# wuqianliang/Diff-Reg

Hardware: AMD Instinct MI355X
Metric: scene-pairs/sec @ 20 denoise steps (N=M=256); IR/FMR parity vs ref (higher is better)
Workload: dtype f32; 1 GPU; cfg2: 3DMatch N=M=256, C=432, 20 denoise steps, max_condition_num=200 (warp active), 256 independent B=1 pairs per pass per GPU as 2 concurrent batch(es), one HIP-graph replay each on its own stream; pairs_per_pass_per_gpu=256, streams=2, denoise_steps=20, N=256, M=256, graph=True, parallelism=pairs sharded over 1 GPU(s)

## Files before the change

diff-reg_amd/csrc/api.hip:

```cpp
#include <stdlib.h>
#include "loop_common.h"
#include <vector>
#include <stdio.h>
#include <string.h>

namespace dr {
static thread_local char g_hip_err[512] = "";
void set_hip_error(hipError_t e, const char* where) {
    snprintf(g_hip_err, sizeof(g_hip_err), "%s: %s (%d)", where, hipGetErrorString(e), (int)e);
}

static bool g_env_knobs = false;
void enable_env_knobs(bool on) { g_env_knobs = on; }
int env_knob(const char* name, int def) {
    if (!g_env_knobs) return def;
    const char* e = getenv(name);
    return e ? atoi(e) : def;
}

int device_cu_count() {
    static int cache[64];
    int d = 0;
    if (hipGetDevice(&d) != hipSuccess || d < 0 || d >= 64) return 256;
    if (!cache[d]) {
        hipDeviceProp_t pr;
        cache[d] = hipGetDeviceProperties(&pr, d) == hipSuccess && pr.multiProcessorCount > 0 ? pr.multiProcessorCount : 256;
    }
    return cache[d];
}

bool g_prof_on = false;
struct ProfRec { int kind; double work; hipEvent_t a, b; };
static std::vector<ProfRec> g_prof;
static std::vector<hipEvent_t> g_pool;
static hipEvent_t get_event() {
    if (!g_pool.empty()) { hipEvent_t e = g_pool.back(); g_pool.pop_back(); return e; }
    hipEvent_t e = nullptr; (void)hipEventCreate(&e); return e;
}
void prof_begin(int kind, double work, hipStream_t st) {
    ProfRec r; r.kind = kind; r.work = work; r.a = get_event(); r.b = nullptr;
    (void)hipEventRecord(r.a, st);
    g_prof.push_back(r);
}
void prof_end(int kind, hipStream_t st) {
    for (size_t i = g_prof.size(); i-- > 0;)
        if (g_prof[i].kind == kind && !g_prof[i].b) { g_prof[i].b = get_event(); (void)hipEventRecord(g_prof[i].b, st); return; }
}
}

namespace dr {
__global__ void noop_kernel(int* p) { if (p && threadIdx.x == 0 && blockIdx.x == 0) *p = 0; }
}

extern "C" {
void dr_prof_enable(int on) { dr::g_prof_on = on != 0; }

int dr_prof_collect(int* calls, double* ms, double* work) {
    using namespace dr;
    DR_HIP_CHECK(hipDeviceSynchronize());
    for (int k = 0; k < PK_COUNT; ++k) { calls[k] = 0; ms[k] = 0; work[k] = 0; }
    for (auto& r : g_prof) {
        if (r.b) {
            float t = 0.f;
            (void)hipEventElapsedTime(&t, r.a, r.b);
            calls[r.kind] += 1; ms[r.kind] += t; work[r.kind] += r.work;
            g_pool.push_back(r.b);
        }
        g_pool.push_back(r.a);
    }
    g_prof.clear();
    return DR_OK;
}

int dr_debug_launch_chain(int n, int workgroups, int threads, void* stream) {
    if (n < 0 || workgroups < 1 || threads < 64 || threads > 1024) return DR_EINVAL;
    for (int i = 0; i < n; ++i) hipLaunchKernelGGL(dr::noop_kernel, dim3(workgroups), dim3(threads), 0, (hipStream_t)stream, (int*)nullptr);
    DR_LAUNCH_CHECK();
    return DR_OK;
}

int dr_version(void) { return DR_ABI_VERSION;  }

const char* dr_strerror(int code) {
    switch (code) {
        case DR_OK: return "ok";
        case DR_EINVAL: return "invalid argument";
        case DR_ELAUNCH: return "HIP call failed";
        case DR_ENOSUP: return "shape not supported by this build";
        case DR_EWORKSPACE: return "workspace missing or too small";
        case DR_ETIMEOUT: return "a kernel gave up waiting for a workgroup that was not resident (outputs of that call are unspecified: NaN where the waiting workgroup wrote)";
        default: return "unknown error";
    }
}

const char* dr_last_hip_error(void) { return dr::g_hip_err; }
}

using namespace dr;

extern "C" {

int dr_init(void) {
    int rc = attention_configure();
    if (rc == DR_OK) rc = gemm_configure();
    if (rc == DR_OK) rc = pgemm_configure();
    if (rc == DR_OK) rc = vit_f32_configure();
    if (rc == DR_OK && !device_status_word()) rc = DR_ELAUNCH;
    return rc;
}

void dr_debug_enable_env(int on) { enable_env_knobs(on != 0); }
void dr_debug_gemm_config(int c) { gemm_force_config(c); }

int dr_debug_gemm_f32(const dr_debug_gemm_problem* problems, int n, void* stream) {
    if (!problems || n < 1 || n > 4) return DR_EINVAL;
    GemmBatch g;
    memset(&g, 0, sizeof(g));
    for (int i = 0; i < n; ++i) {
        const dr_debug_gemm_problem& q = problems[i];
        const int K1 = q.A2 ? q.K1 : q.K;
        if (q.rows < 0 || q.ncols <= 0 || q.K <= 0 || !q.A || !q.W || !q.out || q.nbatch < 0) return DR_EINVAL;
        if (q.lda < K1 || q.ldo < q.ncols || (q.A2 && (K1 <= 0 || K1 >= q.K || q.lda2 < q.K - K1))) return DR_EINVAL;
        if ((q.epilogue & ~(EPI_RELU | EPI_ROTARY)) ||
            ((q.epilogue & EPI_ROTARY) && (!q.cos_t || !q.sin_t || q.rot_C <= 0 || (q.rot_C & 1))))
            return DR_EINVAL;
        GemmProblem& p = g.p[i];
        p.A = q.A; p.A2 = q.A2; p.W = q.W; p.out = q.out; p.cosT = q.cos_t; p.sinT = q.sin_t; p.bias = q.bias; p.addend = q.addend;
        p.rows = q.rows; p.ncols = q.ncols; p.K = q.K; p.K1 = K1; p.lda = q.lda; p.lda2 = q.A2 ? q.lda2 : 0; p.ldo = q.ldo;
        p.epi = q.epilogue; p.rot_C = q.rot_C; p.scale = q.scale;
        p.nbatch = q.nbatch; p.sA = q.stride_a; p.sW = q.stride_w; p.sO = q.stride_o;
    }
    g.n = n;
    return launch_gemm(g, (hipStream_t)stream);
}
void dr_debug_attention_config(int flash_min_workgroups) { attention_force_flash_min(flash_min_workgroups); }
void dr_debug_attention_split(int on) { attention_force_split(on); }
int dr_debug_attention_last_form(void) { return attention_last_form(); }
int dr_debug_procrustes_last_form(void) { return procrustes_last_form(); }

int dr_vol_pe_f32(int rows, int rows_per_pair, int C, const float* xyz, const float* R, const float* t, float origin_x,
                  float origin_y, float origin_z, float voxel, const float* freq, float* cos_out, float* sin_out,
                  void* stream) {
    if (rows < 0 || C <= 0 || !xyz || !freq || !cos_out || !sin_out || rows_per_pair < 1) return DR_EINVAL;
    if ((R == nullptr) != (t == nullptr)) return DR_EINVAL;
    return launch_vol_pe(xyz, rows, rows_per_pair, R, t, C, origin_x, origin_y, origin_z, voxel, freq, cos_out, sin_out,
                         (hipStream_t)stream);
}

int dr_linear_f32(int rows, int ncols, int K, const float* x, const float* W, float* out, int epilogue, const float* cos_t,
                  const float* sin_t, int rot_C, float scale, void* stream) {
    if (rows < 0 || ncols <= 0 || K <= 0 || !x || !W || !out) return DR_EINVAL;
    if ((epilogue & EPI_ROTARY) && (!cos_t || !sin_t || rot_C <= 0 || (rot_C & 1))) return DR_EINVAL;
    return gemm1(x, K, W, nullptr, out, ncols, rows, ncols, K, epilogue, scale, nullptr, (hipStream_t)stream, cos_t, sin_t, rot_C);
}

int dr_gemm_nt_batched_f32(int nbatch, int rows, int ncols, int K, const float* A, long long stride_a, const float* W, long long stride_w, float* out,
                           long long stride_o, float scale, void* stream) {
    if (nbatch < 0 || rows < 0 || ncols <= 0 || K <= 0 || (K & 3) || !A || !W || !out) return DR_EINVAL;
    if (nbatch == 0 || rows == 0) return DR_OK;
    return gemm1(A, K, W, nullptr, out, ncols, rows, ncols, K, EPI_NONE, scale, nullptr, (hipStream_t)stream, nullptr, nullptr, 0, nbatch, stride_a,
                 stride_w, stride_o);
}

int dr_linear_ex_f32(int rows, int ncols, int K, const float* x, int lda, const float* W, const float* bias, float* out, int ldo,
                     int epilogue, float scale, void* stream) {
    if (rows < 0 || ncols <= 0 || K <= 0 || !x || !W || !out || lda < K || ldo < ncols || (epilogue & EPI_ROTARY)) return DR_EINVAL;
    return gemm1(x, lda, W, bias, out, ldo, rows, ncols, K, epilogue, scale, nullptr, (hipStream_t)stream);
}

size_t dr_procrustes_workspace_bytes(int P, int N, int M) {
    return (P < 1 || N < 1 || M < 1) ? 0 : procrustes_workspace_bytes(P, N, M);
}

int dr_procrustes_f32(int P, int N, int M, const float* conf, const float* src_pcd, const float* tgt_pcd,
                      const uint8_t* src_mask, const uint8_t* tgt_mask, int use_mask_len, float sample_rate,
                      float max_condition_num, float* R, float* t, float* R_forwd, float* t_forwd, double* condition,
                      int32_t* solution_mask, int32_t* topk_idx, void* workspace, size_t workspace_bytes, void* stream) {
    if (P < 0 || N < 1 || M < 1 || !conf || !src_pcd || !tgt_pcd || !R || !t || !R_forwd || !t_forwd || !condition || !solution_mask)
        return DR_EINVAL;
    if (P == 0) return DR_OK;
    const size_t wsb = procrustes_workspace_bytes(P, N, M);
    if (wsb && (!workspace || workspace_bytes < wsb)) return DR_EWORKSPACE;
    return launch_procrustes(conf, src_pcd, tgt_pcd, src_mask, tgt_mask, P, N, M, use_mask_len, sample_rate, max_condition_num,
                             R, t, R_forwd, t_forwd, condition, solution_mask, topk_idx, (hipStream_t)stream, wsb ? workspace : nullptr, wsb);
}

size_t dr_top1_union_workspace_bytes(int P, int N, int M, int elem_bytes) {
    return (P < 1 || N < 1 || M < 1 || (elem_bytes != 4 && elem_bytes != 8)) ? 0 : top1_union_workspace_bytes(P, N, M, (size_t)elem_bytes);
}

}
template <typename T>
static int top1_union_entry(const T* conf, int P, int N, int M, int64_t* matches, int32_t* count, void* ws, size_t ws_bytes, hipStream_t st) {
    if (P < 0 || N < 1 || M < 1 || !conf || !matches || !count) return DR_EINVAL;
    if (P == 0) return DR_OK;
    const size_t wsb = top1_union_workspace_bytes(P, N, M, sizeof(T));
    if (wsb && (!ws || ws_bytes < wsb)) return DR_EWORKSPACE;
    return launch_top1_union<T>(conf, P, N, M, (long long*)matches, count, st, nullptr, nullptr, wsb ? ws : nullptr, wsb);
}
extern "C" {
int dr_top1_union_f64(int P, int N, int M, const double* conf, int64_t* matches, int32_t* count, void* workspace, size_t workspace_bytes,
                      void* stream) {
    return top1_union_entry<double>(conf, P, N, M, matches, count, workspace, workspace_bytes, (hipStream_t)stream);
}
int dr_top1_union_f32(int P, int N, int M, const float* conf, int64_t* matches, int32_t* count, void* workspace, size_t workspace_bytes,
                      void* stream) {
    return top1_union_entry<float>(conf, P, N, M, matches, count, workspace, workspace_bytes, (hipStream_t)stream);
}

}
```

diff-reg_amd/csrc/loop.hip:

```cpp
#include "loop_common.h"

namespace dr {

struct LayerWs {
    float *qkv, *att, *mrg, *msg, *hid, *g2;
    size_t T;
    static size_t carve(Carver& c, LayerWs& w, size_t T, int C) {
        w.T = T;
        w.qkv = c.take<float>(T * 3 * C);
        w.att = c.take<float>(T * C);
        w.mrg = c.take<float>(T * C);
        w.msg = c.take<float>(T * C);
        w.hid = c.take<float>(T * 2 * C);
        w.g2 = c.take<float>(T * C);
        return c.off;
    }
};

struct PrepackLayer {
    PgW qkv, merge, mlp0, mlp2;
    const float *lnB1, *lnB2;
};
struct Prepack {
    static constexpr int MAXL = 16;
    PrepackLayer L[MAXL];
    PgW head;
    int dp;
    static bool supported(const dr_loop_config& cfg) {
        if (!(cfg.n_layers <= MAXL && pgemm_shape_ok(cfg.C) && cfg.C % cfg.H == 0 && (cfg.C / cfg.H) % 4 == 0)) return false;
        const int dp = (cfg.C / cfg.H + 15) / 16 * 16;
        return pgemm_shape_ok(cfg.H * dp) && pgemm_bn(cfg.H * dp) == pgemm_bn(cfg.C) && (dp == 64 || dp == 112 || dp == 144);
    }
    static bool wide_layout(const dr_loop_config& cfg) { return pgemm_bn(cfg.C) > 448 && env_knob("DR_PG_WIDE", 1) != 0; }
    static size_t carve(void* buf, const dr_loop_config& cfg, Prepack* pp) {
        Carver c(buf);
        const int C = cfg.C, d = C / cfg.H, dp = (d + 15) / 16 * 16, nC = C / 16;
        if (pp) pp->dp = dp;
        const bool wide = wide_layout(cfg);
        for (int l = 0; l < cfg.n_layers; ++l) {
            PrepackLayer* L = pp ? &pp->L[l] : nullptr;
            take_weight(c, C, 3, nC, L ? &L->qkv : nullptr, wide);
            take_weight(c, C, 1, cfg.H * dp / 16, L ? &L->merge : nullptr);
            take_weight(c, C, 2, 2 * nC, L ? &L->mlp0 : nullptr, wide);
            take_weight(c, C, 1, 2 * nC, L ? &L->mlp2 : nullptr);
            float* b = c.take<float>(2);
            if (L && buf) { L->lnB1 = b; L->lnB2 = b + 1; }
        }
        take_weight(c, C, 1, nC, pp ? &pp->head : nullptr, wide);
        return c.off + 256;
    }
    static int fill(void* buf, const dr_loop_config& cfg, const dr_loop_weights& W, hipStream_t st) {
        Prepack pp;
        carve(buf, cfg, &pp);
        const int C = cfg.C, d = C / cfg.H;
        for (int l = 0; l < cfg.n_layers; ++l) {
            const dr_layer_weights& w = W.layers[l];
            const PrepackLayer& L = pp.L[l];
            const int Cq = cfg.H * pp.dp;
            int rc = pack_weight_block(w.q_proj, Cq, C, C, C, L.qkv, 0, st, d, pp.dp);
            if (rc == DR_OK) rc = pack_weight_block(w.k_proj, Cq, C, C, C, L.qkv, 1, st, d, pp.dp);
            if (rc == DR_OK) rc = pack_weight_block(w.v_proj, Cq, C, C, C, L.qkv, 2, st, d, pp.dp);
            if (rc == DR_OK) rc = pack_weight_block(w.merge, C, C, d, pp.dp, L.merge, 0, st);
            if (rc == DR_OK) rc = pack_weight_block(w.mlp0, C, 2 * C, 2 * C, 2 * C, L.mlp0, 0, st);
            if (rc == DR_OK) rc = pack_weight_block(w.mlp0 + (size_t)C * 2 * C, C, 2 * C, 2 * C, 2 * C, L.mlp0, 1, st);
            if (rc == DR_OK) rc = pack_weight_block(w.mlp2, C, 2 * C, 2 * C, 2 * C, L.mlp2, 0, st);
            if (rc == DR_OK) rc = launch_ln_bound(w.norm1_w, w.norm1_b, C, (float*)L.lnB1, st);
            if (rc == DR_OK) rc = launch_ln_bound(w.norm2_w, w.norm2_b, C, (float*)L.lnB2, st);
            if (rc) return rc;
        }
        return pack_weight_block(W.src_proj, C, C, C, C, pp.head, 0, st);
    }
};

struct PlanesWs {
    bool on;
    Tok feat0, fa, fb, tgt_l0;
    char *att_img, *msg_img, *hid_img;
    float *att_bnd, *msg_bnd, *hid_bnd;
    char *qkv_img, *kvc_img;
    float *qkv_bnd, *kvc_bnd;
    float* grp_x;
    bool hoist;
    float* pre0;
    char* v0_img; float *v0_bnd, *grp0;
    char* q1_img; float* q1_bnd;
    float* csT;
    size_t qkv_stride;
    size_t side_C, side_att, side_hid;
    void* own_pack;
    float* xk_buf; unsigned* xk_flags; mutable unsigned xk_epoch; unsigned* status;
    static size_t img_bytes(int PN, int PM, int K) { return plane_image_bytes(PN, K) + plane_image_bytes(PM, K); }
    static void carve(Carver& c, PlanesWs& w, const dr_loop_config& cfg, int P, int N, int M) {
        const int C = cfg.C, PN = P * N, PM = P * M, T = PN + PM;
        w.on = planes_wanted(cfg.flags, Prepack::supported(cfg), T);
        if (!w.on) return;
        const int dp = (C / cfg.H + 15) / 16 * 16;
        w.side_C = plane_image_bytes(PN, C); w.side_att = plane_image_bytes(PN, cfg.H * dp); w.side_hid = plane_image_bytes(PN, 2 * C);
        Tok* toks[4] = {&w.feat0, &w.fa, &w.fb, &w.tgt_l0};
        for (Tok* t : toks) { t->f32 = nullptr; t->img = c.take<char>(img_bytes(PN, PM, C)); t->bnd = c.take<float>(T); }
        w.att_img = c.take<char>(img_bytes(PN, PM, cfg.H * dp)); w.att_bnd = c.take<float>(T);
        w.msg_img = c.take<char>(img_bytes(PN, PM, C)); w.msg_bnd = c.take<float>(T);
        w.hid_img = c.take<char>(img_bytes(PN, PM, 2 * C)); w.hid_bnd = c.take<float>(T);
        w.qkv_stride = (img_bytes(PN, PM, cfg.H * dp) + 255) & ~(size_t)255;
        w.qkv_img = c.take<char>(3 * w.qkv_stride); w.qkv_bnd = c.take<float>(3 * (size_t)T);
        w.kvc_img = c.take<char>(2 * w.qkv_stride); w.kvc_bnd = c.take<float>(2 * (size_t)T);
        w.grp_x = c.take<float>(2 * (size_t)P);
        w.hoist = false;
        w.csT = c.take<float>((size_t)T * C);
        w.own_pack = c.take<char>(Prepack::carve(nullptr, cfg, nullptr));
        const bool xk = (T + 63) / 64 + 2 <= PG_XK_MAX_RB;
        w.xk_buf = xk ? c.take<float>(pgemm_xk_buf_bytes(pgemm_bn(C)) / 4) : nullptr;
        w.xk_flags = xk ? c.take<unsigned>(pgemm_xk_flag_bytes() / 4) : nullptr;
        w.xk_epoch = 0; w.status = nullptr;
    }
    static void carve_hoist(PlanesWs& w, char* mem, size_t bytes, const dr_loop_config& cfg, int P, int N, int M) {
        const int PN = P * N, PM = P * M, T = PN + PM, Cq = cfg.H * ((cfg.C / cfg.H + 15) / 16 * 16);
        Carver c(mem);
        w.pre0 = c.take<float>((size_t)PN * 2 * Cq);
        w.v0_img = c.take<char>(plane_image_bytes(PN, Cq)); w.v0_bnd = c.take<float>(PN); w.grp0 = c.take<float>(P);
        w.q1_img = c.take<char>(plane_image_bytes(PM, Cq)); w.q1_bnd = c.take<float>(T);
        w.hoist = c.off <= bytes && env_knob("DR_LOOP_HOIST", 1) != 0;
    }
};

static int layer_call(const dr_layer_weights& W, int C, int H, int P, const float* xin, int xr0, int xrows,
                      const float* yin, int yr0, int yrows, const float* cosT, const float* sinT,
                      const uint8_t* tokmask, const Family& f1, const Family* f2, const LayerWs& ws, float* out,
                      hipStream_t st, const float* kv_cached = nullptr, float* kv_store = nullptr, const float* xq_in = nullptr,
                      const float* yk_in = nullptr) {
    const int halfC = C / 2, d = C / H;
    const bool rotary = cosT != nullptr;
    const float* const qin = xq_in ? xq_in : xin;
    const float* const kin = yk_in ? yk_in : yin;
    GemmBatch g;
    memset(&g, 0, sizeof(g));
    auto proj = [&](GemmProblem& p, const float* in, int r0, int rows, const float* Wm, int coloff, bool rot) {
        p.A = in + (size_t)r0 * C; p.A2 = nullptr; p.W = Wm; p.out = ws.qkv + (size_t)r0 * 3 * C + coloff;
        p.rows = rows; p.ncols = C; p.K = C; p.K1 = C; p.lda = C; p.lda2 = 0; p.ldo = 3 * C;
        p.epi = (rot && rotary) ? EPI_ROTARY : EPI_NONE; p.rot_C = C; p.scale = 1.f;
        p.cosT = rotary ? cosT + (size_t)r0 * halfC : nullptr; p.sinT = rotary ? sinT + (size_t)r0 * halfC : nullptr;
    };
    int rc;
    if (kv_store) {
        proj(g.p[0], kin, yr0, yrows, W.k_proj, 0, true);
        proj(g.p[1], yin, yr0, yrows, W.v_proj, 0, false);
        g.p[0].out = kv_store + (size_t)yr0 * 2 * C; g.p[0].ldo = 2 * C;
        g.p[1].out = kv_store + (size_t)yr0 * 2 * C + C; g.p[1].ldo = 2 * C;
        g.n = 2;
        return launch_gemm(g, st);
    }
    proj(g.p[0], qin, xr0, xrows, W.q_proj, 0, true);
    g.n = 1;
    if (!kv_cached) {
        proj(g.p[1], kin, yr0, yrows, W.k_proj, C, true);
        proj(g.p[2], yin, yr0, yrows, W.v_proj, 2 * C, false);
        g.n = 3;
    }
    rc = launch_gemm(g, st);
    if (rc) return rc;

    AttnArgs a;
    memset(&a, 0, sizeof(a));
    a.q = ws.qkv; a.k = ws.qkv + C; a.v = ws.qkv + 2 * C; a.out = ws.att;
    a.ldq = a.ldk = a.ldv = 3 * C; a.ldo = C; a.H = H; a.d = d;
    if (kv_cached) { a.k = kv_cached; a.v = kv_cached + C; a.ldk = a.ldv = 2 * C; }
    a.qmask = tokmask; a.kmask = tokmask;
    attn_families(a, P, f1, f2);
    a.scale = 1.0f / sqrtf((float)d);
    rc = launch_attention(a, st);
    if (rc) return rc;

    memset(&g, 0, sizeof(g));
    GemmProblem& m = g.p[0];
    m.A = ws.att + (size_t)xr0 * C; m.W = W.merge; m.out = ws.mrg + (size_t)xr0 * C;
    m.rows = xrows; m.ncols = C; m.K = C; m.K1 = C; m.lda = C; m.ldo = C; m.epi = EPI_NONE; m.scale = 1.f;
    g.n = 1;
    rc = launch_gemm(g, st);
    if (rc) return rc;
    rc = launch_layernorm(ws.mrg + (size_t)xr0 * C, C, W.norm1_w, W.norm1_b, nullptr, 0, ws.msg + (size_t)xr0 * C, C, xrows, C, st);
    if (rc) return rc;
    memset(&g, 0, sizeof(g));
    GemmProblem& h = g.p[0];
    h.A = xin + (size_t)xr0 * C; h.A2 = ws.msg + (size_t)xr0 * C; h.W = W.mlp0; h.out = ws.hid + (size_t)xr0 * 2 * C;
    h.rows = xrows; h.ncols = 2 * C; h.K = 2 * C; h.K1 = C; h.lda = C; h.lda2 = C; h.ldo = 2 * C; h.epi = EPI_RELU; h.scale = 1.f;
    g.n = 1;
    rc = launch_gemm(g, st);
    if (rc) return rc;
    memset(&g, 0, sizeof(g));
    GemmProblem& o = g.p[0];
    o.A = ws.hid + (size_t)xr0 * 2 * C; o.W = W.mlp2; o.out = ws.g2 + (size_t)xr0 * C;
    o.rows = xrows; o.ncols = C; o.K = 2 * C; o.K1 = 2 * C; o.lda = 2 * C; o.ldo = C; o.epi = EPI_NONE; o.scale = 1.f;
    g.n = 1;
    rc = launch_gemm(g, st);
    if (rc) return rc;
    return launch_layernorm(ws.g2 + (size_t)xr0 * C, C, W.norm2_w, W.norm2_b, xin + (size_t)xr0 * C, C, out + (size_t)xr0 * C, C,
                            xrows, C, st);
}


using PlCtx = PlaneCtx<Prepack, PlanesWs>;
static void xk_assign(const PlanesWs& pw, int C, PgProblem& p, size_t& next, size_t units) {
    if (!pw.xk_buf || next + units > (size_t)PG_XK_MAX_RB) return;
    p.xk_buf = pw.xk_buf + next * (pgemm_xk_buf_bytes(pgemm_bn(C)) / 4 / PG_XK_MAX_RB); p.xk_flags = pw.xk_flags + next * 2; p.xk_cap = (int)units;
    p.xk_epoch = pw.xk_epoch + 1; p.xk_status = pw.status;
    next += units;
}
static size_t xk_wide_units(const PgProblem& p) { return (size_t)(p.rows + 127) / 128 * p.nblk * 2; }

struct PlHoist {
    bool l0_fill = false;
    bool l0_use = false;
    bool q1_fill = false;
    bool q1_use = false;
};
static int layer_call_planes(const PlCtx& X, const dr_layer_weights& W, int l, const Tok& xin, int xs, const Tok& yin, int ys,
                             const Tok& out, const Family& f1, const Family* f2, hipStream_t st, const float* kv_cached = nullptr,
                             float* kv_store = nullptr, const PlHoist& hz = PlHoist()) {
    const Sides& S = X.S;
    const int C = X.C, H = X.H, PN = S.rows_a, PM = S.rows_b, halfC = C / 2, d = C / H, nC = C / 16, dp = X.pp->dp;
    const PrepackLayer& L = X.pp->L[l];
    const PlanesWs& pw = *X.pw;
    PgBatch g;
    size_t xk_next = 0;
    auto reset = [&]() { memset(&g, 0, sizeof(g)); xk_next = 0; };
    auto add = [&]() -> PgProblem& { return g.p[g.n++]; };
    auto xk = [&](PgProblem& p, size_t units) { xk_assign(pw, C, p, xk_next, units); };
    int rc;

    const int T = PN + PM, Cq = H * dp, nq = Cq / 16;
    const bool cached = kv_cached != nullptr;
    char* const kv_img = kv_store ? pw.kvc_img : pw.qkv_img + pw.qkv_stride;
    float* const kv_bnd = kv_store ? pw.kvc_bnd : pw.qkv_bnd + T;
    const bool grp_inline = S.La % 128 == 0 && S.Lb % 128 == 0 && env_knob("DR_LOOP_GRP_INLINE", 1) != 0;
    if (!cached && !grp_inline && !hz.l0_fill && !hz.l0_use && !hz.q1_fill) {
        rc = side_group_max(S, ys, yin.bnd, pw.grp_x, st);
        if (rc) return rc;
    }
    auto proj = [&](const Tok& tin, int side, int b0, int nblk, char* img, float* bnd, int rotm, int grpm) {
        PgProblem& p = add();
        p.A0 = S.at(tin.img, pw.side_C, side); p.bnd0 = tin.bnd + S.r0(side); p.nc0 = nC;
        p.W = pgw_blocks(L.qkv, b0, C); p.nblk = nblk; p.rows = S.rows(side); p.C = Cq; p.k_alg = C; p.mode = PG_PLANES;
        p.rot_mask = rotm; p.rot_C = C; p.rot_piece_len = d; p.rot_piece_pad = dp; p.scale = 1.f;
        p.cosT = X.cosT + (size_t)S.r0(side) * halfC; p.sinT = X.sinT + (size_t)S.r0(side) * halfC;
        p.csT = X.pw->csT + (size_t)S.r0(side) * halfC * 2;
        p.pimg = S.at(img, pw.side_att, side); p.p_nct = nq; p.pbnd = bnd + S.r0(side);
        p.pimg_blk_stride = (long long)pw.qkv_stride; p.pbnd_blk_stride = T;
        p.grp_bnd = grp_inline ? nullptr : pw.grp_x; p.grp_mask = grpm; p.grp_first = S.grp_first(side); p.grp_rows = S.per_pair(side);
        if (p.W.sub == 2) xk(p, xk_wide_units(p));
    };
    reset();
    if (kv_store) {
        S.for_sides(ys, [&](int side) { proj(yin, side, 1, 2, kv_img, kv_bnd, 1, 3); });
        ++pw.xk_epoch;
        return launch_pgemm(g, st);
    }
    const int rbS = (PN + 127) / 128, rbT = (PM + 127) / 128;
    if (hz.l0_fill) {
        rc = launch_group_max(xin.bnd, S.P, S.La, pw.grp0, st);
        if (rc) return rc;
        proj(xin, SIDE_A, 0, 2, pw.qkv_img, pw.qkv_bnd, 0, 0);
        g.p[0].mode = PG_F32; g.p[0].pimg = nullptr; g.p[0].pbnd = nullptr;
        g.p[0].out = pw.pre0; g.p[0].ldo = 2 * Cq; g.p[0].blk_stride = Cq;
        g.wg_as = 3 * rbS;
        ++pw.xk_epoch;
        rc = launch_pgemm(g, st);
        if (rc) return rc;
        reset();
        proj(xin, SIDE_A, 2, 1, pw.v0_img, pw.v0_bnd, 0, 1);
        g.p[0].grp_bnd = pw.grp0; g.p[0].grp_first = 0;
        g.wg_as = 3 * rbS;
        ++pw.xk_epoch;
        return launch_pgemm(g, st);
    }
    if (hz.q1_fill) {
        proj(xin, SIDE_B, 0, 1, pw.qkv_img, pw.qkv_bnd, 1, 0);
        g.p[0].pimg = pw.q1_img; g.p[0].pbnd = pw.q1_bnd + PN;
        g.wg_as = rbT + 2 * rbS;
        ++pw.xk_epoch;
        return launch_pgemm(g, st);
    }
    const bool self = xs == ys && xin.img == yin.img && !cached;
    if (hz.l0_use) {
        RotImgArgs r;
        memset(&r, 0, sizeof(r));
        r.x = pw.pre0; r.ldx = 2 * Cq; r.x_blk = Cq; r.rows = PN; r.C = Cq; r.nblk = 2;
        r.csT = pw.csT; r.rot_mask = 3; r.rot_C = C; r.rot_piece_len = d; r.rot_piece_pad = dp; r.scale = 1.f;
        r.bnd0 = xin.bnd; r.wnorm = L.qkv.wnorm; r.wide_form = L.qkv.sub == 2; r.grp_bnd = pw.grp0; r.grp_mask = 2; r.grp_first = 0; r.grp_rows = S.La;
        r.pimg = pw.qkv_img; r.p_nct = nq; r.pbnd = pw.qkv_bnd; r.pimg_blk_stride = (long long)pw.qkv_stride; r.pbnd_blk_stride = T;
        rc = launch_rot_images(r, st);
        if (rc) return rc;
    } else {
        if (self) {
            S.for_sides(xs, [&](int side) { proj(xin, side, 0, 3, pw.qkv_img, pw.qkv_bnd, 3, 6); });
        } else {
            if (!hz.q1_use) S.for_sides(xs, [&](int side) { proj(xin, side, 0, 1, pw.qkv_img, pw.qkv_bnd, 1, 0); });
            else g.wg_as = rbT + 2 * rbS;
            if (!cached) S.for_sides(ys, [&](int side) { proj(yin, side, 1, 2, kv_img, kv_bnd, 1, 3); });
        }
        ++pw.xk_epoch;
        rc = launch_pgemm(g, st);
        if (rc) return rc;
    }

    AttnArgs a;
    memset(&a, 0, sizeof(a));
    a.H = H; a.d = d;
    a.qmask = X.tokmask; a.kmask = X.tokmask;
    attn_families(a, S.P, f1, f2);
    a.scale = 1.0f / sqrtf((float)d);
    a.pimg[0] = pw.att_img; a.pimg[1] = pw.att_img + pw.side_att; a.p_split = PN; a.p_nct = nq; a.p_dp = dp;
    a.pbnd = pw.att_bnd;
    {
        const char* kimg = cached ? pw.kvc_img : pw.qkv_img + pw.qkv_stride;
        const float* kb = cached ? pw.kvc_bnd : pw.qkv_bnd + T;
        a.qimg[0] = pw.qkv_img; a.qimg[1] = pw.qkv_img + pw.side_att;
        a.kimg[0] = kimg; a.kimg[1] = kimg + pw.side_att;
        a.vimg[0] = kimg + pw.qkv_stride; a.vimg[1] = kimg + pw.qkv_stride + pw.side_att;
        a.qbnd = pw.qkv_bnd; a.kgb = kb; a.vgb = kb + T;
        if (hz.l0_use) { a.vimg[0] = pw.v0_img; a.vgb = pw.v0_bnd; }
        if (hz.q1_use) { a.qimg[1] = pw.q1_img; a.qbnd = pw.q1_bnd; }
        a.f16_single = X.attn_f16;
    }
    rc = launch_attention(a, st);
    if (rc) return rc;

    reset();
    S.for_sides(xs, [&](int side) {
        PgProblem& p = add();
        p.A0 = S.at(pw.att_img, pw.side_att, side); p.bnd0 = pw.att_bnd + S.r0(side); p.nc0 = H * dp / 16;
        p.W = L.merge; p.nblk = 1; p.rows = S.rows(side); p.C = C; p.mode = PG_LN; p.k_alg = C;
        p.gamma = W.norm1_w; p.beta = W.norm1_b; p.lnB = L.lnB1;
        p.pimg = S.at(pw.msg_img, pw.side_C, side); p.p_nct = nC; p.pbnd = pw.msg_bnd + S.r0(side);
        xk(p, (size_t)(p.rows + 63) / 64);
    });
    ++pw.xk_epoch;
    rc = launch_pgemm(g, st);
    if (rc) return rc;
    reset();
    S.for_sides(xs, [&](int side) {
        PgProblem& p = add();
        p.A0 = S.at(xin.img, pw.side_C, side); p.bnd0 = xin.bnd + S.r0(side); p.nc0 = nC;
        p.A1 = S.at(pw.msg_img, pw.side_C, side); p.bnd1 = pw.msg_bnd + S.r0(side); p.nc1 = nC;
        p.W = L.mlp0; p.nblk = 2; p.rows = S.rows(side); p.C = C; p.mode = PG_PLANES; p.relu = 1; p.scale = 1.f;
        p.pimg = S.at(pw.hid_img, pw.side_hid, side); p.p_nct = 2 * nC; p.pbnd = pw.hid_bnd + S.r0(side);
        if (p.W.sub == 2) xk(p, xk_wide_units(p));
    });
    ++pw.xk_epoch;
    rc = launch_pgemm(g, st);
    if (rc) return rc;
    reset();
    S.for_sides(xs, [&](int side) {
        PgProblem& p = add();
        p.A0 = S.at(pw.hid_img, pw.side_hid, side); p.bnd0 = pw.hid_bnd + S.r0(side); p.nc0 = 2 * nC;
        p.W = L.mlp2; p.nblk = 1; p.rows = S.rows(side); p.C = C; p.mode = PG_LN;
        p.gamma = W.norm2_w; p.beta = W.norm2_b; p.lnB = L.lnB2;
        p.resid = xin.f32 + (size_t)S.r0(side) * C; p.ldr = C; p.bnd_res = xin.bnd + S.r0(side);
        p.out = out.f32 + (size_t)S.r0(side) * C; p.ldo = C;
        p.pimg = S.at(out.img, pw.side_C, side); p.p_nct = nC; p.pbnd = out.bnd + S.r0(side);
        xk(p, (size_t)(p.rows + 63) / 64);
    });
    ++pw.xk_epoch;
    return launch_pgemm(g, st);
}

struct DenoiseWs {
    LayerWs lw;
    float *fa, *fb, *cosT, *sinT, *proj, *sim;
    float *tgt_l0, *kv_l1;
    PlanesWs pl;
    const Prepack* pp;
    Sides S;
    static void carve(Carver& c, DenoiseWs& w, const dr_loop_config& cfg, int P, int N, int M) {
        const int C = cfg.C;
        w.S = Sides(P, N, M);
        const size_t T = (size_t)P * (N + M);
        const size_t lw_begin = align256(c.off);
        LayerWs::carve(c, w.lw, T, C);
        const size_t lw_end = c.off;
        PlanesWs::carve(c, w.pl, cfg, P, N, M);
        if (w.pl.on) PlanesWs::carve_hoist(w.pl, c.base ? c.base + lw_begin : nullptr, lw_end - lw_begin, cfg, P, N, M);
        w.tgt_l0 = c.take<float>(T * C);
        w.kv_l1 = c.take<float>(T * 2 * C);
        w.fa = c.take<float>(T * C);
        w.fb = c.take<float>(T * C);
        w.cosT = c.take<float>(T * (C / 2));
        w.sinT = c.take<float>(T * (C / 2));
        w.proj = c.take<float>(T * C);
        w.sim = c.take<float>((size_t)P * N * M);
        if (w.pl.on) { w.pl.fa.f32 = w.fa; w.pl.fb.f32 = w.fb; w.pl.tgt_l0.f32 = w.tgt_l0; }
    }
};

static PlCtx plane_ctx(const dr_loop_config& cfg, const DenoiseWs& ws, const uint8_t* tokmask) {
    return PlCtx{ws.pp, &ws.pl, ws.S, cfg.C, cfg.H, (cfg.flags & DR_LOOP_ATTN_F16) ? 1 : 0, ws.cosT, ws.sinT, tokmask};
}
static int layer_call_sides(const dr_loop_config& cfg, const dr_layer_weights& W, const float* x, int xs, const float* y, int ys, const uint8_t* tokmask,
                            const Family& f1, const Family* f2, const DenoiseWs& ws, float* out, hipStream_t st, const float* kv_cached = nullptr,
                            float* kv_store = nullptr) {
    const Sides& S = ws.S;
    return layer_call(W, cfg.C, cfg.H, S.P, x, S.r0(xs), S.rows(xs), y, S.r0(ys), S.rows(ys), ws.cosT, ws.sinT, tokmask, f1, f2, ws.lw, out, st,
                      kv_cached, kv_store);
}

static int fill_step_invariants(const dr_loop_config& cfg, const dr_loop_weights& w, const float* feat0, const uint8_t* tokmask, DenoiseWs& ws,
                                hipStream_t st) {
    const Family self_s = ws.S.self_a(), self_t = ws.S.self_b();
    if (ws.pl.on) {
        const PlCtx X = plane_ctx(cfg, ws, tokmask);
        int rc = layer_call_planes(X, w.layers[0], 0, ws.pl.feat0, SIDE_B, ws.pl.feat0, SIDE_B, ws.pl.tgt_l0, self_t, nullptr, st);
        if (rc == DR_OK && ws.pl.hoist) {
            PlHoist hz; hz.l0_fill = true;
            rc = layer_call_planes(X, w.layers[0], 0, ws.pl.feat0, SIDE_A, ws.pl.feat0, SIDE_A, ws.pl.tgt_l0, self_s, nullptr, st, nullptr, nullptr, hz);
        }
        if (rc || cfg.n_layers < 2) return rc;
        rc = layer_call_planes(X, w.layers[1], 1, ws.pl.tgt_l0, 0, ws.pl.tgt_l0, SIDE_B, ws.pl.tgt_l0, self_t, nullptr, st, nullptr, ws.kv_l1);
        if (rc || !ws.pl.hoist) return rc;
        PlHoist hz; hz.q1_fill = true;
        return layer_call_planes(X, w.layers[1], 1, ws.pl.tgt_l0, SIDE_B, ws.pl.tgt_l0, 0, ws.pl.tgt_l0, self_t, nullptr, st, nullptr, nullptr, hz);
    }
    int rc = layer_call_sides(cfg, w.layers[0], feat0, SIDE_B, feat0, SIDE_B, tokmask, self_t, nullptr, ws, ws.tgt_l0, st);
    if (rc || cfg.n_layers < 2) return rc;
    return layer_call_sides(cfg, w.layers[1], nullptr, 0, ws.tgt_l0, SIDE_B, tokmask, self_t, nullptr, ws, nullptr, st, nullptr, ws.kv_l1);
}

static int denoiser_and_sim(const dr_loop_config& cfg, const dr_loop_weights& w, const float* feat0, const uint8_t* tokmask, DenoiseWs& ws,
                            const float** final_feats, hipStream_t st, bool use_cache = false) {
    const Sides& S = ws.S;
    const int C = cfg.C, P = S.P, N = S.La, M = S.Lb, PN = S.rows_a;
    auto head = [&](const float* feats) {
        return gemm1(feats, C, w.src_proj, nullptr, ws.proj, C, S.rows(SIDE_BOTH), C, C, EPI_ROTARY, 1.0f / sqrtf((float)C), nullptr, st, ws.cosT, ws.sinT, C);
    };
    auto sim = [&]() {
        return gemm1(ws.proj, C, ws.proj + (size_t)PN * C, nullptr, ws.sim, M, N, M, C, EPI_NONE, 1.f, nullptr, st, nullptr, nullptr, 0, P,
                     (long long)N * C, (long long)M * C, (long long)N * M);
    };
    const int l_begin = use_cache ? 1 : 0;
    if (ws.pl.on) {
        const PlCtx X = plane_ctx(cfg, ws, tokmask);
        const Tok* cur = &ws.pl.feat0;
        int rc = DR_OK;
        if (use_cache) {
            PlHoist hz; hz.l0_use = ws.pl.hoist;
            rc = layer_call_planes(X, w.layers[0], 0, *cur, SIDE_A, *cur, SIDE_A, ws.pl.tgt_l0, S.self_a(), nullptr, st, nullptr, nullptr, hz);
            cur = &ws.pl.tgt_l0;
        }
        if (rc == DR_OK)
            rc = layer_schedule(S, l_begin, cfg.n_layers, cur, (const Tok*)&ws.pl.fa, (const Tok*)&ws.pl.fb,
                                [&](int l, int xs, const Tok* x, int ys, const Tok* y, const Tok* out, const Family& f1, const Family* f2) {
                const bool l1 = use_cache && l == 1;
                PlHoist hz; hz.q1_use = l1 && xs == SIDE_B && ws.pl.hoist;
                return layer_call_planes(X, w.layers[l], l, *x, xs, *y, ys, *out, f1, f2, st, (l1 && xs == SIDE_A) ? ws.kv_l1 : nullptr, nullptr, hz);
            });
        if (rc) return rc;
        *final_feats = cur->f32;
        if (env_knob("DR_HEAD_F32", 0)) {
            rc = head(cur->f32);
            return rc ? rc : sim();
        }
        PgBatch g;
        memset(&g, 0, sizeof(g));
        size_t xk_next = 0;
        S.for_sides(SIDE_BOTH, [&](int side) {
            PgProblem& p = g.p[g.n++];
            const int r0 = S.r0(side);
            p.A0 = S.at(cur->img, ws.pl.side_C, side); p.bnd0 = cur->bnd + r0; p.nc0 = C / 16;
            p.W = ws.pp->head; p.nblk = 1; p.rows = S.rows(side); p.C = C; p.mode = PG_F32;
            p.out = ws.proj + (size_t)r0 * C; p.ldo = C; p.blk_stride = 0; p.rot_mask = 1; p.rot_C = C; p.scale = 1.0f / sqrtf((float)C);
            p.cosT = ws.cosT + (size_t)r0 * (C / 2); p.sinT = ws.sinT + (size_t)r0 * (C / 2);
            p.csT = ws.pl.csT + (size_t)r0 * C;
            if (p.W.sub == 2) xk_assign(ws.pl, C, p, xk_next, xk_wide_units(p));
        });
        ++ws.pl.xk_epoch;
        rc = launch_pgemm(g, st);
        return rc ? rc : sim();
    }
    const float* cur = feat0;
    int rc = DR_OK;
    if (use_cache) {
        rc = layer_call_sides(cfg, w.layers[0], cur, SIDE_A, cur, SIDE_A, tokmask, S.self_a(), nullptr, ws, ws.tgt_l0, st);
        cur = ws.tgt_l0;
    }
    if (rc == DR_OK)
        rc = layer_schedule(S, l_begin, cfg.n_layers, cur, ws.fa, ws.fb,
                            [&](int l, int xs, const float* x, int ys, const float* y, float* out, const Family& f1, const Family* f2) {
            return layer_call_sides(cfg, w.layers[l], x, xs, y, ys, tokmask, f1, f2, ws, out, st, (use_cache && l == 1 && xs == SIDE_A) ? ws.kv_l1 : nullptr);
        });
    if (rc) return rc;
    *final_feats = cur;
    rc = head(cur);
    return rc ? rc : sim();
}

static int fill_pe(const dr_loop_config& cfg, const dr_loop_weights& w, int P, int N, int M, const float* s_pcd,
                   const float* Rf, const float* tf, const float* t_pcd, bool do_src, bool do_tgt, DenoiseWs& ws,
                   hipStream_t st) {
    const int halfC = cfg.C / 2;
    int rc = DR_OK;
    if (do_src)
        rc = launch_vol_pe(s_pcd, P * N, N, Rf, tf, cfg.C, cfg.origin[0], cfg.origin[1], cfg.origin[2], cfg.voxel, w.pe_freq,
                           ws.cosT, ws.sinT, st, ws.pl.on ? ws.pl.csT : nullptr);
    if (rc == DR_OK && do_tgt)
        rc = launch_vol_pe(t_pcd, P * M, M, nullptr, nullptr, cfg.C, cfg.origin[0], cfg.origin[1], cfg.origin[2], cfg.voxel,
                           w.pe_freq, ws.cosT + (size_t)P * N * halfC, ws.sinT + (size_t)P * N * halfC, st,
                           ws.pl.on ? ws.pl.csT + (size_t)P * N * halfC * 2 : nullptr);
    return rc;
}

struct LoopWs {
    DenoiseWs dw;
    float *feat0, *wconf, *x0, *R, *t, *Rf, *tf, *conf32;
    double *x, *dmin, *cond;
    void* pmin;
    int* ok;
    uint8_t* tokmask;
    void* skws;
    size_t skws_bytes;
    void* pws;
    size_t pws_bytes;
    unsigned* status;
    static size_t carve(Carver& c, LoopWs& w, const dr_loop_config& cfg, int P, int N, int M) {
        const size_t T = (size_t)P * (N + M), NM = (size_t)P * N * M;
        w.status = c.take<unsigned>(4);
        DenoiseWs::carve(c, w.dw, cfg, P, N, M);
        w.feat0 = c.take<float>(T * cfg.C);
        if (w.dw.pl.on) w.dw.pl.feat0.f32 = w.feat0;
        w.wconf = c.take<float>(NM);
        w.x0 = c.take<float>(NM);
        w.conf32 = c.take<float>(NM);
        w.x = c.take<double>(NM);
        w.dmin = c.take<double>(P);
        w.cond = c.take<double>(P);
        w.pmin = (void*)c.take<char>(pair_min_scratch_bytes(P));
        w.R = c.take<float>((size_t)P * 9);
        w.t = c.take<float>((size_t)P * 3);
        w.Rf = c.take<float>((size_t)P * 9);
        w.tf = c.take<float>((size_t)P * 3);
        w.ok = c.take<int>(P);
        w.tokmask = c.take<uint8_t>(T);
        sampler_scratch(c, P, N, M, cfg.flags, w.skws, w.skws_bytes, w.pws, w.pws_bytes);
        return c.off + 256;
    }
};

static int planes_begin(const dr_loop_config& cfg, const dr_loop_weights& w, DenoiseWs& ws, Prepack& pp, hipStream_t st) {
    if (!ws.pl.on) return DR_OK;
    int rc = packed_or_own(cfg, w, ws.pl.own_pack, pp, st);
    if (rc) return rc;
    ws.pp = &pp;
    if (ws.pl.xk_flags) {
        DR_HIP_CHECK(hipMemsetAsync(ws.pl.xk_flags, 0, pgemm_xk_flag_bytes(), st));
        ws.pl.xk_epoch = 0;
    }
    ws.S.for_sides(SIDE_BOTH, [&](int side) { if (rc == DR_OK) rc = side_planes_from_f32(ws.S, side, ws.pl.feat0, cfg.C, ws.pl.side_C, st); });
    return rc;
}

static int loop_begin(const dr_loop_config& cfg, int P, int N, int M, const float* src_feats, const float* tgt_feats, const uint8_t* src_mask,
                      const uint8_t* tgt_mask, void* workspace, LoopWs& L, hipStream_t st) {
    Carver c(workspace);
    LoopWs::carve(c, L, cfg, P, N, M);
    DR_HIP_CHECK(hipMemsetAsync(L.status, 0, 16, st));
    L.dw.pl.status = L.status;
    const size_t PN = (size_t)P * N, PM = (size_t)P * M;
    DR_HIP_CHECK(hipMemcpyAsync(L.feat0, src_feats, PN * cfg.C * 4, hipMemcpyDeviceToDevice, st));
    DR_HIP_CHECK(hipMemcpyAsync(L.feat0 + PN * cfg.C, tgt_feats, PM * cfg.C * 4, hipMemcpyDeviceToDevice, st));
    if (src_mask) {
        DR_HIP_CHECK(hipMemcpyAsync(L.tokmask, src_mask, PN, hipMemcpyDeviceToDevice, st));
        DR_HIP_CHECK(hipMemcpyAsync(L.tokmask + PN, tgt_mask, PM, hipMemcpyDeviceToDevice, st));
    }
    return DR_OK;
}

}

using namespace dr;

extern "C" {

size_t dr_attention_layer_workspace_bytes(int P, int Lx, int Ly, int C) {
    Carver c(nullptr);
    LayerWs w;
    const size_t T = (size_t)P * (Lx + Ly);
    LayerWs::carve(c, w, T, C);
    c.take<float>(T * C);
    c.take<float>(T * C);
    c.take<float>(T * (C / 2));
    c.take<float>(T * (C / 2));
    c.take<uint8_t>(T);
    c.take<float>(T * C);
    return c.off + 256;
}

int dr_attention_layer_f32(const dr_layer_weights* w, int C, int H, int P, int Lx, int Ly, const float* x, const float* y,
                           const float* cos_x, const float* sin_x, const float* cos_y, const float* sin_y,
                           const uint8_t* x_mask, const uint8_t* y_mask, float* out, void* workspace,
                           size_t workspace_bytes, void* stream) {
    if (!cos_x || !sin_x || !cos_y || !sin_y) return DR_EINVAL;
    return dr_attention_layer_pe_f32(w, C, H, P, Lx, Ly, x, y, nullptr, nullptr, cos_x, sin_x, cos_y, sin_y, x_mask, y_mask, out, workspace,
                                     workspace_bytes, stream);
}

int dr_attention_layer_pe_f32(const dr_layer_weights* w, int C, int H, int P, int Lx, int Ly, const float* x, const float* y,
                              const float* xq, const float* yk, const float* cos_x, const float* sin_x, const float* cos_y, const float* sin_y,
                              const uint8_t* x_mask, const uint8_t* y_mask, float* out, void* workspace,
                              size_t workspace_bytes, void* stream) {
    if (!w || !x || !y || !out || P < 1 || Lx < 1 || Ly < 1 || C % H || (C / H) % 4 || C % 4) return DR_EINVAL;
    if ((x_mask == nullptr) != (y_mask == nullptr)) return DR_EINVAL;
    const bool rotary = cos_x != nullptr;
    if ((sin_x != nullptr) != rotary || (cos_y != nullptr) != rotary || (sin_y != nullptr) != rotary) return DR_EINVAL;
    if ((xq == nullptr) != (yk == nullptr) || (xq && rotary)) return DR_EINVAL;
    if (workspace_bytes < dr_attention_layer_workspace_bytes(P, Lx, Ly, C) || !workspace) return DR_EWORKSPACE;
    hipStream_t st = (hipStream_t)stream;
    Carver c(workspace);
    LayerWs lw;
    const size_t T = (size_t)P * (Lx + Ly), PX = (size_t)P * Lx, PY = (size_t)P * Ly;
    const int halfC = C / 2;
    LayerWs::carve(c, lw, T, C);
    float* tok = c.take<float>(T * C);
    float* otok = c.take<float>(T * C);
    float* cosT = c.take<float>(T * halfC);
    float* sinT = c.take<float>(T * halfC);
    uint8_t* mask = c.take<uint8_t>(T);
    float* qk_buf = c.take<float>(T * C);
    DR_HIP_CHECK(hipMemcpyAsync(tok, x, PX * C * 4, hipMemcpyDeviceToDevice, st));
    DR_HIP_CHECK(hipMemcpyAsync(tok + PX * C, y, PY * C * 4, hipMemcpyDeviceToDevice, st));
    float* qk_tok = nullptr;
    if (rotary) {
        DR_HIP_CHECK(hipMemcpyAsync(cosT, cos_x, PX * halfC * 4, hipMemcpyDeviceToDevice, st));
        DR_HIP_CHECK(hipMemcpyAsync(cosT + PX * halfC, cos_y, PY * halfC * 4, hipMemcpyDeviceToDevice, st));
        DR_HIP_CHECK(hipMemcpyAsync(sinT, sin_x, PX * halfC * 4, hipMemcpyDeviceToDevice, st));
        DR_HIP_CHECK(hipMemcpyAsync(sinT + PX * halfC, sin_y, PY * halfC * 4, hipMemcpyDeviceToDevice, st));
    } else if (xq) {
        qk_tok = qk_buf;
        DR_HIP_CHECK(hipMemcpyAsync(qk_tok, xq, PX * C * 4, hipMemcpyDeviceToDevice, st));
        DR_HIP_CHECK(hipMemcpyAsync(qk_tok + PX * C, yk, PY * C * 4, hipMemcpyDeviceToDevice, st));
    }
    if (x_mask) {
        DR_HIP_CHECK(hipMemcpyAsync(mask, x_mask, PX, hipMemcpyDeviceToDevice, st));
        DR_HIP_CHECK(hipMemcpyAsync(mask + PX, y_mask, PY, hipMemcpyDeviceToDevice, st));
    }
    const Family f{0, Lx, (int)PX, Ly};
    int rc = layer_call(*w, C, H, P, tok, 0, (int)PX, tok, (int)PX, (int)PY, rotary ? cosT : nullptr, rotary ? sinT : nullptr,
                        x_mask ? mask : nullptr, f, nullptr, lw, otok, st, nullptr, nullptr, qk_tok, qk_tok);
    if (rc) return rc;
    DR_HIP_CHECK(hipMemcpyAsync(out, otok, PX * C * 4, hipMemcpyDeviceToDevice, st));
    return DR_OK;
}

static int check_cfg(const dr_loop_config* cfg, const dr_loop_weights* w, int P, int N, int M) {
    if (!cfg || !w || P < 1 || N < 1 || M < 1) return DR_EINVAL;
    if (cfg->C % cfg->H || (cfg->C / cfg->H) % 4 || cfg->C % 6 || cfg->n_layers < 1 || cfg->sk_iters < 1) return DR_EINVAL;
    if (!w->layers || !w->src_proj || !w->bin_score || !w->pe_freq) return DR_EINVAL;
    if (cfg->variant != DR_VARIANT_3DMATCH && cfg->variant != DR_VARIANT_4DMATCH) return DR_EINVAL;
    return DR_OK;
}

size_t dr_loop_prepack_bytes(const dr_loop_config* cfg) {
    if (!cfg || !Prepack::supported(*cfg)) return 0;
    return Prepack::carve(nullptr, *cfg, nullptr);
}

int dr_loop_prepack(const dr_loop_config* cfg, const dr_loop_weights* w, void* packed, size_t packed_bytes, void* stream) {
    if (!cfg || !w || !w->layers || !w->src_proj || !packed || ((uintptr_t)packed & 255)) return DR_EINVAL;
    if (!Prepack::supported(*cfg)) return DR_ENOSUP;
    if (packed_bytes < Prepack::carve(nullptr, *cfg, nullptr)) return DR_EWORKSPACE;
    return Prepack::fill(packed, *cfg, *w, (hipStream_t)stream);
}

size_t dr_denoise_loop_workspace_bytes(const dr_loop_config* cfg, int P, int N, int M) {
    if (!cfg || P < 1 || N < 1 || M < 1) return 0;
    Carver c(nullptr);
    LoopWs w;
    return LoopWs::carve(c, w, *cfg, P, N, M);
}

int dr_denoise_loop_status(void* workspace, void* stream, int clear) {
    if (!workspace) return DR_EINVAL;
    Carver c(workspace);
    return sinkhorn_call_status(c.take<unsigned>(4), (hipStream_t)stream, clear != 0);
}

int dr_denoiser_match_f32(const dr_loop_config* cfg, const dr_loop_weights* w, int P, int N, int M, const float* src_feats,
                          const float* tgt_feats, const float* s_pcd_warped, const float* t_pcd, const uint8_t* src_mask,
                          const uint8_t* tgt_mask, float* src_out, float* tgt_out, float* conf, void* workspace,
                          size_t workspace_bytes, void* stream) {
    int rc = check_cfg(cfg, w, P, N, M);
    if (rc) return rc;
    if (!src_feats || !tgt_feats || !s_pcd_warped || !t_pcd || !conf) return DR_EINVAL;
    if ((src_mask == nullptr) != (tgt_mask == nullptr)) return DR_EINVAL;
    if (!workspace || workspace_bytes < dr_denoise_loop_workspace_bytes(cfg, P, N, M)) return DR_EWORKSPACE;
    hipStream_t st = (hipStream_t)stream;
    LoopWs L;
    rc = loop_begin(*cfg, P, N, M, src_feats, tgt_feats, src_mask, tgt_mask, workspace, L, st);
    if (rc) return rc;
    const int C = cfg->C;
    const size_t PN = (size_t)P * N, PM = (size_t)P * M;
    Prepack pp;
    rc = planes_begin(*cfg, *w, L.dw, pp, st);
    if (rc) return rc;
    rc = fill_pe(*cfg, *w, P, N, M, s_pcd_warped, nullptr, nullptr, t_pcd, true, true, L.dw, st);
    if (rc) return rc;
    const float* fin = nullptr;
    rc = denoiser_and_sim(*cfg, *w, L.feat0, src_mask ? L.tokmask : nullptr, L.dw, &fin, st);
    if (rc) return rc;
    if (src_out) DR_HIP_CHECK(hipMemcpyAsync(src_out, fin, PN * C * 4, hipMemcpyDeviceToDevice, st));
    if (tgt_out) DR_HIP_CHECK(hipMemcpyAsync(tgt_out, fin + PN * C, PM * C * 4, hipMemcpyDeviceToDevice, st));
    return sinkhorn_f32(P, N, M, L.dw.sim, src_mask, tgt_mask, w->bin_score, cfg->sk_iters,
                        DR_SK_OUT_CONF | (src_mask ? DR_SK_APPLY_MASK : 0), conf, L.skws, L.skws_bytes, st, L.status);
}

int dr_denoise_loop(const dr_loop_config* cfg, const dr_loop_weights* w, int P, int N, int M, const float* src_feats,
                    const float* tgt_feats, const float* s_pcd, const float* t_pcd, const uint8_t* src_mask,
                    const uint8_t* tgt_mask, const float* x_T, const float* noise, double* conf, double* x_final,
                    int64_t* matches, int32_t* match_count, float* R_final, float* t_final, const dr_loop_trace* trace,
                    void* workspace, size_t workspace_bytes, void* stream) {
    int rc = check_cfg(cfg, w, P, N, M);
    if (rc) return rc;
    if (!src_feats || !tgt_feats || !s_pcd || !t_pcd || !x_T || !conf || cfg->steps < 1 || !cfg->h_alphas_cumprod || !cfg->h_times)
        return DR_EINVAL;
    if ((src_mask == nullptr) != (tgt_mask == nullptr)) return DR_EINVAL;
    const bool v4d = cfg->variant == DR_VARIANT_4DMATCH;
    if (v4d && !noise) return DR_EINVAL;
    if ((matches == nullptr) != (match_count == nullptr) || (R_final == nullptr) != (t_final == nullptr)) return DR_EINVAL;
    if (trace && (trace->force_R == nullptr) != (trace->force_t == nullptr)) return DR_EINVAL;
    if (!workspace || workspace_bytes < dr_denoise_loop_workspace_bytes(cfg, P, N, M)) return DR_EWORKSPACE;
    hipStream_t st = (hipStream_t)stream;
    LoopWs L;
    rc = loop_begin(*cfg, P, N, M, src_feats, tgt_feats, src_mask, tgt_mask, workspace, L, st);
    if (rc) return rc;
    const int C = cfg->C;
    const size_t PN = (size_t)P * N, PM = (size_t)P * M, NM = (size_t)P * N * M;
    const uint8_t* tokmask = src_mask ? L.tokmask : nullptr;
    const int strict = (cfg->flags & DR_LOOP_STRICT_F64) ? DR_SK_STRICT : 0;
    const bool ragged = (cfg->flags & DR_LOOP_RAGGED) && src_mask;
    const int mflag = src_mask ? (DR_SK_APPLY_MASK | (ragged ? DR_SK_RAGGED : 0)) : 0;
    const uint8_t* rsm = ragged ? src_mask : nullptr;
    const uint8_t* rtm = ragged ? tgt_mask : nullptr;

    rc = launch_f32_to_f64(x_T, L.x, NM, st);
    if (rc) return rc;
    if (!v4d && P <= 32)
        DR_HIP_CHECK(hipMemsetAsync((char*)L.pmin + pair_min_scratch_bytes(P) - 64 * (size_t)P, 0, 64 * (size_t)P, st));
    Prepack pp;
    rc = planes_begin(*cfg, *w, L.dw, pp, st);
    if (rc) return rc;
    rc = fill_pe(*cfg, *w, P, N, M, s_pcd, nullptr, nullptr, t_pcd, false, true, L.dw, st);
    if (rc) return rc;
    rc = fill_step_invariants(*cfg, *w, L.feat0, tokmask, L.dw, st);
    if (rc) return rc;

    const float* fin = nullptr;
    SamplerArgs sa;
    memset(&sa, 0, sizeof(sa));
    sa.P = P; sa.N = N; sa.M = M; sa.steps = cfg->steps; sa.alphas_cumprod = cfg->h_alphas_cumprod; sa.times = cfg->h_times;
    sa.sample_rate = cfg->sample_rate; sa.max_condition_num = cfg->max_condition_num; sa.sk_iters = cfg->sk_iters; sa.strict = strict;
    sa.s_pcd = s_pcd; sa.warp_tgt_pcd = t_pcd; sa.src_mask = src_mask; sa.warp_tgt_mask = tgt_mask;
    sa.warp_mflag = mflag; sa.use_mask_len = (v4d || ragged) ? 1 : 0;
    sa.min_shift = !v4d; sa.rsm = rsm; sa.rtm = rtm; sa.dmin = L.dmin; sa.pmin = P <= 32 ? L.pmin : nullptr;
    sa.noise = v4d ? noise : nullptr; sa.bin_score = w->bin_score; sa.trace = trace;
    sa.x = L.x; sa.x_final = x_final; sa.x0 = L.x0; sa.wconf = L.wconf; sa.R = L.R; sa.t = L.t; sa.Rf = L.Rf; sa.tf = L.tf; sa.cond = L.cond; sa.ok = L.ok;
    sa.skws = L.skws; sa.skws_bytes = L.skws_bytes; sa.pws = L.pws; sa.pws_bytes = L.pws_bytes; sa.status = L.status;
    rc = reverse_sampling(sa, [&](const float* Rf, const float* tf) -> int {
        int r = fill_pe(*cfg, *w, P, N, M, s_pcd, Rf, tf, t_pcd, true, false, L.dw, st);
        if (r == DR_OK) r = denoiser_and_sim(*cfg, *w, L.feat0, tokmask, L.dw, &fin, st, true);
        if (r) return r;
        return sinkhorn_f32(P, N, M, L.dw.sim, src_mask, tgt_mask, w->bin_score, cfg->sk_iters, DR_SK_OUT_CONF | mflag, L.x0, L.skws, L.skws_bytes, st,
                            L.status);
    }, st);
    if (rc) return rc;
    if (trace && (trace->feats_nopos || trace->feats_pos) && fin) {
        for (int pos = 0; pos < 2; ++pos) {
            float* dst = pos ? trace->feats_pos : trace->feats_nopos;
            if (!dst) continue;
            rc = gemm1(fin, C, w->src_proj, nullptr, dst, C, (int)(PN + PM), C, C, pos ? EPI_ROTARY : EPI_NONE, 1.f, nullptr, st, L.dw.cosT, L.dw.sinT, C);
            if (rc) return rc;
        }
    }

    if (v4d) {
        rc = launch_sigmoid(L.x, conf, NM, st);
        if (rc) return rc;
    } else {
        rc = launch_pair_min(L.x, P, N * M, L.dmin, st, M, rsm, rtm, P <= 32 ? L.pmin : nullptr);
        if (rc) return rc;
        rc = sinkhorn_f64(P, N, M, L.x, L.dmin, src_mask, tgt_mask, w->bin_score, cfg->sk_iters, DR_SK_OUT_CONF | mflag | strict,
                          conf, L.skws, L.skws_bytes, st, L.status);
        if (rc) return rc;
        if (matches) {
            rc = launch_top1_union<double>(conf, P, N, M, (long long*)matches, match_count, st, rsm, rtm, L.x0, NM * 4);
            if (rc) return rc;
        }
    }
    if (R_final) {
        rc = launch_f64_to_f32(conf, L.conf32, NM, st);
        if (rc) return rc;
        rc = launch_procrustes(L.conf32, s_pcd, t_pcd, src_mask, tgt_mask, P, N, M, (v4d || ragged) ? 1 : 0, cfg->sample_rate,
                               cfg->max_condition_num, R_final, t_final, L.Rf, L.tf, L.cond, L.ok, nullptr, st, L.pws, L.pws_bytes);
        if (rc) return rc;
    }
    return DR_OK;
}

}
```

diff-reg_amd/csrc/pgemm.h:

```cpp
#pragma once
#include "kernels.h"

namespace dr {

constexpr int PI_BM = 128;
inline size_t plane_image_bytes(size_t rows, int K) { return ((rows + PI_BM - 1) / PI_BM) * (size_t)(K / 16) * (PI_BM * 64); }

struct PgW {
    const char* img;
    const float* cinv;
    const float* wnorm;
    int nct;
    int sub;
};

enum { PG_F32 = 0, PG_PLANES = 1, PG_LN = 2 };

struct PgProblem {
    const char* A0; const char* A1;
    const float* bnd0; const float* bnd1;
    int nc0, nc1;
    PgW W;
    int nblk;
    int rows, C;
    int k_alg;
    int mode;
    float* out; int ldo; int blk_stride;
    const float* cosT; const float* sinT; int rot_mask; int rot_C; float scale;
    const float* csT;
    int rot_piece_len, rot_piece_pad;
    char* pimg; int p_nct; int p_kc0; float* pbnd;
    long long pimg_blk_stride; long long pbnd_blk_stride;
    const float* grp_bnd; int grp_mask, grp_first, grp_rows;
    int relu;
    const float* gamma; const float* beta; const float* resid; int ldr; const float* bnd_res; const float* lnB;
    int ln_postadd;
    const float* bias; const float* bias_max;
    float* xk_buf; unsigned* xk_flags; unsigned xk_epoch; unsigned* xk_status; int ksplit;
    int xk_cap;
};
constexpr int PG_XK_MAX_RB = 160;
inline size_t pgemm_xk_buf_bytes(int bn) { return (size_t)PG_XK_MAX_RB * 2 * 4 * (bn / 64) * 2 * 64 * 16; }
inline size_t pgemm_xk_flag_bytes() { return (size_t)PG_XK_MAX_RB * 2 * sizeof(unsigned); }
struct PgBatch { PgProblem p[3]; int n; int dbg; int wg_as; };

bool pgemm_shape_ok(int C);
int pgemm_bn(int C);
int launch_pgemm(const PgBatch& g, hipStream_t st);
int pgemm_configure();

size_t pgemm_weight_bytes(int C, int nblk, int nct);
void pgemm_weight_view(void* buf, int C, int nblk, int nct, PgW* view);
int pgemm_pack_weights(const float* W, int nblk, int C, int K, int piece_len, int piece_pad, void* buf, hipStream_t st);
int pgemm_pack_weights_block(const float* W, int C, int K, int piece_len, int piece_pad, const PgW& view, int nb, hipStream_t st, int out_len = 0,
                             int out_pad = 0);
bool pgemm16w_shape_ok(int C);
size_t pgemm16w_weight_bytes(int nblk, int nct);
void pgemm16w_weight_view(void* buf, int nblk, int nct, PgW* view);
int pgemm16w_pack_weights_block(const float* W, int C, int K, int piece_len, int piece_pad, const PgW& view, int nb, hipStream_t st, int out_len = 0,
                                int out_pad = 0);
int launch_group_max(const float* bnd, int ngroups, int grp_rows, float* out, hipStream_t st);

struct RotImgArgs {
    const float* x; int ldx, x_blk;
    int rows, C, nblk;
    const float* csT; int rot_mask, rot_C, rot_piece_len, rot_piece_pad; float scale;
    const float* bnd0;
    const float* wnorm;
    int wide_form;
    const float* grp_bnd; int grp_mask, grp_first, grp_rows;
    char* pimg; int p_nct; float* pbnd; long long pimg_blk_stride, pbnd_blk_stride;
};
int launch_rot_images(const RotImgArgs& a, hipStream_t st);

int launch_planes_from_f32(const float* x, int ldx, int rows, int K, char* img, float* bnd, hipStream_t st, const float* bnd_in = nullptr);
int launch_planes_to_f32(const char* img, const float* bnd, int rows, int K, float* out, int ldo, hipStream_t st);
int launch_ln_bound(const float* gamma, const float* beta, int C, float* out, hipStream_t st);
int launch_absmax_blocks(const float* x, int nblk, int n, float* out, hipStream_t st);

}
```

diff-reg_amd/csrc/pgemm.hip:

```cpp
#include <cstdlib>
#include <string.h>
#include <type_traits>
#include "pgemm.h"

namespace dr {
namespace {

typedef float f32x16 __attribute__((ext_vector_type(16)));
typedef float f32x2 __attribute__((ext_vector_type(2)));
typedef _Float16 f16x8 __attribute__((ext_vector_type(8)));
typedef _Float16 f16x2 __attribute__((ext_vector_type(2)));
typedef unsigned u32x4 __attribute__((ext_vector_type(4)));
typedef __attribute__((address_space(3))) void lds_void;
typedef const __attribute__((address_space(1))) void glb_void;

__device__ __forceinline__ void split2(float x0, float x1, unsigned& hi, unsigned& lo) {
    const f32x2 f = {x0, x1};
    const f16x2 h = __builtin_convertvector(f, f16x2);
    hi = __builtin_bit_cast(unsigned, h);
    const f32x2 hf = __builtin_convertvector(h, f32x2);
    const f32x2 r = {x0 - hf.x, x1 - hf.y};
    lo = __builtin_bit_cast(unsigned, __builtin_convertvector(r, f16x2));
}
__device__ __forceinline__ int scale_exp(float m) {
    const unsigned bits = __float_as_uint(m);
    const int e = (int)((bits >> 23) & 0xff) - 127;
    const bool ok = m > 0.f && e < 128;
    return ok ? min(max(14 - e, -100), 100) : 0;
}
__device__ __forceinline__ float pow2i(int s) { return __uint_as_float((unsigned)(127 + s) << 23); }
__device__ __forceinline__ unsigned dpp_xor1(unsigned v) {
    return (unsigned)__builtin_amdgcn_mov_dpp((int)v, 0xB1, 0xF, 0xF, true);
}
__device__ __forceinline__ float dpp_xor1f(float v) { return __uint_as_float(dpp_xor1(__float_as_uint(v))); }
__device__ __forceinline__ float dpp_xor2f(float v) {
    return __uint_as_float((unsigned)__builtin_amdgcn_mov_dpp((int)__float_as_uint(v), 0x4E, 0xF, 0xF, true));
}
__device__ __forceinline__ void wave_fence() {
    __builtin_amdgcn_fence(__ATOMIC_ACQ_REL, "wavefront");
    __builtin_amdgcn_wave_barrier();
}

template <int TNW_, int NST_, int WMN_ = 4>
struct PgGeom {
    static constexpr int TNW = TNW_, NST = NST_, WMN = WMN_;
    static constexpr int BM = 32 * WMN, BNW = 32 * TNW, BN = 2 * BNW, NTHR = 128 * WMN;
    static constexpr int A_ST = BM * 64, B_ST = BN * 64, STAGE = A_ST + B_ST;
    static constexpr int A_IMG = 128 * 64;
    static constexpr int NA = A_ST / 1024;
    static constexpr int NB = B_ST / 1024;
    static constexpr int NFULL = NB / 8, REM = NB % 8;
    static constexpr int RING = NST * STAGE;
    static constexpr int NI = BNW / 16;
    static constexpr int EP_S = (BNW - 48 + 63) / 64 * 64 + 48;
    static constexpr int EP_BYTES = 2 * WMN * 16 * EP_S * 4;
    static constexpr int WORK = RING > EP_BYTES ? RING : EP_BYTES;
    static constexpr int SMEM = WORK + 7 * 128 * 4 + 4 * BN * 4;
    static constexpr int SMEM16 = WORK + 11 * 128 * 4 + 4 * BN * 4;
    static constexpr int MID = (TNW - 1) / 2 - 1 < 0 ? 0 : (TNW - 1) / 2 - 1;
};

#define PG_READ(dst, addr, off) asm volatile("ds_read_b128 %0, %1 offset:%2" : "=v"(dst) : "v"(addr), "i"(off) : "memory")
#define PG_VMCNT(n) asm volatile("s_waitcnt vmcnt(%0)" ::"i"(n) : "memory")

typedef float f32x4 __attribute__((ext_vector_type(4)));

template <int TNW, int NST, int MODE, int WMN = 4, bool M16 = false>
__global__ __launch_bounds__(128 * WMN) __attribute__((amdgpu_waves_per_eu(WMN / 2, WMN / 2))) void pgemm_kernel(PgBatch G) {
    using GG = PgGeom<TNW, NST, WMN>;
    constexpr int BNW = GG::BNW, BN = GG::BN, STAGE = GG::STAGE, A_ST = GG::A_ST, NI = GG::NI, EP_S = GG::EP_S, BM = GG::BM, NTHR = GG::NTHR;
    extern __shared__ __attribute__((aligned(16))) float smem[];
    char* const lds = reinterpret_cast<char*>(smem);
    const unsigned lds_base = (unsigned)(size_t)(lds_void*)lds;

    const PgProblem& P = G.p[blockIdx.y];
    constexpr bool KS_OK = !M16 && WMN == 2 && MODE == PG_LN;
    const bool ksplit = KS_OK && P.ksplit != 0;
    const int rows = P.rows, C = P.C, nblk = ksplit ? 2 : P.nblk, nc1 = P.A1 ? P.nc1 : 0;
    const int rbs = (rows + BM - 1) / BM;
    const int grp = blockIdx.x / (8 * nblk), rem = blockIdx.x % (8 * nblk);
    const int rb = grp * 8 + (rem & 7), khalf = ksplit ? (rem >> 3) : 0, nb = ksplit ? 0 : (rem >> 3);
    if (rb >= rbs) return;
    const int kbeg = khalf ? (P.nc0 + 1) / 2 : 0;
    const int nc0 = ksplit ? (khalf ? P.nc0 - kbeg : (P.nc0 + 1) / 2) : P.nc0, nst = nc0 + nc1;
    const int t = threadIdx.x, lane = t & 63, l31 = lane & 31, h = lane >> 5;
    const int w = __builtin_amdgcn_readfirstlane(t >> 6), wm = w % WMN, wn = w / WMN;
    const int rb128 = (rb * BM) >> 7, sub = (rb * BM) & 127;

    float* const s_fac = reinterpret_cast<float*>(lds + GG::WORK);
    float* const s_rinv = s_fac + 128;
    constexpr int NCW = M16 ? 4 : 2;
    float* const s_sum = s_rinv + 128;
    float* const s_sq = s_sum + NCW * 128;
    const bool has_bias = P.bias != nullptr;
    float* const s_bias = s_sq + NCW * 128 + 2 * BN;
    float* const s_gam = s_sq + NCW * 128;
    float* const s_bet = s_gam + BN;
    float* const s_cinv = s_bias + BN;
    float* const s_bound = s_cinv + BN;
    const bool rot = MODE != PG_LN && ((P.rot_mask >> nb) & 1);
    const bool per_blk = P.pimg_blk_stride != 0;
    auto stage_inputs = [&]() __attribute__((always_inline)) {
        if (has_bias) {
            const float* bp = P.bias + (size_t)nb * C;
            for (int c = t; c < BN; c += NTHR) s_bias[c] = c < C ? bp[c] : 0.f;
        }
        {
            const float* cp = P.W.cinv + (size_t)nb * BN;
            for (int c = t; c < BN; c += NTHR) s_cinv[c] = cp[c];
            if (MODE == PG_LN && P.gamma)
                for (int c = t; c < BN; c += NTHR) {
                    s_gam[c] = c < C ? P.gamma[c] : 0.f;
                    s_bet[c] = c < C ? P.beta[c] : 0.f;
                }
        }
        float gmax = 0.f;
        if (MODE != PG_LN && ((P.grp_mask >> nb) & 1) && !P.grp_bnd) {
            const int gbase = (rb * BM) / P.grp_rows * P.grp_rows;
            float m = 0.f;
            for (int i = t; i < P.grp_rows; i += NTHR) m = fmaxf(m, P.bnd0[gbase + i]);
            m = wave_max(m);
            if (lane == 0) s_sum[w] = m;
            __syncthreads();
#pragma unroll
            for (int k = 0; k < NTHR / 64; ++k) gmax = fmaxf(gmax, s_sum[k]);
        }
        if (t < BM) {
            const int row = min(rb * BM + t, rows - 1);
            const float b0 = P.bnd0[row], b1 = nc1 > 0 ? P.bnd1[row] : 0.f;
            const int e0 = scale_exp(b0);
            int e1 = e0;
            if (nc1 > 0) e1 = scale_exp(b1);
            s_fac[t] = pow2i(min(max(e1 - e0, -120), 120));
            s_rinv[t] = pow2i(-e1);
            if (P.pimg) {
                float bound;
                if (MODE == PG_LN) bound = ((P.bnd_res && !P.ln_postadd) ? P.bnd_res[row] : 0.f) + (P.lnB ? P.lnB[0] : 0.f);
                else {
                    const float bin = ((P.grp_mask >> nb) & 1) ? (P.grp_bnd ? P.grp_bnd[P.grp_first + row / P.grp_rows] : gmax) : fmaxf(b0, b1);
                    float wn_ = P.W.wnorm[nb];
                    if (!per_blk)
                        for (int b2 = 0; b2 < nblk; ++b2) wn_ = fmaxf(wn_, P.W.wnorm[b2]);
                    float bm = 0.f;
                    if (P.bias_max) {
                        bm = P.bias_max[nb];
                        if (!per_blk)
                            for (int b2 = 0; b2 < nblk; ++b2) bm = fmaxf(bm, P.bias_max[b2]);
                    }
                    bound = (bin * wn_ + bm) * (rot ? 1.41421366f : 1.f) * fabsf(P.scale);
                }
                s_bound[t] = bound;
            }
        }
    };

    const int sw = (l31 >> 2) & 3;
    const unsigned offAh = (wm * 32 + l31) * 64 + ((h ^ sw) << 4), offAl = (wm * 32 + l31) * 64 + (((2 + h) ^ sw) << 4);
    const unsigned offBh = A_ST + (wn * BNW + l31) * 64 + ((h ^ sw) << 4), offBl = A_ST + (wn * BNW + l31) * 64 + (((2 + h) ^ sw) << 4);

    f32x16 acc[TNW];
#pragma unroll
    for (int j = 0; j < TNW; ++j)
#pragma unroll
        for (int r = 0; r < 16; ++r) acc[j][r] = 0.f;
    u32x4 fa0[2], fa1[2], fx[TNW / 2][2], fy[TNW - TNW / 2][2];
    f32x4 c16[M16 ? 4 : 1][M16 ? 7 : 1];

    auto run = [&](auto grp_t) __attribute__((always_inline)) {
        constexpr int GRP = decltype(grp_t)::value;
        constexpr bool EARLY = GRP == 0 && NST >= 4;
        constexpr int AHEAD = EARLY ? NST - 2 : NST - 1;
        constexpr bool ALL0 = NST >= 4 && WMN == 4;
        constexpr int AG = ALL0 ? 0 : 1;
        constexpr int WB_CNT = ALL0 ? 0 : (GG::NB + GG::NA) / 2 - GG::NA;
        constexpr int NW0 = GG::NB - WB_CNT;
        constexpr int NAP = GRP == AG ? 2 : 0;
        constexpr int NPIECE = GRP ? NAP + (WB_CNT + WMN - 1) / WMN : NAP + (NW0 + WMN - 1) / WMN;
        constexpr int NFULLP = GRP ? NAP + WB_CNT / WMN : NAP + NW0 / WMN;
        constexpr int PSTEP = (2 * NPIECE <= 3 * (TNW - TNW / 2)) ? 2 : 1;
        static_assert(EARLY || PSTEP * NPIECE <= 3 * (TNW - TNW / 2), "the DMA pieces of a stage must fit the gaps of the second burst");
        static_assert(!EARLY || NPIECE <= 3 * (TNW / 2), "... and those of the early group the gaps of the first");
        constexpr int REMP = GRP ? WB_CNT % WMN : NW0 % WMN;
        const int wl = w % WMN;
        const int st0 = GRP ? wl * (WB_CNT / WMN) + min(wl, WB_CNT % WMN) : WB_CNT + wl * (NW0 / WMN) + min(wl, NW0 % WMN);
        const unsigned voffW = lane * 16 + st0 * 1024, voffA = lane * 16 + 2 * wl * 1024;
        const char* ga = P.A0 + ((size_t)rb128 * P.nc0 + kbeg) * GG::A_IMG + sub * 64;
        const char* gb = P.W.img + ((size_t)nb * (P.nc0 + nc1) + kbeg) * GG::B_ST;
        const char* const ga1 = nc1 > 0 ? P.A1 + (size_t)rb128 * nc1 * GG::A_IMG + sub * 64 : nullptr;
        int ti = 0;
#define PG_DMA(ldsaddr, voff, gbase, imm)                                                                  \
    asm volatile("s_mov_b32 m0, %0\n\ts_nop 0\n\tglobal_load_lds_dwordx4 %1, %2 offset:%3" ::"s"(ldsaddr), "v"(voff), "s"(gbase), "i"(imm) : "memory")
        auto dma_piece = [&](int p, unsigned dstb) __attribute__((always_inline)) {
            const unsigned m0w = dstb + A_ST + st0 * 1024;
            const int pw = p - NAP;
            const unsigned hop = (unsigned)(pw >> 2) * 4096;
            if (p < NAP) PG_DMA(dstb + 2 * wl * 1024, voffA, ga, p * 1024);
            else if (pw < (GRP ? WB_CNT : NW0) / WMN || wl < (GRP ? WB_CNT : NW0) % WMN) PG_DMA(m0w + hop, voffW + hop, gb, (pw & 3) * 1024);
        };
        auto dma_advance = [&]() __attribute__((always_inline)) {
            ++ti;
            gb += GG::B_ST;
            ga = (ti == nc0) ? ga1 : ga + GG::A_IMG;
        };

        auto stage = [&](int s, auto steady_t, u32x4 (&ac)[2], u32x4 (&an)[2]) __attribute__((always_inline)) {
            constexpr bool STEADY = decltype(steady_t)::value;
            constexpr int NT1 = TNW / 2, NT2 = TNW - NT1, M1 = 3 * NT1;
            const unsigned sb = lds_base + (unsigned)(s % NST) * STAGE, sbn = lds_base + (unsigned)((s + 1) % NST) * STAGE;
            const unsigned Bh = sb + offBh, Bl = sb + offBl, Bhn = sbn + offBh, Bln = sbn + offBl;
            const bool has_next = STEADY || s + 1 < nst;
            const bool do_issue = STEADY || ti < nst;
            const unsigned dstb = lds_base + (unsigned)(ti % NST) * STAGE;
            if (s == nc0 && nc1 > 0) {
                const unsigned fb0 = lds_base + GG::WORK + (wm * 32 + 4 * h) * 4;
                u32x4 f[4];
                PG_READ(f[0], fb0, 0); PG_READ(f[1], fb0, 32); PG_READ(f[2], fb0, 64); PG_READ(f[3], fb0, 96);
                asm volatile("s_waitcnt lgkmcnt(0)" ::: "memory");
                __builtin_amdgcn_sched_barrier(0);
#pragma unroll
                for (int j = 0; j < TNW; ++j)
#pragma unroll
                    for (int r = 0; r < 16; ++r) acc[j][r] *= __uint_as_float(f[r >> 2][r & 3]);
                __builtin_amdgcn_sched_barrier(0);
            }
            auto gap = [&](int m) __attribute__((always_inline)) {
                {
                    if (m < NT2) {
                        PG_READ(fy[m][0], Bh, (NT1 + m) * 2048);
                        PG_READ(fy[m][1], Bl, (NT1 + m) * 2048);
                    } else if (m == M1 && has_next) {
                        PG_READ(an[0], sbn + offAh, 0);
                        PG_READ(an[1], sbn + offAl, 0);
                    } else if (m > M1 && m <= M1 + NT1 && has_next) {
                        PG_READ(fx[m - M1 - 1][0], Bhn, (m - M1 - 1) * 2048);
                        PG_READ(fx[m - M1 - 1][1], Bln, (m - M1 - 1) * 2048);
                    }
                }
                constexpr int MF = EARLY ? 0 : (PSTEP == 2 ? M1 + 1 : M1), STEP = EARLY ? 1 : PSTEP;
                if (m >= MF && m < MF + STEP * NPIECE && (m - MF) % STEP == 0) {
                    if (do_issue) dma_piece((m - MF) / STEP, dstb);
                    if ((m - MF) / STEP == NPIECE - 1 && do_issue) dma_advance();
                }
                if (m == M1 - 1) {
                    if (has_next) {
                        if (NST >= 4 && (STEADY || s + 2 < nst)) {
                            if (wl < REMP) PG_VMCNT(NFULLP + 1); else PG_VMCNT(NFULLP);
                        } else {
                            PG_VMCNT(0);
                        }
                    }
                    __builtin_amdgcn_s_barrier();
                    asm volatile("s_waitcnt lgkmcnt(0)" ::: "memory");
                }
            };
            const f16x8 ah = __builtin_bit_cast(f16x8, ac[0]), al = __builtin_bit_cast(f16x8, ac[1]);
#define PG_MFMA(X, Y, g)                                                        \
    acc[j] = __builtin_amdgcn_mfma_f32_32x32x16_f16(X, Y, acc[j], 0, 0, 0);      \
    __builtin_amdgcn_sched_barrier(0);                                          \
    gap(3 * j + g);                                                             \
    __builtin_amdgcn_sched_barrier(0);
            asm volatile("s_waitcnt lgkmcnt(0)" ::: "memory");
            __builtin_amdgcn_sched_barrier(0);
#pragma unroll
            for (int j = 0; j < NT1; ++j) {
                const f16x8 bh = __builtin_bit_cast(f16x8, fx[j][0]), bl = __builtin_bit_cast(f16x8, fx[j][1]);
                PG_MFMA(al, bh, 0)
                PG_MFMA(ah, bl, 1)
                PG_MFMA(ah, bh, 2)
            }
#pragma unroll
            for (int j = NT1; j < TNW; ++j) {
                const f16x8 bh = __builtin_bit_cast(f16x8, fy[j - NT1][0]), bl = __builtin_bit_cast(f16x8, fy[j - NT1][1]);
                PG_MFMA(al, bh, 0)
                PG_MFMA(ah, bl, 1)
                PG_MFMA(ah, bh, 2)
            }
#undef PG_MFMA
        };

#pragma unroll
        for (int q2 = 0; q2 < AHEAD; ++q2) {
            const unsigned dstb = lds_base + (unsigned)q2 * STAGE;
#pragma unroll
            for (int i = 0; i < NPIECE; ++i) dma_piece(i, dstb);
            dma_advance();
            if (q2 == 0) {
                __builtin_amdgcn_sched_barrier(0);
                stage_inputs();
                __builtin_amdgcn_sched_barrier(0);
                PG_VMCNT(0);
            }
        }
        __builtin_amdgcn_s_barrier();
        PG_READ(fa0[0], lds_base + offAh, 0);
        PG_READ(fa0[1], lds_base + offAl, 0);
#pragma unroll
        for (int j = 0; j < TNW / 2; ++j) {
            PG_READ(fx[j][0], lds_base + offBh, j * 2048);
            PG_READ(fx[j][1], lds_base + offBl, j * 2048);
        }
        int s = 0;
        for (; s + 1 < nst - (NST - 1); s += 2) {
            stage(s, std::true_type{}, fa0, fa1);
            stage(s + 1, std::true_type{}, fa1, fa0);
        }
        for (; s < nst; s += 2) {
            stage(s, std::false_type{}, fa0, fa1);
            if (s + 1 < nst) stage(s + 1, std::false_type{}, fa1, fa0);
        }
    };
    auto run16 = [&](auto iss_t) __attribute__((always_inline)) {
        constexpr bool ISS = decltype(iss_t)::value;
        const int l15 = lane & 15, g = lane >> 4, cs = g & 1, uh = g >> 1, sw16 = (l15 >> 2) & 3;
        const int wn4 = w & 3, wm2 = w >> 2;
        const unsigned oAh = cs * STAGE + (wm2 * 64 + l15) * 64 + ((uh ^ sw16) << 4), oAl = cs * STAGE + (wm2 * 64 + l15) * 64 + (((2 + uh) ^ sw16) << 4);
        const unsigned oBh = cs * STAGE + A_ST + (wn4 * 112 + l15) * 64 + ((uh ^ sw16) << 4), oBl = cs * STAGE + A_ST + (wn4 * 112 + l15) * 64 + (((2 + uh) ^ sw16) << 4);
#pragma unroll
        for (int i = 0; i < 4; ++i)
#pragma unroll
            for (int j = 0; j < 7; ++j) c16[i][j] = f32x4{0.f, 0.f, 0.f, 0.f};
        u32x4 fb[7][2], fa[2][2];
        const int nv0 = (nc0 + 1) & ~1, nvt = nv0 + ((nc1 + 1) & ~1), npair = nvt >> 1;
        const int z0 = (nc0 & 1) ? nv0 - 1 : -1, z1 = (nc1 & 1) ? nvt - 1 : -1;
        const int wl = w & 3, st0 = wl * 7;
        const unsigned voffW = lane * 16 + st0 * 1024, voffA = lane * 16 + 2 * wl * 1024;
        const char* ga = P.A0 + (size_t)rb128 * nc0 * GG::A_IMG + sub * 64;
        const char* gb = P.W.img + (size_t)nb * nst * GG::B_ST;
        const char* const ga1 = nc1 > 0 ? P.A1 + (size_t)rb128 * nc1 * GG::A_IMG + sub * 64 : nullptr;
        int ti = 0, tr = 0;
        auto piece = [&](int q) __attribute__((always_inline)) {
            if (ti == z0 || ti == z1) return;
            const unsigned dstb = lds_base + (unsigned)(ti % NST) * STAGE;
            const unsigned m0w = dstb + A_ST + st0 * 1024;
            const int pw = q - 2;
            const unsigned hop = (unsigned)(pw >> 2) * 4096;
            if (q < 2) PG_DMA(dstb + 2 * wl * 1024, voffA, ga, q * 1024);
            else PG_DMA(m0w + hop, voffW + hop, gb, (pw & 3) * 1024);
        };
        auto advance = [&]() __attribute__((always_inline)) {
            if (ti != z0 && ti != z1) {
                ++tr;
                gb += GG::B_ST;
                ga = (tr == nc0) ? ga1 : ga + GG::A_IMG;
            }
            ++ti;
        };
        auto stage = [&](int p, auto steady_t) __attribute__((always_inline)) {
            constexpr bool STEADY = decltype(steady_t)::value;
            const unsigned zm = ((2 * p + 1 == z0 || 2 * p + 1 == z1) && cs) ? 0u : ~0u;
            const unsigned sb = lds_base + (unsigned)(p & 1) * 2 * STAGE, sbn = lds_base + (unsigned)((p + 1) & 1) * 2 * STAGE;
            const bool has_next = STEADY || p + 1 < npair;
            if (2 * p == nv0 && nc1 > 0) {
#pragma unroll
                for (int i = 0; i < 4; ++i) {
                    const float f = s_fac[wm2 * 64 + 16 * i + l15];
#pragma unroll
                    for (int j = 0; j < 7; ++j) c16[i][j] *= f;
                }
                __builtin_amdgcn_sched_barrier(0);
            }
            auto gap = [&](int m) __attribute__((always_inline)) {
                const int pass = m / 21, gi = m % 21;
                if (pass < 3) {
                    if (gi == 0) PG_READ(fa[(pass + 1) & 1][0], sb + oAh, (pass + 1) * 1024);
                    if (gi == 1) PG_READ(fa[(pass + 1) & 1][1], sb + oAl, (pass + 1) * 1024);
                } else if (has_next) {
                    if (gi == 0) PG_READ(fa[0][0], sbn + oAh, 0);
                    if (gi == 1) PG_READ(fa[0][1], sbn + oAl, 0);
                    if (gi >= 1 && gi <= 7) PG_READ(fb[gi - 1][1], sbn + oBl, (gi - 1) * 1024);
                    if (gi >= 15 && gi <= 20) PG_READ(fb[gi - 15][0], sbn + oBh, (gi - 15) * 1024);
                    if (gi == 20) PG_READ(fb[6][0], sbn + oBh, 6 * 1024);
                }
                if (ISS) {
                    if (pass == 3 && gi >= 8 && gi <= 14) {
                        if (STEADY || ti < nvt) piece(gi - 8);
                    }
                    if (pass == 0 && gi % 3 == 2) {
                        const int q = 7 + gi / 3;
                        if (STEADY || ti < nvt) {
                            piece(q < 9 ? q : q - 9);
                            if (q == 8) advance();
                        }
                    }
                    if (pass == 1 && gi % 3 == 2 && gi <= 11) {
                        const int q = 14 + gi / 3;
                        if (STEADY || ti < nvt) {
                            piece(q - 9);
                            if (q == 17) advance();
                        }
                    }
                }
                if (pass == 2 && gi == 17) {
                    if (ISS && has_next) PG_VMCNT(0);
                    __builtin_amdgcn_s_barrier();
                }
            };
#define PG_MFMA16(X, Y, m)                                                              \
    c16[i][j] = __builtin_amdgcn_mfma_f32_16x16x32_f16(Y, X, c16[i][j], 0, 0, 0);       \
    __builtin_amdgcn_sched_barrier(0);                                                  \
    gap(m);                                                                             \
    __builtin_amdgcn_sched_barrier(0);
#pragma unroll
            for (int i = 0; i < 4; ++i) {
                if (i == 0) asm volatile("s_waitcnt lgkmcnt(7)" ::: "memory");
                else asm volatile("s_waitcnt lgkmcnt(0)" ::: "memory");
                __builtin_amdgcn_sched_barrier(0);
                const u32x4 a_h = fa[i & 1][0] & zm, a_l = fa[i & 1][1] & zm;
                const f16x8 ah = __builtin_bit_cast(f16x8, a_h), al = __builtin_bit_cast(f16x8, a_l);
#pragma unroll
                for (int j = 0; j < 7; ++j) { PG_MFMA16(ah, __builtin_bit_cast(f16x8, fb[j][1]), 21 * i + j) }
                if (i == 0) { asm volatile("s_waitcnt lgkmcnt(2)" ::: "memory"); __builtin_amdgcn_sched_barrier(0); }
#pragma unroll
                for (int j = 0; j < 7; ++j) { PG_MFMA16(al, __builtin_bit_cast(f16x8, fb[j][0]), 21 * i + 7 + j) }
#pragma unroll
                for (int j = 0; j < 7; ++j) { PG_MFMA16(ah, __builtin_bit_cast(f16x8, fb[j][0]), 21 * i + 14 + j) }
            }
#undef PG_MFMA16
        };
        if (ISS) {
#pragma unroll
            for (int q = 0; q < 9; ++q) piece(q);
            advance();
#pragma unroll
            for (int q = 0; q < 9; ++q) piece(q);
            advance();
            __builtin_amdgcn_sched_barrier(0);
            stage_inputs();
            __builtin_amdgcn_sched_barrier(0);
            PG_VMCNT(0);
#pragma unroll
            for (int q = 0; q < 7; ++q) piece(q);
        } else {
            stage_inputs();
        }
        __builtin_amdgcn_s_barrier();
        PG_READ(fa[0][0], lds_base + oAh, 0);
        PG_READ(fa[0][1], lds_base + oAl, 0);
#pragma unroll
        for (int j = 0; j < 7; ++j) PG_READ(fb[j][1], lds_base + oBl, j * 1024);
#pragma unroll
        for (int j = 0; j < 7; ++j) PG_READ(fb[j][0], lds_base + oBh, j * 1024);
        int p = 0;
        for (; p < npair - 2; ++p) stage(p, std::true_type{});
        for (; p < npair; ++p) stage(p, std::false_type{});
    };
    if constexpr (M16) {
        if (w < 4) run16(std::true_type{});
        else run16(std::false_type{});
    } else {
        if (wn == 0) run(std::integral_constant<int, 0>{});
        else run(std::integral_constant<int, 1>{});
    }
    if (G.dbg & 1) {
        float keep = 0.f;
        if constexpr (M16) {
#pragma unroll
            for (int i = 0; i < 4; ++i)
#pragma unroll
                for (int j = 0; j < 7; ++j) keep += c16[i][j][0] + c16[i][j][1] + c16[i][j][2] + c16[i][j][3];
        } else {
#pragma unroll
            for (int j = 0; j < TNW; ++j)
#pragma unroll
                for (int r = 0; r < 16; ++r) keep += acc[j][r];
        }
        if (keep == 123.456f && P.out) P.out[0] = keep;
        return;
    }
    __syncthreads();

    int keep = -1;
    if constexpr (KS_OK) {
        if (ksplit) {
            keep = khalf;
            const int give = 1 - khalf;
            int* const s_bad = reinterpret_cast<int*>(s_sum);
            if (t == 0) *s_bad = 0;
            float* const xsend = P.xk_buf + ((((size_t)rb * 2 + give) * 4 + w) * TNW * 2) * 256 + lane * 4;
            const float* const xrecv = P.xk_buf + ((((size_t)rb * 2 + khalf) * 4 + w) * TNW * 2) * 256 + lane * 4;
#pragma unroll
            for (int j = 0; j < TNW; ++j)
#pragma unroll
                for (int q2 = 0; q2 < 2; ++q2) {
                    const f32x4 x = {acc[j][8 * give + 4 * q2], acc[j][8 * give + 4 * q2 + 1], acc[j][8 * give + 4 * q2 + 2], acc[j][8 * give + 4 * q2 + 3]};
                    asm volatile("global_store_dwordx4 %0, %1, off sc0 sc1\n\ts_nop 1" ::"v"(xsend + (j * 2 + q2) * 256), "v"(x) : "memory");
                }
            asm volatile("s_waitcnt vmcnt(0)" ::: "memory");
            __syncthreads();
            unsigned* const fl = P.xk_flags + (size_t)rb * 2;
            if (t == 0) __hip_atomic_store(fl + khalf, P.xk_epoch, __ATOMIC_RELAXED, __HIP_MEMORY_SCOPE_AGENT);
            if (w == 0) {
                unsigned spins = 0;
                while (__hip_atomic_load(fl + give, __ATOMIC_RELAXED, __HIP_MEMORY_SCOPE_AGENT) != P.xk_epoch) {
                    __builtin_amdgcn_s_sleep(1);
                    if (++spins > (1u << 22)) {
                        if (lane == 0) { *s_bad = 1; if (P.xk_status) atomicOr(P.xk_status, 2u); }
                        break;
                    }
                }
            }
            __syncthreads();
            const bool bad = *s_bad != 0;
            f32x4 y[TNW][2];
#pragma unroll
            for (int j = 0; j < TNW; ++j)
#pragma unroll
                for (int q2 = 0; q2 < 2; ++q2)
                    asm volatile("global_load_dwordx4 %0, %1, off sc1" : "=&v"(y[j][q2]) : "v"(xrecv + (j * 2 + q2) * 256) : "memory");
            asm volatile("s_waitcnt vmcnt(0)" ::: "memory");
            __builtin_amdgcn_sched_barrier(0);
            const float poison = bad ? __uint_as_float(0x7fc00000u) : 0.f;
#pragma unroll
            for (int j = 0; j < TNW; ++j)
#pragma unroll
                for (int q2 = 0; q2 < 2; ++q2)
#pragma unroll
                    for (int e = 0; e < 4; ++e) acc[j][8 * khalf + 4 * q2 + e] += y[j][q2][e] + poison;
            __syncthreads();
            if (G.dbg & 64) {
                float kp = 0.f;
#pragma unroll
                for (int j = 0; j < TNW; ++j)
#pragma unroll
                    for (int r = 0; r < 16; ++r) kp += acc[j][r];
                if (kp == 123.456f && P.out) P.out[0] = kp;
                return;
            }
        }
    }
    auto skip = [&](int rr) __attribute__((always_inline)) { return KS_OK && keep >= 0 && rr != keep; };

    const int lr = M16 ? (lane & 15) : (lane >> 2), q = M16 ? (lane >> 4) : (lane & 3);
    constexpr int NR = M16 ? 4 : 2, NIE = M16 ? 7 : NI, EPS = M16 ? 112 : EP_S;
    const int wcol0 = M16 ? (w & 3) * 112 : wn * BNW, wrow0 = M16 ? (w >> 2) * 64 : wm * 32, wcw = M16 ? (w & 3) : wn;
    const int lrow = lr;
    float* const ep = reinterpret_cast<float*>(lds) + w * (16 * EPS);
    float cv[M16 ? 1 : TNW];
    if constexpr (!M16) {
#pragma unroll
        for (int j = 0; j < TNW; ++j) cv[j] = s_cinv[wn * BNW + l31 + 32 * j];
    }
    auto transpose_round = [&](int rr, float4 (&dst)[NIE]) __attribute__((always_inline)) {
        if constexpr (M16) {
            const float rinv = s_rinv[wrow0 + 16 * rr + lrow];
#pragma unroll
            for (int i = 0; i < NIE; ++i) {
                const float4 c4 = *reinterpret_cast<const float4*>(s_cinv + wcol0 + 16 * i + 4 * q);
                const f32x4 a = c16[rr][i];
                dst[i] = make_float4(a[0] * c4.x * rinv, a[1] * c4.y * rinv, a[2] * c4.z * rinv, a[3] * c4.w * rinv);
            }
            return;
        } else {
#pragma unroll
            for (int j = 0; j < TNW; ++j)
#pragma unroll
                for (int r8 = 0; r8 < 8; ++r8) {
                    const int r = 8 * rr + r8;
                    ep[((r & 3) + 8 * ((r >> 2) & 1) + 4 * h) * EPS + 32 * j + l31] = acc[j][r] * cv[j];
                }
        }
        wave_fence();
        const float rinv = s_rinv[wrow0 + 16 * rr + lrow];
#pragma unroll
        for (int i = 0; i < NIE; ++i) {
            float4 x = *reinterpret_cast<const float4*>(ep + lr * EPS + 16 * i + 4 * q);
            x.x *= rinv; x.y *= rinv; x.z *= rinv; x.w *= rinv;
            dst[i] = x;
        }
        wave_fence();
    };
    const int colw = wcol0 + 4 * q;
    auto add_bias = [&](float4 (&dst)[NIE]) __attribute__((always_inline)) {
        if (has_bias) {
#pragma unroll
            for (int i = 0; i < NIE; ++i) {
                const float4 b4 = *reinterpret_cast<const float4*>(s_bias + colw + 16 * i);
                dst[i].x += b4.x; dst[i].y += b4.y; dst[i].z += b4.z; dst[i].w += b4.w;
            }
        }
    };
    int grow[NR];
#pragma unroll
    for (int rr = 0; rr < NR; ++rr) grow[rr] = rb * BM + wrow0 + 16 * rr + lrow;
    constexpr int mode = MODE;

    float4 v[NR][NIE];
    auto row_sum4 = [&](float s) __attribute__((always_inline)) {
        if constexpr (M16) {
            typedef unsigned u32x2 __attribute__((ext_vector_type(2)));
            const unsigned u = __float_as_uint(s);
            const u32x2 a = __builtin_amdgcn_permlane16_swap(u, u, false, false);
            const float t2 = __uint_as_float(a.x) + __uint_as_float(a.y);
            const unsigned w2 = __float_as_uint(t2);
            const u32x2 b = __builtin_amdgcn_permlane32_swap(w2, w2, false, false);
            return __uint_as_float(b.x) + __uint_as_float(b.y);
        } else {
            s += dpp_xor1f(s);
            s += dpp_xor2f(s);
            return s;
        }
    };
    if (mode != PG_LN) {
        const int halfC = P.rot_C >> 1, rpad = P.rot_piece_pad, rlen = P.rot_piece_len;
        const unsigned rmagic = rpad > 0 ? ((1u << 20) + rpad - 1) / rpad : 0u;
        const float scale = P.scale;
#define PG_TABLE_INDEX(i)                                                                                                   \
    int col = min(colw + 16 * (i), C - 4);                                                                                  \
    if (rpad > 0) { const int hq = (int)(((unsigned)col * rmagic) >> 20); col = hq * rlen + min(col - hq * rpad, rlen - 4); } \
    if (col >= P.rot_C) col %= P.rot_C;                     \
    const int ridx = col >> 1;
#define PG_LOAD_TABLES(rr, tb)                                                                                              \
    {                                                                                                                       \
    if (P.csT) {                                          \
        const float* pp = P.csT + (size_t)min(grow[rr], rows - 1) * halfC * 2;                                              \
        _Pragma("unroll") for (int i = 0; i < NIE; ++i) {                                                                   \
            PG_TABLE_INDEX(i)                                                                                               \
            const float4 cs = *reinterpret_cast<const float4*>(pp + 2 * ridx);                                              \
            tb[i] = make_float4(cs.x, cs.z, cs.y, cs.w);                                                                    \
        }                                                                                                                   \
    } else {                                                                                                                \
        const float* cp = P.cosT + (size_t)min(grow[rr], rows - 1) * halfC;                                                 \
        const float* sp = P.sinT + (size_t)min(grow[rr], rows - 1) * halfC;                                                 \
        _Pragma("unroll") for (int i = 0; i < NIE; ++i) {                                                                   \
            PG_TABLE_INDEX(i)                                                                                               \
            const float2 c = *reinterpret_cast<const float2*>(cp + ridx), sn = *reinterpret_cast<const float2*>(sp + ridx); \
            tb[i] = make_float4(c.x, c.y, sn.x, sn.y);                                                                      \
        }                                                                                                                   \
    }                                                                                                                       \
    }
        auto finish_round = [&](int rr, const float4 (&tb)[NIE]) __attribute__((always_inline)) {
            add_bias(v[rr]);
#pragma unroll
            for (int i = 0; i < NIE; ++i) {
                float4 x = v[rr][i];
                if (rot) {
                    const float x0 = x.x, x1 = x.y, x2 = x.z, x3 = x.w;
                    x.x = __fadd_rn(__fmul_rn(x0, tb[i].x), __fmul_rn(-x1, tb[i].z));
                    x.y = __fadd_rn(__fmul_rn(x1, tb[i].x), __fmul_rn(x0, tb[i].z));
                    x.z = __fadd_rn(__fmul_rn(x2, tb[i].y), __fmul_rn(-x3, tb[i].w));
                    x.w = __fadd_rn(__fmul_rn(x3, tb[i].y), __fmul_rn(x2, tb[i].w));
                }
                x.x *= scale; x.y *= scale; x.z *= scale; x.w *= scale;
                if (mode == PG_PLANES && P.relu) { x.x = fmaxf(x.x, 0.f); x.y = fmaxf(x.y, 0.f); x.z = fmaxf(x.z, 0.f); x.w = fmaxf(x.w, 0.f); }
                v[rr][i] = x;
            }
        };
        if constexpr (!M16) {
#pragma unroll
            for (int rr = 0; rr < NR; ++rr) {
                float4 tb[NIE];
                if (rot && !(G.dbg & 32)) PG_LOAD_TABLES(rr, tb)
                transpose_round(rr, v[rr]);
                finish_round(rr, tb);
                __builtin_amdgcn_sched_barrier(0);
            }
        } else {
            float4 tb0[NIE], tb1[NIE];
            if (rot && !(G.dbg & 32)) { PG_LOAD_TABLES(0, tb0) PG_LOAD_TABLES(1, tb1) }
            transpose_round(0, v[0]);
            transpose_round(1, v[1]);
            finish_round(0, tb0);
            __builtin_amdgcn_sched_barrier(0);
            if (rot && !(G.dbg & 32)) PG_LOAD_TABLES(2, tb0)
            finish_round(1, tb1);
            __builtin_amdgcn_sched_barrier(0);
            if (rot && !(G.dbg & 32)) PG_LOAD_TABLES(3, tb1)
            transpose_round(2, v[2]);
            transpose_round(3, v[3]);
            finish_round(2, tb0);
            finish_round(3, tb1);
            __builtin_amdgcn_sched_barrier(0);
        }
#undef PG_LOAD_TABLES
#undef PG_TABLE_INDEX
        if (mode == PG_F32) {
            float* __restrict__ outp = P.out + (size_t)nb * P.blk_stride;
#pragma unroll
            for (int rr = 0; rr < NR; ++rr) {
                if (grow[rr] >= rows) continue;
#pragma unroll
                for (int i = 0; i < NIE; ++i) {
                    const int col = colw + 16 * i;
                    if (wcol0 + 16 * i < C && !(G.dbg & 4)) *reinterpret_cast<float4*>(outp + (size_t)grow[rr] * P.ldo + col) = v[rr][i];
                }
            }
            return;
        }
        if (mode == PG_PLANES && P.out) {
            float* __restrict__ outp = P.out + (size_t)nb * P.blk_stride;
#pragma unroll
            for (int rr = 0; rr < NR; ++rr) {
                if (grow[rr] >= rows) continue;
#pragma unroll
                for (int i = 0; i < NIE; ++i) {
                    const int col = colw + 16 * i;
                    if (wcol0 + 16 * i < C && !(G.dbg & 4)) *reinterpret_cast<float4*>(outp + (size_t)grow[rr] * P.ldo + col) = v[rr][i];
                }
            }
        }
    } else {
#pragma unroll
        for (int rr = 0; rr < NR; ++rr) if (!skip(rr)) transpose_round(rr, v[rr]);
#pragma unroll
        for (int rr = 0; rr < NR; ++rr) if (!skip(rr)) add_bias(v[rr]);
    }

    if (mode == PG_LN) {
        const float* __restrict__ res = P.resid;
        constexpr int NRR = NR / 2;
        float4 r0[NRR][NIE];
        auto park = [&](int rr) __attribute__((always_inline)) { return ep + (rr - NRR) * (8 * 16 * EPS) + lr * EPS + 4 * q; };
        if (res && !(G.dbg & 16)) {
#pragma unroll
            for (int rr = NRR; rr < NR; ++rr) {
                if (skip(rr)) continue;
                const float* rp = res + (size_t)min(grow[rr], rows - 1) * P.ldr;
#pragma unroll
                for (int i = 0; i < NIE; ++i) {
                    const int col = colw + 16 * i;
                    const float4 x = wcol0 + 16 * i < C ? *reinterpret_cast<const float4*>(rp + col) : make_float4(0.f, 0.f, 0.f, 0.f);
                    *reinterpret_cast<float4*>(park(rr) + 16 * i) = x;
                }
            }
#pragma unroll
            for (int rr = 0; rr < NRR; ++rr) {
                if (skip(rr)) continue;
                const float* rp = res + (size_t)min(grow[rr], rows - 1) * P.ldr;
#pragma unroll
                for (int i = 0; i < NIE; ++i) {
                    const int col = colw + 16 * i;
                    r0[rr][i] = wcol0 + 16 * i < C ? *reinterpret_cast<const float4*>(rp + col) : make_float4(0.f, 0.f, 0.f, 0.f);
                }
            }
        }
        const bool postadd = res && P.ln_postadd;
        if (postadd) {
#pragma unroll
            for (int rr = 0; rr < NR; ++rr)
#pragma unroll
                for (int i = 0; i < NIE; ++i) {
                    if (skip(rr)) continue;
                    const float4 r4 = rr < NRR ? r0[rr < NRR ? rr : 0][i] : *reinterpret_cast<const float4*>(park(rr) + 16 * i);
                    v[rr][i].x += r4.x; v[rr][i].y += r4.y; v[rr][i].z += r4.z; v[rr][i].w += r4.w;
                }
        }
// ... 354 lines not shown
            unsigned spins = 0;
            while (__hip_atomic_load(fl + give, __ATOMIC_RELAXED, __HIP_MEMORY_SCOPE_AGENT) != P.xk_epoch) {
                __builtin_amdgcn_s_sleep(1);
                if (++spins > (1u << 22)) {
                    if (lane == 0) { *s_bad = 1; if (P.xk_status) atomicOr(P.xk_status, 2u); }
                    break;
                }
            }
        }
        __syncthreads();
        const float poison = *s_bad != 0 ? __uint_as_float(0x7fc00000u) : 0.f;
        auto recv = [&](auto KV) __attribute__((always_inline)) {
            constexpr int k0 = 2 * decltype(KV)::value;
            const float* const xr = xrecv;
            f32x4 y[NJ][2];
#pragma unroll
            for (int j = 0; j < NJ; ++j)
#pragma unroll
                for (int r2 = 0; r2 < 2; ++r2)
                    asm volatile("global_load_dwordx4 %0, %1, off sc1" : "=&v"(y[j][r2]) : "v"(xr + (j * 2 + r2) * 256) : "memory");
            asm volatile("s_waitcnt vmcnt(0)" ::: "memory");
            __builtin_amdgcn_sched_barrier(0);
#pragma unroll
            for (int j = 0; j < NJ; ++j)
#pragma unroll
                for (int r2 = 0; r2 < 2; ++r2) c16[k0 + r2][j] += y[j][r2] + poison;
        };
        if (khalf == 0) recv(std::integral_constant<int, 0>{}); else recv(std::integral_constant<int, 1>{});
        __syncthreads();
    }
    auto skip = [&](int rr) __attribute__((always_inline)) { return ksplit && (rr >> 1) != khalf; };

    const int lr = l15, q = g;
    constexpr int NR = 4, NIE = NJ;
    const int wloc = wn * 144, wcol0 = csub + wloc, wrow0 = wm2 * 64;
    const int colw = wcol0 + 4 * q;
    int grow[NR];
#pragma unroll
    for (int rr = 0; rr < NR; ++rr) grow[rr] = rb * BM + wrow0 + 16 * rr + lr;
    float4 v[NR][NIE];
    auto scale_round = [&](int rr, float4 (&dst)[NIE]) __attribute__((always_inline)) {
        const float rinv = s_rinv[wrow0 + 16 * rr + lr];
#pragma unroll
        for (int i = 0; i < NIE; ++i) {
            const float4 c4 = *reinterpret_cast<const float4*>(s_cinv + wloc + 16 * i + 4 * q);
            const f32x4 a = c16[rr][i];
            dst[i] = make_float4(a[0] * c4.x * rinv, a[1] * c4.y * rinv, a[2] * c4.z * rinv, a[3] * c4.w * rinv);
        }
    };
    const int halfC = P.rot_C >> 1, rpad = P.rot_piece_pad, rlen = P.rot_piece_len;
    const unsigned rmagic = rpad > 0 ? ((1u << 20) + rpad - 1) / rpad : 0u;
    const float scale = P.scale;
    auto load_tables = [&](int rr, float4 (&tb)[NIE]) __attribute__((always_inline)) {
#pragma unroll
        for (int i = 0; i < NIE; ++i) {
            int col = min(colw + 16 * i, C - 4);
            if (rpad > 0) { const int hq = (int)(((unsigned)col * rmagic) >> 20); col = hq * rlen + min(col - hq * rpad, rlen - 4); }
            if (col >= P.rot_C) col %= P.rot_C;
            const int ridx = col >> 1;
            if (P.csT) {
                const float4 cs4 = *reinterpret_cast<const float4*>(P.csT + (size_t)min(grow[rr], rows - 1) * halfC * 2 + 2 * ridx);
                tb[i] = make_float4(cs4.x, cs4.z, cs4.y, cs4.w);
            } else {
                const float2 c = *reinterpret_cast<const float2*>(P.cosT + (size_t)min(grow[rr], rows - 1) * halfC + ridx);
                const float2 sn = *reinterpret_cast<const float2*>(P.sinT + (size_t)min(grow[rr], rows - 1) * halfC + ridx);
                tb[i] = make_float4(c.x, c.y, sn.x, sn.y);
            }
        }
    };
    auto finish_round = [&](int rr, const float4 (&tb)[NIE]) __attribute__((always_inline)) {
#pragma unroll
        for (int i = 0; i < NIE; ++i) {
            float4 x = v[rr][i];
            if (has_bias) {
                const float4 b4 = *reinterpret_cast<const float4*>(s_bias + wloc + 4 * q + 16 * i);
                x.x += b4.x; x.y += b4.y; x.z += b4.z; x.w += b4.w;
            }
            if (rot) {
                const float x0 = x.x, x1 = x.y, x2 = x.z, x3 = x.w;
                x.x = __fadd_rn(__fmul_rn(x0, tb[i].x), __fmul_rn(-x1, tb[i].z));
                x.y = __fadd_rn(__fmul_rn(x1, tb[i].x), __fmul_rn(x0, tb[i].z));
                x.z = __fadd_rn(__fmul_rn(x2, tb[i].y), __fmul_rn(-x3, tb[i].w));
                x.w = __fadd_rn(__fmul_rn(x3, tb[i].y), __fmul_rn(x2, tb[i].w));
            }
            x.x *= scale; x.y *= scale; x.z *= scale; x.w *= scale;
            if (MODE == PG_PLANES && P.relu) { x.x = fmaxf(x.x, 0.f); x.y = fmaxf(x.y, 0.f); x.z = fmaxf(x.z, 0.f); x.w = fmaxf(x.w, 0.f); }
            v[rr][i] = x;
        }
    };
    if (ksplit) {
        float4 tb0[NIE], tb1[NIE];
        if (khalf == 0) {
            if (rot) { load_tables(0, tb0); load_tables(1, tb1); }
            scale_round(0, v[0]); scale_round(1, v[1]);
            finish_round(0, tb0); finish_round(1, tb1);
        } else {
            if (rot) { load_tables(2, tb0); load_tables(3, tb1); }
            scale_round(2, v[2]); scale_round(3, v[3]);
            finish_round(2, tb0); finish_round(3, tb1);
        }
        __builtin_amdgcn_sched_barrier(0);
    } else {
        float4 tb0[NIE], tb1[NIE];
        if (rot) { load_tables(0, tb0); load_tables(1, tb1); }
        scale_round(0, v[0]);
        scale_round(1, v[1]);
        finish_round(0, tb0);
        __builtin_amdgcn_sched_barrier(0);
        if (rot) load_tables(2, tb0);
        finish_round(1, tb1);
        __builtin_amdgcn_sched_barrier(0);
        if (rot) load_tables(3, tb1);
        scale_round(2, v[2]);
        scale_round(3, v[3]);
        finish_round(2, tb0);
        finish_round(3, tb1);
        __builtin_amdgcn_sched_barrier(0);
    }
    if (MODE == PG_F32 || P.out) {
        float* __restrict__ outp = P.out + (size_t)nb * P.blk_stride;
#pragma unroll
        for (int rr = 0; rr < NR; ++rr) {
            if (grow[rr] >= rows || skip(rr)) continue;
#pragma unroll
            for (int i = 0; i < NIE; ++i)
                if (wcol0 + 16 * i < C) *reinterpret_cast<float4*>(outp + (size_t)grow[rr] * P.ldo + colw + 16 * i) = v[rr][i];
        }
    }
    if (MODE == PG_F32 || !P.pimg) return;
#pragma unroll
    for (int rr = 0; rr < NR; ++rr) {
        if (skip(rr)) continue;
        const bool rok = grow[rr] < rows;
        const float bound = s_bound[wrow0 + 16 * rr + lr];
        if (P.pbnd && rok && (nb == 0 || per_blk) && wcol0 == 0 && q == 0) P.pbnd[(size_t)nb * P.pbnd_blk_stride + grow[rr]] = bound;
        const float sc = pow2i(scale_exp(bound));
        const int rl = wrow0 + 16 * rr + lr, swz = (rl >> 2) & 3;
        char* const rowp = P.pimg + (size_t)nb * P.pimg_blk_stride +
                           (((size_t)rb * P.p_nct + P.p_kc0 + (per_blk ? 0 : nb * (C >> 4)) + (wcol0 >> 4)) * 128 + rl) * 64;
        const unsigned uhi = (unsigned)(((q >> 1) ^ swz) << 4), ulo = (unsigned)(((2 + (q >> 1)) ^ swz) << 4);
        const bool odd = q & 1;
#pragma unroll
        for (int i = 0; i < NIE; ++i) {
            if (wcol0 + 16 * i >= C) continue;
            unsigned h0, l0, h1, l1;
            split2(v[rr][i].x * sc, v[rr][i].y * sc, h0, l0);
            split2(v[rr][i].z * sc, v[rr][i].w * sc, h1, l1);
            typedef unsigned u32x2 __attribute__((ext_vector_type(2)));
            const u32x2 e0 = __builtin_amdgcn_permlane16_swap(h0, l0, false, false), e1 = __builtin_amdgcn_permlane16_swap(h1, l1, false, false);
            const u32x4 U = {e0.x, e1.x, e0.y, e1.y};
            if (rok) __builtin_nontemporal_store(U, reinterpret_cast<u32x4*>(rowp + (size_t)i * 8192 + (odd ? ulo : uhi)));
        }
    }
}

__device__ __forceinline__ int pg_src_row(int c, int C, int olen, int opad, int rows_src) {
    if (c >= C) return -1;
    const int r = (c / opad) * olen + c % opad;
    return (c % opad < olen && r < rows_src) ? r : -1;
}
__global__ __launch_bounds__(256) void pg_wscale_kernel(const float* __restrict__ W, int nblk, int C, int K, int BN, float* __restrict__ cinv,
                                                        float* __restrict__ wnorm, int olen, int opad, int rows_src) {
    const int idx = blockIdx.x * 4 + (threadIdx.x >> 6), lane = threadIdx.x & 63;
    if (idx >= nblk * BN) return;
    const int nb = idx / BN, c = idx % BN;
    const int sr = pg_src_row(c, C, olen, opad, rows_src);
    if (sr < 0) { if (lane == 0) cinv[idx] = 1.f; return; }
    const float* wr = W + (size_t)(nb * rows_src + sr) * K;
    float mx = 0.f, l1 = 0.f;
    for (int k = lane; k < K; k += 64) { const float a = fabsf(wr[k]); mx = fmaxf(mx, a); l1 += a; }
    mx = wave_max(mx);
    l1 = wave_sum(l1);
    if (lane == 0) {
        cinv[idx] = pow2i(-scale_exp(mx));
        if (l1 == l1) atomicMax(reinterpret_cast<unsigned*>(wnorm + nb), __float_as_uint(l1 * 1.0001f));
        else wnorm[nb] = l1;
    }
}
__global__ __launch_bounds__(256) void pg_pack_kernel(const float* __restrict__ W, int nblk, int C, int K, int BN, int nct, int piece_len,
                                                      int piece_pad, const float* __restrict__ cinv, char* __restrict__ img, int olen, int opad,
                                                      int rows_src) {
    const size_t n = (size_t)nblk * nct * BN * 2, idx = (size_t)blockIdx.x * blockDim.x + threadIdx.x;
    if (idx >= n) return;
    const int half = (int)(idx & 1);
    size_t rest = idx >> 1;
    const int c = (int)(rest % BN); rest /= BN;
    const int kc = (int)(rest % nct), nb = (int)(rest / nct);
    const int sr = c < BN ? pg_src_row(c, C, olen, opad, rows_src) : -1;
    const float sc = sr >= 0 ? 1.0f / cinv[nb * BN + c] : 0.f;
    float x[8];
#pragma unroll
    for (int e = 0; e < 8; ++e) {
        const int kp = kc * 16 + half * 8 + e, piece = kp / piece_pad, off = kp % piece_pad, k = piece * piece_len + off;
        x[e] = (sr >= 0 && off < piece_len && k < K) ? W[(size_t)(nb * rows_src + sr) * K + k] * sc : 0.f;
    }
    uint4 hi, lo;
    split2(x[0], x[1], hi.x, lo.x); split2(x[2], x[3], hi.y, lo.y); split2(x[4], x[5], hi.z, lo.z); split2(x[6], x[7], hi.w, lo.w);
    char* d = img + (((size_t)nb * nct + kc) * BN + c) * 64;
    const int swz = (c >> 2) & 3;
    *reinterpret_cast<uint4*>(d + ((half ^ swz) << 4)) = hi;
    *reinterpret_cast<uint4*>(d + (((2 + half) ^ swz) << 4)) = lo;
}

__global__ __launch_bounds__(256) void pg_pack16w_kernel(const float* __restrict__ W, int nblk, int C, int K, int nct, int piece_len, int piece_pad,
                                                         const float* __restrict__ cinv, char* __restrict__ img, int olen, int opad, int rows_src) {
    constexpr int SB = PgGeomW::BN, LBN = PgGeomW::LBN;
    const size_t n = (size_t)nblk * 2 * nct * SB * 2, idx = (size_t)blockIdx.x * blockDim.x + threadIdx.x;
    if (idx >= n) return;
    const int half = (int)(idx & 1);
    size_t rest = idx >> 1;
    const int c = (int)(rest % SB); rest /= SB;
    const int kc = (int)(rest % nct), pb = (int)(rest / nct), nb = pb >> 1, cl = (pb & 1) * SB + c;
    const int sr = pg_src_row(cl, C, olen, opad, rows_src);
    const float sc = sr >= 0 ? 1.0f / cinv[nb * LBN + cl] : 0.f;
    float x[8];
#pragma unroll
    for (int e = 0; e < 8; ++e) {
        const int kp = kc * 16 + half * 8 + e, piece = kp / piece_pad, off = kp % piece_pad, k = piece * piece_len + off;
        x[e] = (sr >= 0 && off < piece_len && k < K) ? W[(size_t)(nb * rows_src + sr) * K + k] * sc : 0.f;
    }
    uint4 hi, lo;
    split2(x[0], x[1], hi.x, lo.x); split2(x[2], x[3], hi.y, lo.y); split2(x[4], x[5], hi.z, lo.z); split2(x[6], x[7], hi.w, lo.w);
    char* d = img + (((size_t)pb * nct + kc) * SB + c) * 64;
    const int swz = (c >> 2) & 3;
    *reinterpret_cast<uint4*>(d + ((half ^ swz) << 4)) = hi;
    *reinterpret_cast<uint4*>(d + (((2 + half) ^ swz) << 4)) = lo;
}

__global__ __launch_bounds__(256) void planes_from_f32_kernel(const float* __restrict__ x, int ldx, int rows, int K, char* __restrict__ img,
                                                              float* __restrict__ bnd, const float* __restrict__ bnd_in) {
    const int row = blockIdx.x * 4 + (threadIdx.x >> 6), lane = threadIdx.x & 63;
    if (row >= rows) return;
    const int ng = K >> 3, nct = K >> 4;
    float4 v[2][2];
    float mx = 0.f;
#pragma unroll
    for (int g = 0; g < 2; ++g) {
        const int gi = lane + 64 * g;
        if (gi < ng) {
            v[g][0] = *reinterpret_cast<const float4*>(x + (size_t)row * ldx + 8 * gi);
            v[g][1] = *reinterpret_cast<const float4*>(x + (size_t)row * ldx + 8 * gi + 4);
            mx = fmaxf(mx, fmaxf(fmaxf(fabsf(v[g][0].x), fabsf(v[g][0].y)), fmaxf(fabsf(v[g][0].z), fabsf(v[g][0].w))));
            mx = fmaxf(mx, fmaxf(fmaxf(fabsf(v[g][1].x), fabsf(v[g][1].y)), fmaxf(fabsf(v[g][1].z), fabsf(v[g][1].w))));
        }
    }
    mx = wave_max(mx);
    if (bnd_in) mx = bnd_in[row];
    if (lane == 0) bnd[row] = mx;
    const float sc = pow2i(scale_exp(mx));
    const int rb = row >> 7, r = row & 127, swz = (r >> 2) & 3;
#pragma unroll
    for (int g = 0; g < 2; ++g) {
        const int gi = lane + 64 * g;
        if (gi < ng) {
            uint4 hi, lo;
            split2(v[g][0].x * sc, v[g][0].y * sc, hi.x, lo.x); split2(v[g][0].z * sc, v[g][0].w * sc, hi.y, lo.y);
            split2(v[g][1].x * sc, v[g][1].y * sc, hi.z, lo.z); split2(v[g][1].z * sc, v[g][1].w * sc, hi.w, lo.w);
            char* d = img + (((size_t)rb * nct + (gi >> 1)) * 128 + r) * 64;
            *reinterpret_cast<uint4*>(d + (((gi & 1) ^ swz) << 4)) = hi;
            *reinterpret_cast<uint4*>(d + (((2 + (gi & 1)) ^ swz) << 4)) = lo;
        }
    }
}
__global__ __launch_bounds__(256) void planes_to_f32_kernel(const char* __restrict__ img, const float* __restrict__ bnd, int rows, int K,
                                                            float* __restrict__ out, int ldo) {
    const int row = blockIdx.x * 4 + (threadIdx.x >> 6), lane = threadIdx.x & 63;
    if (row >= rows) return;
    const int ng = K >> 3, nct = K >> 4, rb = row >> 7, r = row & 127, swz = (r >> 2) & 3;
    const float inv = pow2i(-scale_exp(bnd[row]));
    for (int gi = lane; gi < ng; gi += 64) {
        const char* d = img + (((size_t)rb * nct + (gi >> 1)) * 128 + r) * 64;
        const f16x8 hi = *reinterpret_cast<const f16x8*>(d + (((gi & 1) ^ swz) << 4));
        const f16x8 lo = *reinterpret_cast<const f16x8*>(d + (((2 + (gi & 1)) ^ swz) << 4));
#pragma unroll
        for (int e = 0; e < 8; ++e) out[(size_t)row * ldo + 8 * gi + e] = ((float)hi[e] + (float)lo[e]) * inv;
    }
}
__global__ __launch_bounds__(256) void ln_bound_kernel(const float* __restrict__ g, const float* __restrict__ b, int C, float* __restrict__ out) {
    __shared__ float sg[4], sb[4];
    float mg = 0.f, mb = 0.f;
    for (int c = threadIdx.x; c < C; c += 256) { mg = fmaxf(mg, fabsf(g[c])); mb = fmaxf(mb, fabsf(b[c])); }
    mg = wave_max(mg); mb = wave_max(mb);
    if ((threadIdx.x & 63) == 0) { sg[threadIdx.x >> 6] = mg; sb[threadIdx.x >> 6] = mb; }
    __syncthreads();
    if (threadIdx.x == 0) {
        mg = fmaxf(fmaxf(sg[0], sg[1]), fmaxf(sg[2], sg[3]));
        mb = fmaxf(fmaxf(sb[0], sb[1]), fmaxf(sb[2], sb[3]));
        out[0] = (sqrtf((float)C) * mg + mb) * 1.0001f;
    }
}

using G4 = PgGeom<4, 4>;
using G4H = PgGeom<4, 4, 2>;
using G7 = PgGeom<7, 4>;
using G9 = PgGeom<9, 3>;
using G7H = PgGeom<7, 4, 2>;
using G9H = PgGeom<9, 3, 2>;

}

bool pgemm_shape_ok(int C) { return C > 0 && C % 16 == 0 && C <= G9::BN; }
int pgemm_bn(int C) { return C <= G4::BN ? G4::BN : (C <= G7::BN ? G7::BN : G9::BN); }
static size_t pg_bst(int C) { return (size_t)pgemm_bn(C) * 64; }

template <int TNW, int NST, int MODE>
static int configure_mode() {
    if constexpr (TNW <= 7)
        DR_HIP_CHECK(hipFuncSetAttribute((const void*)pgemm_kernel<TNW, NST, MODE, 4>, hipFuncAttributeMaxDynamicSharedMemorySize, (int)PgGeom<TNW, NST, 4>::SMEM));
    if constexpr (TNW == 7) {
        DR_HIP_CHECK(hipFuncSetAttribute((const void*)pgemm_kernel<TNW, NST, MODE, 4, true>, hipFuncAttributeMaxDynamicSharedMemorySize, (int)PgGeom<TNW, NST, 4>::SMEM16));
    }
    DR_HIP_CHECK(hipFuncSetAttribute((const void*)pgemm_kernel<TNW, NST, MODE, 2>, hipFuncAttributeMaxDynamicSharedMemorySize, (int)PgGeom<TNW, NST, 2>::SMEM));
    return DR_OK;
}
int pgemm_configure() {
    int rc = configure_mode<4, 4, PG_F32>();
    if (rc == DR_OK) rc = configure_mode<4, 4, PG_PLANES>();
    if (rc == DR_OK) rc = configure_mode<4, 4, PG_LN>();
    if (rc == DR_OK) rc = configure_mode<7, 4, PG_F32>();
    if (rc == DR_OK) rc = configure_mode<7, 4, PG_PLANES>();
    if (rc == DR_OK) rc = configure_mode<7, 4, PG_LN>();
    if (rc == DR_OK) rc = configure_mode<9, 3, PG_F32>();
    if (rc == DR_OK) rc = configure_mode<9, 3, PG_PLANES>();
    if (rc == DR_OK) rc = configure_mode<9, 3, PG_LN>();
    if (rc == DR_OK) {
        DR_HIP_CHECK(hipFuncSetAttribute((const void*)pgemm16w_kernel<PG_F32>, hipFuncAttributeMaxDynamicSharedMemorySize, (int)PgGeomW::SMEM));
        DR_HIP_CHECK(hipFuncSetAttribute((const void*)pgemm16w_kernel<PG_PLANES>, hipFuncAttributeMaxDynamicSharedMemorySize, (int)PgGeomW::SMEM));
    }
    return rc;
}

template <int TNW, int NST, int WMN>
static void pg_launch(int mode, dim3 grid, hipStream_t st, const PgBatch& g) {
    using GG = PgGeom<TNW, NST, WMN>;
    if (mode == PG_F32) hipLaunchKernelGGL((pgemm_kernel<TNW, NST, PG_F32, WMN>), grid, dim3(GG::NTHR), GG::SMEM, st, g);
    else if (mode == PG_PLANES) hipLaunchKernelGGL((pgemm_kernel<TNW, NST, PG_PLANES, WMN>), grid, dim3(GG::NTHR), GG::SMEM, st, g);
    else hipLaunchKernelGGL((pgemm_kernel<TNW, NST, PG_LN, WMN>), grid, dim3(GG::NTHR), GG::SMEM, st, g);
}

static int launch_pgemm16w(const PgBatch& g, hipStream_t st) {
    int maxt = 0;
    double flops = 0;
    const int mode = g.p[0].mode;
    if (mode != PG_F32 && mode != PG_PLANES) return DR_ENOSUP;
    bool ksplit = env_knob("DR_PG_KSPLIT", 1) != 0 && env_knob("DR_PG_KSPLITW", 1) != 0;
    long tiles = 0;
    for (int i = 0; i < g.n; ++i) {
        const PgProblem& p = g.p[i];
        const long tl_ = (long)((p.rows + 127) / 128) * p.nblk * 2;
        ksplit = ksplit && p.xk_buf && p.xk_flags && tl_ <= p.xk_cap && (p.A1 ? (p.nc0 >= 5 && p.nc1 >= 5) : p.nc0 >= 12);
        tiles += tl_;
    }
    if (g.wg_as > 0) tiles = 2L * g.wg_as;
    ksplit = ksplit && 2 * tiles <= (long)device_cu_count();
    for (int i = 0; i < g.n; ++i) {
        const PgProblem& p = g.p[i];
        const int nst = p.nc0 + (p.A1 ? p.nc1 : 0);
        if (p.W.sub != 2 || !pgemm16w_shape_ok(p.C) || p.rows < 1 || p.nblk < 1 || p.nc0 < 5 || (p.A1 && p.nc1 < 5) || p.mode != mode) return DR_ENOSUP;
        if (p.W.nct != nst) return DR_EINVAL;
        const int tl = ((p.rows + 127) / 128 + 7) / 8 * 8 * p.nblk * 2 * (ksplit ? 2 : 1);
        maxt = tl > maxt ? tl : maxt;
        flops += 2.0 * p.rows * p.C * p.nblk * (p.k_alg > 0 ? (double)p.k_alg : 16.0 * p.W.nct);
    }
    ProfScope ps(PK_GEMM_SPLIT, flops, st);
    PgBatch gd = g;
    gd.dbg = env_knob("DR_PG_NOEPI", 0);
    for (int i = 0; i < g.n; ++i) gd.p[i].ksplit = ksplit ? 1 : 0;
    const dim3 grid(maxt, g.n);
    if (mode == PG_F32) hipLaunchKernelGGL((pgemm16w_kernel<PG_F32>), grid, dim3(PgGeomW::NTHR), PgGeomW::SMEM, st, gd);
    else hipLaunchKernelGGL((pgemm16w_kernel<PG_PLANES>), grid, dim3(PgGeomW::NTHR), PgGeomW::SMEM, st, gd);
    DR_LAUNCH_CHECK();
    return DR_OK;
}

int launch_pgemm(const PgBatch& g, hipStream_t st) {
    if (g.n < 1 || g.n > 3) return DR_EINVAL;
    if (g.p[0].W.sub == 2) return launch_pgemm16w(g, st);
    int maxt = 0;
    double flops = 0;
    const int bn = pgemm_bn(g.p[0].C), nst_min = bn == G9::BN ? G9::NST : G7::NST;
    const int half_env = env_knob("DR_PG_HALF", 1);
    const int n_cu = device_cu_count();
    long wg128 = 0;
    for (int i = 0; i < g.n; ++i) wg128 += (long)((g.p[i].rows + 127) / 128) * g.p[i].nblk;
    if (g.wg_as > 0) wg128 = g.wg_as;
    const bool half = bn == G9::BN || half_env == 2 || (half_env == 1 && wg128 * 100 < (long)n_cu * env_knob("DR_PG_HALF_PCT", 51));
    const int bm = half ? 64 : 128;
    bool ksplit = half && g.p[0].mode == PG_LN && env_knob("DR_PG_KSPLIT", 1) != 0;
    long wg64 = 0;
    for (int i = 0; i < g.n; ++i) {
        const PgProblem& p = g.p[i];
        const long rb64 = (p.rows + 63) / 64;
        ksplit = ksplit && p.xk_buf && p.xk_flags && p.nblk == 1 && !p.A1 && p.nc0 / 2 >= nst_min && rb64 <= p.xk_cap;
        wg64 += rb64;
    }
    ksplit = ksplit && 2 * wg64 <= (long)n_cu;
    for (int i = 0; i < g.n; ++i) {
        const PgProblem& p = g.p[i];
        if (!pgemm_shape_ok(p.C) || pgemm_bn(p.C) != bn || p.rows < 1 || p.nblk < 1 || p.nc0 < 1 || p.nc0 + (p.A1 ? p.nc1 : 0) < nst_min) return DR_ENOSUP;
        if (p.W.nct != p.nc0 + (p.A1 ? p.nc1 : 0)) return DR_EINVAL;
        const int tl = ((p.rows + bm - 1) / bm + 7) / 8 * 8 * (ksplit ? 2 : p.nblk);
        maxt = tl > maxt ? tl : maxt;
        flops += 2.0 * p.rows * p.C * p.nblk * (p.k_alg > 0 ? (double)p.k_alg : 16.0 * p.W.nct);
    }
    ProfScope ps(PK_GEMM_SPLIT, flops, st);
    const int mode = g.p[0].mode;
    for (int i = 1; i < g.n; ++i)
        if (g.p[i].mode != mode) return DR_EINVAL;
    const dim3 grid(maxt, g.n);
    PgBatch gd = g;
    gd.dbg = env_knob("DR_PG_NOEPI", 0);
    for (int i = 0; i < g.n; ++i) gd.p[i].ksplit = ksplit ? 1 : 0;
    if (bn == G9::BN) pg_launch<9, 3, 2>(mode, grid, st, gd);
    else if (bn == G4::BN) { if (half) pg_launch<4, 4, 2>(mode, grid, st, gd); else pg_launch<4, 4, 4>(mode, grid, st, gd); }
    else {
        bool m16 = env_knob("DR_PG_M16", 1) != 0;
        for (int i = 0; i < g.n; ++i) m16 = m16 && g.p[i].nc0 >= 5 && (!g.p[i].A1 || g.p[i].nc1 >= 5);
        if (half) pg_launch<7, 4, 2>(mode, grid, st, gd);
        else if (m16) {
            using GG = PgGeom<7, 4, 4>;
            if (mode == PG_F32) hipLaunchKernelGGL((pgemm_kernel<7, 4, PG_F32, 4, true>), grid, dim3(GG::NTHR), GG::SMEM16, st, gd);
            else if (mode == PG_PLANES) hipLaunchKernelGGL((pgemm_kernel<7, 4, PG_PLANES, 4, true>), grid, dim3(GG::NTHR), GG::SMEM16, st, gd);
            else hipLaunchKernelGGL((pgemm_kernel<7, 4, PG_LN, 4, true>), grid, dim3(GG::NTHR), GG::SMEM16, st, gd);
        } else pg_launch<7, 4, 4>(mode, grid, st, gd);
    }
    DR_LAUNCH_CHECK();
    return DR_OK;
}

size_t pgemm_weight_bytes(int C, int nblk, int nct) {
    size_t b = (size_t)nblk * nct * pg_bst(C);
    b += (size_t)nblk * pgemm_bn(C) * 4;
    b += (size_t)nblk * 4;
    return (b + 255) & ~(size_t)255;
}
void pgemm_weight_view(void* buf, int C, int nblk, int nct, PgW* v) {
    char* p = (char*)buf;
    v->img = p;
    v->cinv = reinterpret_cast<const float*>(p + (size_t)nblk * nct * pg_bst(C));
    v->wnorm = v->cinv + (size_t)nblk * pgemm_bn(C);
    v->nct = nct;
    v->sub = 0;
}

bool pgemm16w_shape_ok(int C) { return C > 0 && C % 16 == 0 && C <= PgGeomW::LBN; }
size_t pgemm16w_weight_bytes(int nblk, int nct) {
    size_t b = (size_t)nblk * 2 * nct * PgGeomW::B_ST + (size_t)nblk * PgGeomW::LBN * 4 + (size_t)nblk * 4;
    return (b + 255) & ~(size_t)255;
}
void pgemm16w_weight_view(void* buf, int nblk, int nct, PgW* v) {
    char* p = (char*)buf;
    v->img = p;
    v->cinv = reinterpret_cast<const float*>(p + (size_t)nblk * 2 * nct * PgGeomW::B_ST);
    v->wnorm = v->cinv + (size_t)nblk * PgGeomW::LBN;
    v->nct = nct;
    v->sub = 2;
}
int pgemm16w_pack_weights_block(const float* W, int C, int K, int piece_len, int piece_pad, const PgW& v, int nb, hipStream_t st, int out_len,
                                int out_pad) {
    const int olen = out_len > 0 ? out_len : C, opad = out_pad > 0 ? out_pad : C, rows_src = out_len > 0 ? C / opad * olen : C;
    if (!pgemm16w_shape_ok(C) || v.sub != 2 || piece_pad % 16 || piece_len > piece_pad || piece_len < 1) return DR_EINVAL;
    const int nct = (K + piece_len - 1) / piece_len * piece_pad / 16;
    if (nct != v.nct) return DR_EINVAL;
    constexpr int LBN = PgGeomW::LBN;
    float* cinv = (float*)v.cinv + (size_t)nb * LBN;
    float* wnorm = (float*)v.wnorm + nb;
    char* img = (char*)v.img + (size_t)nb * 2 * nct * PgGeomW::B_ST;
    DR_HIP_CHECK(hipMemsetAsync(wnorm, 0, 4, st));
    hipLaunchKernelGGL(pg_wscale_kernel, dim3((LBN + 3) / 4), dim3(256), 0, st, W, 1, C, K, LBN, cinv, wnorm, olen, opad, rows_src);
    DR_LAUNCH_CHECK();
    const size_t n = (size_t)2 * nct * PgGeomW::BN * 2;
    hipLaunchKernelGGL(pg_pack16w_kernel, dim3((unsigned)((n + 255) / 256)), dim3(256), 0, st, W, 1, C, K, nct, piece_len, piece_pad,
                       (const float*)cinv, img, olen, opad, rows_src);
    DR_LAUNCH_CHECK();
    return DR_OK;
}
int pgemm_pack_weights(const float* W, int nblk, int C, int K, int piece_len, int piece_pad, void* buf, hipStream_t st) {
    if (!pgemm_shape_ok(C) || piece_pad % 16 || piece_len > piece_pad || piece_len < 1) return DR_EINVAL;
    const int nct = (K + piece_len - 1) / piece_len * piece_pad / 16, BN = pgemm_bn(C);
    PgW v;
    pgemm_weight_view(buf, C, nblk, nct, &v);
    DR_HIP_CHECK(hipMemsetAsync((void*)v.wnorm, 0, (size_t)nblk * 4, st));
    hipLaunchKernelGGL(pg_wscale_kernel, dim3((nblk * BN + 3) / 4), dim3(256), 0, st, W, nblk, C, K, BN, (float*)v.cinv, (float*)v.wnorm, C, C, C);
    DR_LAUNCH_CHECK();
    const size_t n = (size_t)nblk * nct * BN * 2;
    hipLaunchKernelGGL(pg_pack_kernel, dim3((unsigned)((n + 255) / 256)), dim3(256), 0, st, W, nblk, C, K, BN, nct, piece_len, piece_pad,
                       v.cinv, (char*)v.img, C, C, C);
    DR_LAUNCH_CHECK();
    return DR_OK;
}

int pgemm_pack_weights_block(const float* W, int C, int K, int piece_len, int piece_pad, const PgW& v, int nb, hipStream_t st, int out_len,
                             int out_pad) {
    const int olen = out_len > 0 ? out_len : C, opad = out_pad > 0 ? out_pad : C, rows_src = out_len > 0 ? C / opad * olen : C;
    if (!pgemm_shape_ok(C) || piece_pad % 16 || piece_len > piece_pad || piece_len < 1) return DR_EINVAL;
    const int nct = (K + piece_len - 1) / piece_len * piece_pad / 16;
    if (nct != v.nct) return DR_EINVAL;
    const int BN = pgemm_bn(C);
    float* cinv = (float*)v.cinv + (size_t)nb * BN;
    float* wnorm = (float*)v.wnorm + nb;
    char* img = (char*)v.img + (size_t)nb * nct * pg_bst(C);
    DR_HIP_CHECK(hipMemsetAsync(wnorm, 0, 4, st));
    hipLaunchKernelGGL(pg_wscale_kernel, dim3((BN + 3) / 4), dim3(256), 0, st, W, 1, C, K, BN, cinv, wnorm, olen, opad, rows_src);
    DR_LAUNCH_CHECK();
    const size_t n = (size_t)nct * BN * 2;
    hipLaunchKernelGGL(pg_pack_kernel, dim3((unsigned)((n + 255) / 256)), dim3(256), 0, st, W, 1, C, K, BN, nct, piece_len, piece_pad,
                       (const float*)cinv, img, olen, opad, rows_src);
    DR_LAUNCH_CHECK();
    return DR_OK;
}

__global__ __launch_bounds__(256) void group_max_kernel(const float* __restrict__ bnd, int ngroups, int grp_rows, float* __restrict__ out) {
    const int g = blockIdx.x * 4 + (threadIdx.x >> 6), lane = threadIdx.x & 63;
    if (g >= ngroups) return;
    float m = 0.f;
    for (int r = lane; r < grp_rows; r += 64) m = fmaxf(m, bnd[(size_t)g * grp_rows + r]);
    m = wave_max(m);
    if (lane == 0) out[g] = m;
}
int launch_group_max(const float* bnd, int ngroups, int grp_rows, float* out, hipStream_t st) {
    if (ngroups < 1) return DR_OK;
    hipLaunchKernelGGL(group_max_kernel, dim3((ngroups + 3) / 4), dim3(256), 0, st, bnd, ngroups, grp_rows, out);
    DR_LAUNCH_CHECK();
    return DR_OK;
}

__global__ __launch_bounds__(256) void rot_images_kernel(RotImgArgs A) {
    const int t = threadIdx.x, row = blockIdx.x * 64 + (t >> 2), j = t & 3;
    const int kc = 2 * blockIdx.y + (j >> 1), hh = j & 1, col0 = kc * 16 + hh * 8;
    if (row >= A.rows || col0 >= A.C) return;
    const int halfC = A.rot_C >> 1, rpad = A.rot_piece_pad, rlen = A.rot_piece_len;
    float4 tb[2];
    if (A.rot_mask) {
        const float* pp = A.csT + (size_t)row * halfC * 2;
#pragma unroll
        for (int i = 0; i < 2; ++i) {
            int col = min(col0 + 4 * i, A.C - 4);
            if (rpad > 0) { const int hq = col / rpad; col = hq * rlen + min(col - hq * rpad, rlen - 4); }
            if (col >= A.rot_C) col %= A.rot_C;
            const float4 cs = *reinterpret_cast<const float4*>(pp + 2 * (col >> 1));
            tb[i] = make_float4(cs.x, cs.z, cs.y, cs.w);
        }
    }
    const float b0 = A.bnd0[row], scale = A.scale;
    const int rl = row & 127, swz = (rl >> 2) & 3;
    typedef unsigned u32x4v __attribute__((ext_vector_type(4)));
    for (int nb = 0; nb < A.nblk; ++nb) {
        const bool rot = (A.rot_mask >> nb) & 1;
        const float* xp = A.x + (size_t)row * A.ldx + (size_t)nb * A.x_blk + col0;
        float4 v[2] = {*reinterpret_cast<const float4*>(xp), *reinterpret_cast<const float4*>(xp + 4)};
#pragma unroll
        for (int i = 0; i < 2; ++i) {
            float4 x = v[i];
            if (rot) {
                const float x0 = x.x, x1 = x.y, x2 = x.z, x3 = x.w;
                x.x = __builtin_fmaf(x0, tb[i].x, -(x1 * tb[i].z));
                x.z = __builtin_fmaf(x2, tb[i].y, -(x3 * tb[i].w));
                if (A.wide_form) {
                    x.y = __builtin_fmaf(x0, tb[i].z, x1 * tb[i].x);
                    x.w = __builtin_fmaf(x2, tb[i].w, x3 * tb[i].y);
                } else {
                    x.y = __builtin_fmaf(x1, tb[i].x, x0 * tb[i].z);
                    x.w = __builtin_fmaf(x3, tb[i].y, x2 * tb[i].w);
                }
            }
            x.x *= scale; x.y *= scale; x.z *= scale; x.w *= scale;
            v[i] = x;
        }
        const float bin = ((A.grp_mask >> nb) & 1) ? A.grp_bnd[A.grp_first + row / A.grp_rows] : fmaxf(b0, 0.f);
        const float bound = (bin * A.wnorm[nb] + 0.f) * (rot ? 1.41421366f : 1.f) * fabsf(scale);
        if (col0 == 0) A.pbnd[(size_t)nb * A.pbnd_blk_stride + row] = bound;
        const float sc = pow2i(scale_exp(bound));
        unsigned h0, l0, h1, l1, h2, l2, h3, l3;
        split2(v[0].x * sc, v[0].y * sc, h0, l0); split2(v[0].z * sc, v[0].w * sc, h1, l1);
        split2(v[1].x * sc, v[1].y * sc, h2, l2); split2(v[1].z * sc, v[1].w * sc, h3, l3);
        const u32x4v hi = {h0, h1, h2, h3}, lo = {l0, l1, l2, l3};
        char* const rowp = A.pimg + (size_t)nb * A.pimg_blk_stride + (((size_t)(row >> 7) * A.p_nct + kc) * 128 + rl) * 64;
        __builtin_nontemporal_store(hi, reinterpret_cast<u32x4v*>(rowp + ((hh ^ swz) << 4)));
        __builtin_nontemporal_store(lo, reinterpret_cast<u32x4v*>(rowp + (((2 + hh) ^ swz) << 4)));
    }
}
int launch_rot_images(const RotImgArgs& a, hipStream_t st) {
    if (a.rows < 1) return DR_OK;
    if (a.nblk < 1 || a.nblk > 3 || a.C < 16 || a.C % 16 || a.C / 16 > a.p_nct || a.ldx % 4 || a.x_blk % 4 || ((uintptr_t)a.x & 15) || !a.x || !a.bnd0 ||
        !a.wnorm || !a.pimg || !a.pbnd || ((uintptr_t)a.pimg & 15) || (a.grp_mask && (!a.grp_bnd || a.grp_rows < 1)))
        return DR_EINVAL;
    if (a.rot_mask && (!a.csT || ((uintptr_t)a.csT & 15) || a.rot_C % 4 || a.rot_piece_len % 4 || a.rot_piece_pad % 4)) return DR_EINVAL;
    ProfScope ps(PK_PE, (double)a.rows * (8.0 * a.nblk * a.C + (a.rot_mask ? 4.0 * a.rot_C : 0.0)), st);
    hipLaunchKernelGGL(rot_images_kernel, dim3((a.rows + 63) / 64, (a.C / 16 + 1) / 2), dim3(256), 0, st, a);
    DR_LAUNCH_CHECK();
    return DR_OK;
}

int launch_planes_from_f32(const float* x, int ldx, int rows, int K, char* img, float* bnd, hipStream_t st, const float* bnd_in) {
    if (K % 16 || K > 1024 || ldx % 4 || ((uintptr_t)x & 15)) return DR_ENOSUP;
    if (rows < 1) return DR_OK;
    hipLaunchKernelGGL(planes_from_f32_kernel, dim3((rows + 3) / 4), dim3(256), 0, st, x, ldx, rows, K, img, bnd, bnd_in);
    DR_LAUNCH_CHECK();
    return DR_OK;
}
int launch_planes_to_f32(const char* img, const float* bnd, int rows, int K, float* out, int ldo, hipStream_t st) {
    if (K % 16) return DR_ENOSUP;
    if (rows < 1) return DR_OK;
    hipLaunchKernelGGL(planes_to_f32_kernel, dim3((rows + 3) / 4), dim3(256), 0, st, img, bnd, rows, K, out, ldo);
    DR_LAUNCH_CHECK();
    return DR_OK;
}
__global__ __launch_bounds__(256) void absmax_blocks_kernel(const float* __restrict__ x, int n, float* __restrict__ out) {
    __shared__ float sm[4];
    const float* xb = x + (size_t)blockIdx.x * n;
    float m = 0.f;
    for (int c = threadIdx.x; c < n; c += 256) m = fmaxf(m, fabsf(xb[c]));
    m = wave_max(m);
    if ((threadIdx.x & 63) == 0) sm[threadIdx.x >> 6] = m;
    __syncthreads();
    if (threadIdx.x == 0) out[blockIdx.x] = fmaxf(fmaxf(sm[0], sm[1]), fmaxf(sm[2], sm[3])) * 1.0001f;
}
int launch_absmax_blocks(const float* x, int nblk, int n, float* out, hipStream_t st) {
    if (nblk < 1) return DR_OK;
    hipLaunchKernelGGL(absmax_blocks_kernel, dim3(nblk), dim3(256), 0, st, x, n, out);
    DR_LAUNCH_CHECK();
    return DR_OK;
}
int launch_ln_bound(const float* gamma, const float* beta, int C, float* out, hipStream_t st) {
    hipLaunchKernelGGL(ln_bound_kernel, dim3(1), dim3(256), 0, st, gamma, beta, C, out);
    DR_LAUNCH_CHECK();
    return DR_OK;
}

}

using namespace dr;

extern "C" {

size_t dr_plane_image_bytes(int rows, int K) { return (rows > 0 && K > 0 && K % 16 == 0) ? plane_image_bytes((size_t)rows, K) : 0; }

int dr_planes_from_f32(int rows, int K, const float* x, int ldx, void* image, float* bound, void* stream) {
    if (rows < 0 || K <= 0 || !x || !image || !bound || ldx < K) return DR_EINVAL;
    return launch_planes_from_f32(x, ldx, rows, K, (char*)image, bound, (hipStream_t)stream);
}

int dr_planes_from_f32_bounded(int rows, int K, const float* x, int ldx, const float* bound_in, void* image, float* bound, void* stream) {
    if (rows < 0 || K <= 0 || !x || !image || !bound || !bound_in || ldx < K) return DR_EINVAL;
    return launch_planes_from_f32(x, ldx, rows, K, (char*)image, bound, (hipStream_t)stream, bound_in);
}

static int attention_planes_entry(int P, int Lq, int Lk, int H, int d, const void* q_image, const float* q_bound, const void* k_image,
                                  const float* k_bound, const void* v_image, const float* v_bound, const uint8_t* q_mask, const uint8_t* k_mask,
                                  void* out_image, float* out_bound, int f16_single, void* stream) {
    if (P < 1 || Lq < 1 || Lk < 1 || H < 1 || d < 4 || d % 4 || !q_image || !k_image || !v_image || !q_bound || !k_bound || !v_bound || !out_image ||
        !out_bound) return DR_EINVAL;
    const int dp = (d + 15) / 16 * 16;
    AttnArgs a;
    memset(&a, 0, sizeof(a));
    a.H = H; a.d = d; a.qmask = q_mask; a.kmask = k_mask;
    a.nseg = P; a.q0 = 0; a.qstride = Lq; a.Lq = Lq; a.k0 = 0; a.kstride = Lk; a.Lk = Lk;
    a.scale = 1.0f / sqrtf((float)d);
    a.pimg[0] = a.pimg[1] = (char*)out_image; a.p_split = 0x7fffffff; a.p_nct = H * dp / 16; a.p_dp = dp; a.pbnd = out_bound;
    a.qimg[0] = a.qimg[1] = (const char*)q_image; a.kimg[0] = a.kimg[1] = (const char*)k_image; a.vimg[0] = a.vimg[1] = (const char*)v_image;
    a.qbnd = q_bound; a.kgb = k_bound; a.vgb = v_bound;
    a.f16_single = f16_single;
    return launch_attention(a, (hipStream_t)stream);
}

int dr_attention_planes(int P, int Lq, int Lk, int H, int d, const void* q_image, const float* q_bound, const void* k_image,
                        const float* k_bound, const void* v_image, const float* v_bound, const uint8_t* q_mask, const uint8_t* k_mask,
                        void* out_image, float* out_bound, void* stream) {
    return attention_planes_entry(P, Lq, Lk, H, d, q_image, q_bound, k_image, k_bound, v_image, v_bound, q_mask, k_mask, out_image, out_bound, 0, stream);
}
int dr_attention_planes_f16(int P, int Lq, int Lk, int H, int d, const void* q_image, const float* q_bound, const void* k_image,
                            const float* k_bound, const void* v_image, const float* v_bound, const uint8_t* q_mask, const uint8_t* k_mask,
                            void* out_image, float* out_bound, void* stream) {
    return attention_planes_entry(P, Lq, Lk, H, d, q_image, q_bound, k_image, k_bound, v_image, v_bound, q_mask, k_mask, out_image, out_bound, 1, stream);
}

int dr_planes_to_f32(int rows, int K, const void* image, const float* bound, float* out, int ldo, void* stream) {
    if (rows < 0 || K <= 0 || !out || !image || !bound || ldo < K) return DR_EINVAL;
    return launch_planes_to_f32((const char*)image, bound, rows, K, out, ldo, (hipStream_t)stream);
}

static int plane_nct(int K, int piece_len, int piece_pad) { return (K + piece_len - 1) / piece_len * piece_pad / 16; }

size_t dr_plane_weight_bytes(int nblk, int C, int K, int piece_len, int piece_pad) {
    if (nblk < 1 || !pgemm_shape_ok(C) || K < 1 || piece_len < 1 || piece_pad < piece_len || piece_pad % 16) return 0;
    return pgemm_weight_bytes(C, nblk, plane_nct(K, piece_len, piece_pad));
}

int dr_pack_weight_planes_f32(int nblk, int C, int K, int piece_len, int piece_pad, const float* W, void* packed, void* stream) {
    if (nblk < 1 || K < 1 || !W || !packed || ((uintptr_t)packed & 15)) return DR_EINVAL;
    return pgemm_pack_weights(W, nblk, C, K, piece_len, piece_pad, packed, (hipStream_t)stream);
}

size_t dr_plane_weight_bytes_wide(int nblk, int C, int K, int piece_len, int piece_pad) {
    if (nblk < 1 || !pgemm16w_shape_ok(C) || K < 1 || piece_len < 1 || piece_pad < piece_len || piece_pad % 16) return 0;
    return pgemm16w_weight_bytes(nblk, plane_nct(K, piece_len, piece_pad));
}

int dr_pack_weight_planes_wide_f32(int nblk, int C, int K, int piece_len, int piece_pad, const float* W, void* packed, void* stream) {
    if (nblk < 1 || K < 1 || !W || !packed || ((uintptr_t)packed & 15) || !pgemm16w_shape_ok(C) || piece_len < 1 || piece_pad < piece_len || piece_pad % 16)
        return DR_EINVAL;
    PgW v;
    pgemm16w_weight_view(packed, nblk, plane_nct(K, piece_len, piece_pad), &v);
    for (int nb = 0; nb < nblk; ++nb) {
        const int rc = pgemm16w_pack_weights_block(W + (size_t)nb * C * K, C, K, piece_len, piece_pad, v, nb, (hipStream_t)stream);
        if (rc) return rc;
    }
    return DR_OK;
}

int dr_ln_bound_f32(int C, const float* gamma, const float* beta, float* out, void* stream) {
    if (C < 1 || !gamma || !beta || !out) return DR_EINVAL;
    return launch_ln_bound(gamma, beta, C, out, (hipStream_t)stream);
}

int dr_bias_max_f32(int nblk, int n, const float* bias, float* out, void* stream) {
    if (nblk < 1 || n < 1 || !bias || !out) return DR_EINVAL;
    return launch_absmax_blocks(bias, nblk, n, out, (hipStream_t)stream);
}

// ... 78 lines not shown
```

diff-reg_amd/diffreg_hip/lib.py:

```python
import ctypes
import os

import torch

_HERE = os.path.dirname(os.path.abspath(__file__))
LIB_PATH = os.path.join(_HERE, "libdiffreg_hip.so")

if not os.path.exists(LIB_PATH):
    raise ImportError("libdiffreg_hip.so is missing (%s): run `python __graft_entry__.py build` or "
                      "`make -C diff-reg_amd/csrc`" % LIB_PATH)

_lib = ctypes.CDLL(LIB_PATH)

c_int, c_size_t, c_void_p, c_char_p, c_double, c_float = (ctypes.c_int, ctypes.c_size_t, ctypes.c_void_p,
                                                          ctypes.c_char_p, ctypes.c_double, ctypes.c_float)

SIGNATURES = {
    "dr_version": (c_int, []),
    "dr_strerror": (c_char_p, [c_int]),
    "dr_last_hip_error": (c_char_p, []),
    "dr_sinkhorn_workspace_bytes": (c_size_t, [c_int, c_int, c_int, c_int, c_int]),
    "dr_sinkhorn_f32": (c_int, [c_int, c_int, c_int, c_void_p, c_void_p, c_void_p, c_void_p, c_int, c_int,
                                c_void_p, c_void_p, c_size_t, c_void_p]),
    "dr_sinkhorn_f16": (c_int, [c_int, c_int, c_int, c_void_p, c_void_p, c_void_p, c_void_p, c_int, c_int, c_void_p, c_void_p]),
    "dr_sinkhorn_f64": (c_int, [c_int, c_int, c_int, c_void_p, c_void_p, c_void_p, c_void_p, c_int, c_int,
                                c_void_p, c_void_p, c_size_t, c_void_p]),
}


class LayerWeights(ctypes.Structure):
    _fields_ = [(n, c_void_p) for n in ("q_proj", "k_proj", "v_proj", "merge", "mlp0", "mlp2", "norm1_w", "norm1_b",
                                        "norm2_w", "norm2_b")]


class LoopConfig(ctypes.Structure):
    _fields_ = [("variant", c_int), ("C", c_int), ("H", c_int), ("n_layers", c_int), ("steps", c_int),
                ("sk_iters", c_int), ("voxel", c_float), ("origin", c_float * 3), ("sample_rate", c_float),
                ("max_condition_num", c_float), ("flags", c_int), ("h_alphas_cumprod", c_void_p),
                ("h_times", c_void_p)]


class LoopWeights(ctypes.Structure):
    _fields_ = [("layers", ctypes.POINTER(LayerWeights)), ("src_proj", c_void_p), ("bin_score", c_void_p),
                ("pe_freq", c_void_p), ("prepacked", c_void_p)]


class FusionLayerWeights(ctypes.Structure):
    _fields_ = [(n, c_void_p) for n in ("q_w", "q_b", "k_w", "k_b", "v_w", "v_b", "lin_w", "lin_b", "norm1_w", "norm1_b",
                                        "expand_w", "expand_b", "squeeze_w", "squeeze_b", "norm2_w", "norm2_b")]


class FusionWeights(ctypes.Structure):
    _fields_ = [("layers", ctypes.POINTER(FusionLayerWeights))] + \
               [(n, c_void_p) for n in ("img_emb_w", "img_emb_b", "pcd_emb_w", "pcd_emb_b", "img_in_w", "img_in_b", "dino_w",
                                        "dino_b", "all_w", "all_b", "pcd_in_w", "pcd_in_b", "out_w", "out_b", "src_proj",
                                        "bin_score", "prepacked")]


class CircleLossParams(ctypes.Structure):
    _fields_ = [(n, c_float) for n in ("pos_margin", "neg_margin", "pos_optimal", "neg_optimal", "log_scale", "pos_overlap", "neg_overlap")]


class FineLossParams(ctypes.Structure):
    _fields_ = [(n, c_float) for n in ("pos_radius_3d", "neg_radius_3d", "pos_radius_2d", "neg_radius_2d", "pos_margin", "neg_margin", "pos_optimal",
                                       "neg_optimal", "log_scale")]


class PlanesLinear(ctypes.Structure):
    _fields_ = [("rows", c_int), ("C", c_int), ("nblk", c_int),
                ("a0", c_void_p), ("bound0", c_void_p), ("k0", c_int),
                ("a1", c_void_p), ("bound1", c_void_p), ("k1", c_int),
                ("packed", c_void_p), ("mode", c_int),
                ("out", c_void_p), ("ldo", c_int), ("blk_stride", c_int),
                ("cos_t", c_void_p), ("sin_t", c_void_p), ("rot_mask", c_int), ("rot_C", c_int), ("scale", c_float),
                ("out_image", c_void_p), ("out_image_k", c_int), ("out_k0", c_int), ("out_bound", c_void_p),
                ("relu", c_int),
                ("gamma", c_void_p), ("beta", c_void_p), ("resid", c_void_p), ("ldr", c_int), ("bound_resid", c_void_p),
                ("ln_bound", c_void_p), ("bias", c_void_p), ("bias_max", c_void_p), ("ln_postadd", c_int), ("weight_layout", c_int),
                ("split_workspace", c_void_p), ("split_workspace_bytes", c_size_t)]


class Loop2D3DConfig(ctypes.Structure):
    _fields_ = [("C", c_int), ("H", c_int), ("n_layers", c_int), ("img_dim", c_int), ("dino_dim", c_int), ("pcd_dim", c_int),
                ("steps", c_int), ("sk_iters", c_int), ("sample_rate", c_float), ("max_condition_num", c_float),
                ("flags", c_int), ("h_alphas_cumprod", c_void_p), ("h_times", c_void_p)]


class LoopTrace(ctypes.Structure):
    _fields_ = [("x0", c_void_p), ("R_forwd", c_void_p), ("t_forwd", c_void_p), ("cond", c_void_p), ("feats_nopos", c_void_p),
                ("feats_pos", c_void_p), ("force_x", c_void_p), ("force_R", c_void_p), ("force_t", c_void_p), ("x_next", c_void_p),
                ("topk_idx", c_void_p), ("wconf", c_void_p)]


class DebugGemmProblem(ctypes.Structure):
    _fields_ = [(n, c_void_p) for n in ("A", "A2", "W", "out", "cos_t", "sin_t", "bias", "addend")] + \
               [(n, c_int) for n in ("rows", "ncols", "K", "K1", "lda", "lda2", "ldo", "epilogue", "rot_C")] + \
               [("scale", c_float), ("nbatch", c_int)] + [(n, ctypes.c_longlong) for n in ("stride_a", "stride_w", "stride_o")]


_P = ctypes.POINTER
SIGNATURES.update({
    "dr_init": (c_int, []),
    "dr_prof_enable": (None, [c_int]),
    "dr_prof_collect": (c_int, [c_void_p, c_void_p, c_void_p]),
    "dr_vol_pe_f32": (c_int, [c_int, c_int, c_int, c_void_p, c_void_p, c_void_p, c_float, c_float, c_float, c_float,
                              c_void_p, c_void_p, c_void_p, c_void_p]),
    "dr_linear_f32": (c_int, [c_int, c_int, c_int, c_void_p, c_void_p, c_void_p, c_int, c_void_p, c_void_p, c_int,
                              c_float, c_void_p]),
    "dr_plane_image_bytes": (c_size_t, [c_int, c_int]),
    "dr_planes_from_f32": (c_int, [c_int, c_int, c_void_p, c_int, c_void_p, c_void_p, c_void_p]),
    "dr_planes_from_f32_bounded": (c_int, [c_int, c_int, c_void_p, c_int, c_void_p, c_void_p, c_void_p, c_void_p]),
    "dr_attention_planes": (c_int, [c_int] * 5 + [c_void_p] * 10 + [c_void_p]),
    "dr_attention_planes_f16": (c_int, [c_int] * 5 + [c_void_p] * 10 + [c_void_p]),
    "dr_planes_to_f32": (c_int, [c_int, c_int, c_void_p, c_void_p, c_void_p, c_int, c_void_p]),
    "dr_plane_weight_bytes": (c_size_t, [c_int, c_int, c_int, c_int, c_int]),
    "dr_pack_weight_planes_f32": (c_int, [c_int, c_int, c_int, c_int, c_int, c_void_p, c_void_p, c_void_p]),
    "dr_plane_weight_bytes_wide": (c_size_t, [c_int, c_int, c_int, c_int, c_int]),
    "dr_plane_split_workspace_bytes": (c_size_t, [c_int]),
    "dr_plane_split_status": (c_int, [c_void_p, c_void_p, c_int]),
    "dr_pack_weight_planes_wide_f32": (c_int, [c_int, c_int, c_int, c_int, c_int, c_void_p, c_void_p, c_void_p]),
    "dr_ln_bound_f32": (c_int, [c_int, c_void_p, c_void_p, c_void_p, c_void_p]),
    "dr_linear_planes_f32": (c_int, [ctypes.POINTER(PlanesLinear), c_void_p]),
    "dr_bias_max_f32": (c_int, [c_int, c_int, c_void_p, c_void_p, c_void_p]),
    "dr_rotary_planes_f32": (c_int, [c_int, c_int, c_int, c_void_p, c_int, c_int, c_void_p, c_int, c_int, c_float, c_void_p, c_void_p, c_int, c_int,
                                     c_void_p, ctypes.c_longlong, c_void_p, ctypes.c_longlong, c_void_p]),
    "dr_loop2d3d_prepack_bytes": (c_size_t, [ctypes.POINTER(Loop2D3DConfig)]),
    "dr_loop2d3d_prepack": (c_int, [ctypes.POINTER(Loop2D3DConfig), ctypes.POINTER(FusionWeights), c_void_p, c_size_t, c_void_p]),
    "dr_gemm_nt_batched_f32": (c_int, [c_int, c_int, c_int, c_int, c_void_p, ctypes.c_longlong, c_void_p, ctypes.c_longlong, c_void_p, ctypes.c_longlong,
                                       c_float, c_void_p]),
    "dr_linear_ex_f32": (c_int, [c_int, c_int, c_int, c_void_p, c_int, c_void_p, c_void_p, c_void_p, c_int, c_int, c_float, c_void_p]),
    "dr_kpconv_gather_f32": (c_int, [c_int, c_int, c_int, c_int, c_int, c_void_p, c_void_p, c_void_p, c_void_p, c_void_p, c_float,
                                     c_void_p, c_int, c_void_p]),
    "dr_kpconv_gather_mode_f32": (c_int, [c_int, c_int, c_int, c_int, c_int, c_void_p, c_void_p, c_void_p, c_void_p, c_void_p, c_float,
                                          c_int, c_int, c_void_p, c_int, c_void_p]),
    "dr_kpconv_gather_backward_mode_f32": (c_int, [c_int, c_int, c_int, c_int, c_int, c_void_p, c_void_p, c_void_p, c_void_p, c_void_p, c_float,
                                                   c_int, c_int, c_void_p, c_int, c_void_p, c_void_p]),
    "dr_col_stats_workspace_bytes": (c_size_t, [c_int, c_int]),
    "dr_col_stats_f32": (c_int, [c_int, c_int, c_void_p, c_int, c_void_p, c_void_p, c_void_p, c_size_t, c_void_p]),
    "dr_norm_apply_f32": (c_int, [c_int, c_int, c_void_p, c_int, c_void_p, c_void_p, c_void_p, c_int, c_void_p, c_void_p, c_float,
                                  c_int, c_void_p, c_int, c_void_p]),
    "dr_gather_pool_f32": (c_int, [c_int, c_int, c_int, c_int, c_void_p, c_int, c_void_p, c_int, c_void_p, c_void_p]),
    "dr_kpconv_gather_backward_f32": (c_int, [c_int, c_int, c_int, c_int, c_int, c_void_p, c_void_p, c_void_p, c_void_p, c_void_p, c_float,
                                              c_void_p, c_int, c_void_p, c_void_p]),
    "dr_norm_backward_workspace_bytes": (c_size_t, [c_int, c_int]),
    "dr_norm_backward_f32": (c_int, [c_int, c_int, c_void_p, c_int, c_void_p, c_int, c_void_p, c_int, c_void_p, c_void_p, c_void_p, c_int, c_void_p,
                                     c_void_p, c_float, c_int, c_void_p, c_int, c_void_p, c_int, c_void_p, c_size_t, c_void_p]),
    "dr_gather_pool_backward_f32": (c_int, [c_int, c_int, c_int, c_int, c_void_p, c_int, c_void_p, c_int, c_void_p, c_void_p, c_void_p]),
    "dr_attention_layer_workspace_bytes": (c_size_t, [c_int, c_int, c_int, c_int]),
    "dr_attention_layer_f32": (c_int, [_P(LayerWeights), c_int, c_int, c_int, c_int, c_int] + [c_void_p] * 9 +
                               [c_void_p, c_size_t, c_void_p]),
    "dr_attention_layer_pe_f32": (c_int, [_P(LayerWeights), c_int, c_int, c_int, c_int, c_int] + [c_void_p] * 11 +
                                  [c_void_p, c_size_t, c_void_p]),
    "dr_attention_layer_train_saved_bytes": (c_size_t, [c_int, c_int, c_int, c_int]),
    "dr_attention_layer_train_forward_f32": (c_int, [_P(LayerWeights), c_int, c_int, c_int, c_int, c_int] + [c_void_p] * 10 + [c_size_t, c_void_p]),
    "dr_attention_layer_backward_workspace_bytes": (c_size_t, [c_int, c_int, c_int, c_int, c_int]),
    "dr_attention_layer_backward_f32": (c_int, [_P(LayerWeights), c_int, c_int, c_int, c_int, c_int] + [c_void_p] * 12 + [_P(LayerWeights), c_void_p, c_size_t, c_void_p]),
    "dr_procrustes_workspace_bytes": (c_size_t, [c_int, c_int, c_int]),
    "dr_procrustes_f32": (c_int, [c_int, c_int, c_int] + [c_void_p] * 5 + [c_int, c_float, c_float] + [c_void_p] * 7 + [c_void_p, c_size_t, c_void_p]),
    "dr_device_status": (c_int, [c_void_p, c_int]),
    "dr_denoise_loop_status": (c_int, [c_void_p, c_void_p, c_int]),
    "dr_procrustes_backward_f32": (c_int, [c_int, c_int, c_int, c_int] + [c_void_p] * 9),
    "dr_debug_sinkhorn_spin_limit": (None, [ctypes.c_uint]),
    "dr_debug_enable_env": (None, [c_int]),
    "dr_debug_launch_chain": (c_int, [c_int, c_int, c_int, c_void_p]),
    "dr_debug_gemm_config": (None, [c_int]),
    "dr_debug_gemm_f32": (c_int, [_P(DebugGemmProblem), c_int, c_void_p]),
    "dr_debug_attention_config": (None, [c_int]),
    "dr_debug_attention_split": (None, [c_int]),
    "dr_debug_attention_last_form": (c_int, []),
    "dr_debug_procrustes_last_form": (c_int, []),
    "dr_pnp_ransac_workspace_bytes": (c_size_t, [c_int, c_int]),
    "dr_pnp_ransac_f64": (c_int, [c_int, c_void_p, c_void_p, c_int, c_void_p, c_int, c_double, ctypes.c_uint64, c_void_p, c_void_p, c_void_p, c_void_p, c_size_t,
                                  c_void_p]),
    "dr_patch_similarity_f32": (c_int, [c_int, c_int, c_int, c_int, c_void_p, c_void_p, c_void_p, c_void_p, ctypes.c_longlong, c_void_p, c_void_p]),
    "dr_unique_pairs_workspace_bytes": (c_size_t, [c_int]),
    "dr_unique_pairs_i64": (c_int, [c_int, c_void_p, c_void_p, ctypes.c_longlong, c_void_p, c_void_p, c_void_p, c_size_t, c_void_p]),
    "dr_corr_gather_f32": (c_int, [c_int, c_void_p, c_void_p, ctypes.c_longlong, c_int] + [c_void_p] * 14),
    "dr_point_to_node_partition_workspace_bytes": (c_size_t, [c_int]),
    "dr_point_to_node_partition_f32": (c_int, [c_int, c_int, c_int] + [c_void_p] * 9 + [c_size_t, c_void_p]),
    "dr_patchify_f32": (c_int, [c_int] * 5 + [c_void_p] * 14),
    "dr_node_correspondences_2d3d_workspace_bytes": (c_size_t, [c_int, c_int, c_int, ctypes.c_longlong]),
    "dr_node_correspondences_2d3d_f32": (c_int, [c_int] * 4 + [c_void_p] * 11 + [c_float, c_float, ctypes.c_longlong] + [c_void_p] * 9 + [c_size_t, c_void_p]),
    "dr_mutual_nn_radius_workspace_bytes": (c_size_t, [c_int, c_int]),
    "dr_mutual_nn_radius_f32": (c_int, [c_int, c_int, c_void_p, c_void_p, c_float, c_void_p, c_void_p, c_void_p, c_void_p, c_size_t, c_void_p]),
    "dr_radius_pairs_workspace_bytes": (c_size_t, [c_int, c_int]),
    "dr_radius_pairs_f32": (c_int, [c_int, c_int, c_void_p, c_void_p, c_void_p, c_float, ctypes.c_longlong, c_void_p, c_void_p, c_void_p, c_void_p, c_size_t,
                                    c_void_p]),
    "dr_group_norm_workspace_bytes": (c_size_t, [c_int, c_int]),
    "dr_group_norm_stats_f32": (c_int, [c_int, c_int, c_int, c_void_p, c_int, c_float, c_void_p, c_void_p, c_void_p, c_size_t, c_void_p]),
    "dr_group_norm_apply_f32": (c_int, [c_int, c_int, c_int, c_void_p, c_int] + [c_void_p] * 4 + [c_void_p, c_int] + [c_void_p] * 4 +
                                [c_float, c_int, c_void_p, c_int, c_void_p]),
    "dr_group_norm_backward_workspace_bytes": (c_size_t, [c_int, c_int, c_int]),
    "dr_group_norm_backward_f32": (c_int, [c_int, c_int, c_int, c_void_p, c_int, c_void_p, c_int, c_void_p, c_int] + [c_void_p] * 3 +
                                   [c_void_p, c_int] + [c_void_p] * 3 + [c_float, c_int, c_void_p, c_int, c_void_p, c_void_p, c_void_p, c_int,
                                                                          c_void_p, c_void_p, c_void_p, c_size_t, c_void_p]),
    "dr_knn_interpolate_f32": (c_int, [c_int] * 4 + [c_void_p] * 5 + [c_int, c_void_p]),
    "dr_knn_interpolate_backward_f32": (c_int, [c_int] * 4 + [c_void_p] * 4 + [c_int, c_void_p, c_void_p]),
    "dr_kpconv_neighbor_count_f32": (c_int, [c_int] * 4 + [c_void_p] * 4),
    "dr_train_workspace_bytes": (c_size_t, [c_int, c_int, c_int]),
    "dr_match_matrix_f32": (c_int, [c_int, c_int, c_int, c_int, c_void_p, c_void_p, c_void_p]),
    "dr_gt_noising_f64": (c_int, [c_int, c_int, c_int, c_void_p, c_void_p, c_double, c_double, c_void_p, c_void_p, c_void_p]),
    "dr_focal_loss_f32": (c_int, [c_int, c_int, c_int, c_void_p, c_void_p, c_void_p, c_float, c_float, c_float, c_float, c_int, c_void_p, c_void_p,
                                  c_void_p]),
    "dr_match_recall_f32": (c_int, [c_int, c_int, c_int, c_void_p, c_int, c_void_p, c_void_p, c_void_p, c_void_p]),
    "dr_motion_l1_f32": (c_int, [c_int, c_int] + [c_void_p] * 10),
    "dr_motion_l1_backward_f32": (c_int, [c_int, c_int] + [c_void_p] * 11),
    "dr_layernorm_f32": (c_int, [c_int, c_int, c_void_p, c_void_p, c_void_p, c_float, c_void_p, c_void_p, c_void_p]),
    "dr_layernorm_backward_workspace_bytes": (c_size_t, [c_int]),
    "dr_layernorm_backward_f32": (c_int, [c_int, c_int] + [c_void_p] * 9),
    "dr_attention_f32": (c_int, [c_int] * 5 + [c_void_p] * 3 + [c_int, c_void_p, c_void_p, c_float, c_void_p, c_void_p]),
    "dr_attention_backward_workspace_bytes": (c_size_t, [c_int, c_int, c_int]),
    "dr_attention_backward_f32": (c_int, [c_int] * 5 + [c_void_p] * 5 + [c_int, c_void_p, c_void_p, c_float] + [c_void_p] * 3 + [c_void_p, c_size_t, c_void_p]),
    "dr_softmax_rows_f32": (c_int, [c_int, c_int, c_int, c_int, c_void_p, c_float, c_void_p, c_void_p, c_void_p, c_void_p]),
    "dr_dual_softmax_f32": (c_int, [c_int, c_int, c_int, c_void_p, c_float, c_void_p, c_void_p, c_void_p, c_void_p, c_void_p]),
    "dr_dual_softmax_backward_workspace_bytes": (c_size_t, [c_int, c_int, c_int]),
    "dr_dual_softmax_backward_f32": (c_int, [c_int, c_int, c_int, c_void_p, c_float, c_void_p, c_void_p, c_void_p, c_void_p, c_void_p, c_size_t, c_void_p]),
    "dr_softmax_backward_f32": (c_int, [c_int, c_int, c_void_p, c_void_p, c_float, c_void_p, c_void_p]),
    "dr_relu_backward_f32": (c_int, [ctypes.c_longlong, c_void_p, c_void_p, c_void_p, c_void_p]),
    "dr_rotary_f32": (c_int, [c_int, c_int, c_void_p, c_void_p, c_void_p, c_int, c_float, c_void_p, c_void_p]),
    "dr_focal_loss_backward_f32": (c_int, [c_int, c_int, c_int, c_void_p, c_void_p, c_float, c_float, c_float, c_float, c_void_p, c_void_p, c_void_p]),
    "dr_sinkhorn_backward_workspace_bytes": (c_size_t, [c_int, c_int, c_int, c_int]),
    "dr_sinkhorn_backward_f32": (c_int, [c_int, c_int, c_int, c_void_p, c_void_p, c_void_p, c_void_p, c_int, c_void_p, c_void_p, c_void_p, c_void_p,
                                         c_size_t, c_void_p]),
    "dr_scatter_rows_f32": (c_int, [c_int, c_int, c_void_p, ctypes.c_int64, c_void_p, c_void_p, c_void_p, ctypes.c_int64, c_void_p, c_void_p]),
    "dr_mutual_match_f64": (c_int, [c_int, c_int, c_int, c_void_p, c_double, c_int, c_int, c_void_p, c_void_p, c_void_p, c_void_p, c_void_p]),
    "dr_mutual_match_f32": (c_int, [c_int, c_int, c_int, c_void_p, c_float, c_int, c_int, c_void_p, c_void_p, c_void_p, c_void_p, c_void_p]),
    "dr_top1_union_workspace_bytes": (c_size_t, [c_int, c_int, c_int, c_int]),
    "dr_top1_union_f64": (c_int, [c_int, c_int, c_int, c_void_p, c_void_p, c_void_p, c_void_p, c_size_t, c_void_p]),
    "dr_top1_union_f32": (c_int, [c_int, c_int, c_int, c_void_p, c_void_p, c_void_p, c_void_p, c_size_t, c_void_p]),
    "dr_loop_prepack_bytes": (c_size_t, [_P(LoopConfig)]),
    "dr_loop_prepack": (c_int, [_P(LoopConfig), _P(LoopWeights), c_void_p, c_size_t, c_void_p]),
    "dr_denoise_loop_workspace_bytes": (c_size_t, [_P(LoopConfig), c_int, c_int, c_int]),
    "dr_denoise_loop": (c_int, [_P(LoopConfig), _P(LoopWeights), c_int, c_int, c_int] + [c_void_p] * 14 +
                        [_P(LoopTrace), c_void_p, c_size_t, c_void_p]),
    "dr_denoise_loop_2d3d_workspace_bytes": (c_size_t, [_P(Loop2D3DConfig), c_int, c_int, c_int]),
    "dr_denoise_loop_2d3d": (c_int, [_P(Loop2D3DConfig), _P(FusionWeights), c_int, c_int, c_int] + [c_void_p] * 16 +
                             [_P(LoopTrace), c_void_p, c_size_t, c_void_p]),
    "dr_inlier_ratio_f32": (c_int, [c_int] * 4 + [c_void_p] * 7 + [c_float, c_void_p, c_void_p, c_void_p]),
    "dr_nrfmr_f32": (c_int, [c_int] * 4 + [c_void_p] * 9 + [c_int, c_void_p, c_void_p, c_float, c_float] + [c_void_p] * 4),
    "dr_ransac_workspace_bytes": (c_size_t, [c_int, c_int, c_int]),
    "dr_ransac_corr_f64": (c_int, [c_int] * 4 + [c_void_p] * 4 + [c_double, c_int, ctypes.c_uint64] + [c_void_p] * 7 +
                           [c_size_t, c_void_p]),
    "dr_registration_recall_f64": (c_int, [c_int] + [c_void_p] * 5 + [c_double, c_void_p, c_void_p, c_void_p]),
    "dr_grid_subsample_workspace_bytes": (c_size_t, [c_int, c_int]),
    "dr_grid_subsample_f32": (c_int, [c_int, c_int, c_void_p, c_void_p, c_float] + [c_void_p] * 5 + [c_size_t, c_void_p]),
    "dr_radius_neighbors_workspace_bytes": (c_size_t, [c_int, c_int, c_int]),
    "dr_radius_neighbors_f32": (c_int, [c_int, c_int, c_int] + [c_void_p] * 4 + [c_float, c_int] + [c_void_p] * 4 + [c_size_t, c_void_p]),
    "dr_mutual_topk_workspace_bytes": (c_size_t, [c_int, c_int, c_int]),
    "dr_mutual_topk_select_f32": (c_int, [c_int, c_int, c_int, c_void_p, c_int, c_int, c_int, c_float, c_int] + [c_void_p] * 4 +
                                  [ctypes.c_longlong, c_void_p, c_void_p, c_size_t, c_void_p]),
    "dr_denoiser_match_f32": (c_int, [_P(LoopConfig), _P(LoopWeights), c_int, c_int, c_int] + [c_void_p] * 9 +
                              [c_void_p, c_size_t, c_void_p]),
    "dr_fusion_layer_train_saved_bytes": (c_size_t, [c_int, c_int, c_int, c_int]),
    "dr_fusion_layer_train_forward_f32": (c_int, [_P(FusionLayerWeights), c_int, c_int, c_int, c_int, c_int] + [c_void_p] * 5 + [c_size_t, c_void_p]),
    "dr_fusion_layer_backward_workspace_bytes": (c_size_t, [c_int, c_int, c_int, c_int, c_int]),
    "dr_fusion_layer_backward_f32": (c_int, [_P(FusionLayerWeights), c_int, c_int, c_int, c_int, c_int] + [c_void_p] * 7 +
                                     [_P(FusionLayerWeights), c_void_p, c_size_t, c_void_p]),
    "dr_l2_normalize_f32": (c_int, [c_int, c_int, c_void_p, c_float, c_void_p, c_void_p, c_void_p]),
    "dr_l2_normalize_backward_f32": (c_int, [c_int, c_int, c_void_p, c_void_p, c_float, c_void_p, c_void_p, c_void_p]),
    "dr_circle_loss_workspace_bytes": (c_size_t, [c_int, c_int, c_int]),
    "dr_circle_loss_f32": (c_int, [c_int, c_int, c_int, c_void_p, c_void_p, c_int] + [c_void_p] * 4 + [_P(CircleLossParams), c_void_p, c_void_p,
                                                                                                       c_size_t, c_void_p]),
    "dr_circle_loss_backward_f32": (c_int, [c_int, c_int, c_int, c_void_p, c_void_p, c_int] + [c_void_p] * 4 +
                                    [_P(CircleLossParams)] + [c_void_p] * 5 + [c_size_t, c_void_p]),
    "dr_fine_loss_saved_bytes": (c_size_t, [c_int]),
    "dr_fine_loss_f32": (c_int, [c_int] * 4 + [c_void_p] * 8 + [c_int, _P(FineLossParams), c_void_p, c_void_p, c_size_t, c_void_p]),
    "dr_fine_loss_backward_workspace_bytes": (c_size_t, [c_int, c_int]),
    "dr_fine_loss_backward_f32": (c_int, [c_int] * 4 + [c_void_p] * 8 + [c_int, _P(FineLossParams), c_void_p, c_size_t] + [c_void_p] * 4 +
                                  [c_size_t, c_void_p]),
    "dr_sparse_corr_eval_workspace_bytes": (c_size_t, [c_int, c_int]),
    "dr_sparse_corr_eval_i64": (c_int, [c_int, c_int, c_int, c_void_p, c_void_p, c_int, c_void_p, c_void_p, c_void_p, c_float, c_void_p, c_void_p,
                                        c_void_p, c_size_t, c_void_p]),
    "dr_corr_eval_workspace_bytes": (c_size_t, [c_int]),
    "dr_corr_eval_f32": (c_int, [c_int, c_void_p, c_void_p, c_void_p, c_double, c_int, c_void_p, c_int, c_void_p, c_void_p, c_void_p, c_size_t,
                                 c_void_p]),
    "dr_registration_eval_workspace_bytes": (c_size_t, [c_int]),
    "dr_registration_eval_f64": (c_int, [c_int, c_void_p, c_void_p, c_void_p, c_double, c_void_p, c_void_p, c_void_p, c_size_t, c_void_p]),
    "dr_back_project_f32": (c_int, [c_int, c_int, c_void_p, c_void_p, c_int, c_float, c_float, c_void_p, c_void_p, c_int, c_float, c_void_p, c_void_p,
                                    c_void_p, c_void_p]),
    "dr_render_f32": (c_int, [c_int, c_void_p, c_void_p, c_void_p, c_float, c_void_p, c_void_p, c_void_p]),
    "dr_resize_tokens_f32": (c_int, [c_int] * 5 + [c_void_p] * 3),
    "dr_resize_tokens_backward_f32": (c_int, [c_int] * 5 + [c_void_p] * 3),
    "dr_rows_normalize_chw_f32": (c_int, [c_int, ctypes.c_int64, c_void_p, c_void_p, c_void_p]),
    "dr_rows_normalize_chw_backward_f32": (c_int, [c_int, ctypes.c_int64, c_void_p, c_void_p, c_void_p, c_void_p]),
    "dr_rows_normalize_chw_backward_rows_f32": (c_int, [c_int, ctypes.c_int64, c_int, c_void_p, c_void_p, c_void_p, c_void_p, c_void_p]),
    "dr_conv2d_rows_f32": (c_int, [c_int] * 8 + [c_void_p, c_int, c_void_p, c_void_p, c_void_p, c_int, c_void_p, c_int, c_void_p]),
    "dr_resize_rows_f32": (c_int, [c_int] * 5 + [c_void_p, c_int, c_void_p, c_int, c_void_p, c_int, c_void_p]),
    "dr_conv2d_rows_backward_data_f32": (c_int, [c_int] * 8 + [c_void_p, c_int, c_void_p, c_void_p, c_int, c_void_p, c_int, c_void_p]),
    "dr_conv2d_rows_backward_weight_workspace_bytes": (c_size_t, [c_int] * 8),
    "dr_conv2d_rows_backward_weight_f32": (c_int, [c_int] * 8 + [c_void_p, c_int, c_void_p, c_int, c_void_p, c_void_p, c_void_p, c_size_t, c_void_p]),
    "dr_resize_rows_backward_f32": (c_int, [c_int] * 5 + [c_void_p, c_int, c_void_p, c_int, c_void_p]),
})


class GemmRowsF16Args(ctypes.Structure):
    _fields_ = [("a", c_void_p), ("w_packed", c_void_p), ("bias", c_void_p), ("gamma", c_void_p), ("addend", c_void_p), ("out", c_void_p),
                ("M", c_int), ("K", c_int), ("N", c_int), ("lda", c_int), ("ldo", c_int), ("ld_addend", c_int), ("mode", c_int),
                ("colscale_cols", c_int), ("colscale", c_float)]


class VitBlockF16(ctypes.Structure):
    _fields_ = [(n, c_void_p) for n in ("norm1_g", "norm1_b", "qkv_w", "qkv_b", "proj_w", "proj_b", "ls1", "norm2_g", "norm2_b", "fc1_w", "fc1_b",
                                        "fc2_w", "fc2_b", "ls2")]


class VitConfigF16(ctypes.Structure):
    _fields_ = [("H", c_int), ("W", c_int), ("p", c_int), ("D", c_int), ("heads", c_int), ("Dh", c_int), ("depth", c_int), ("eps", c_float),
                ("img", c_void_p), ("img_f32", c_int), ("patch_w", c_void_p), ("patch_b", c_void_p), ("cls", c_void_p), ("pos", c_void_p),
                ("blocks", ctypes.POINTER(VitBlockF16)), ("norm_g", c_void_p), ("norm_b", c_void_p), ("x_prenorm", c_void_p), ("x_norm", c_void_p),
                ("n_take", c_int), ("take", ctypes.POINTER(c_int)), ("take_out", ctypes.POINTER(c_void_p)), ("workspace", c_void_p),
                ("workspace_bytes", c_size_t)]


SIGNATURES.update({
    "dr_pack_weight_f16_bytes": (c_size_t, [c_int, c_int]),
    "dr_pack_weight_f16": (c_int, [c_int, c_int, c_void_p, c_int, c_void_p, c_void_p]),
    "dr_gemm_rows_f16": (c_int, [ctypes.POINTER(GemmRowsF16Args), c_void_p]),
    "dr_layernorm_rows_f16": (c_int, [c_int, c_int, c_void_p, c_int, c_void_p, c_void_p, c_float, c_int, c_void_p, c_int, c_void_p]),
    "dr_attention_rows_f16": (c_int, [c_int, c_int, c_int, c_void_p, c_int, c_void_p, c_int, c_void_p]),
    "dr_patch_rows_f16": (c_int, [c_int, c_int, c_int, c_void_p, c_int, c_void_p, c_int, c_void_p]),
    "dr_vit_workspace_bytes": (c_size_t, [c_int] * 5),
    "dr_vit_forward_f16": (c_int, [ctypes.POINTER(VitConfigF16), c_void_p]),
    "dr_debug_gemm_rows_tile": (None, [c_int]),
    "dr_conv2d_rows_act_f32": (c_int, [c_int] * 8 + [c_void_p, c_int, c_void_p, c_void_p, c_int, c_void_p, c_int, c_void_p, c_int, c_void_p, c_int,
                                       c_void_p]),
    "dr_conv_transpose2d_rows_f32": (c_int, [c_int] * 5 + [c_void_p, c_int, c_void_p, c_void_p, c_void_p, c_int, c_void_p]),
    "dr_conv2d_rows_project_f32": (c_int, [c_int] * 8 + [c_void_p, c_int, c_void_p, c_void_p, c_void_p, c_void_p, c_int, c_void_p, c_int, c_void_p]),
})


class GemmRowsF32Args(ctypes.Structure):
    _fields_ = [("a", c_void_p), ("w", c_void_p), ("bias", c_void_p), ("gamma", c_void_p), ("addend", c_void_p), ("out", c_void_p),
                ("M", c_int), ("K", c_int), ("N", c_int), ("lda", c_int), ("ldw", c_int), ("ldo", c_int), ("ld_addend", c_int), ("mode", c_int),
                ("colscale_cols", c_int), ("colscale", c_float)]


class VitBlockF32(ctypes.Structure):
    _fields_ = [(n, c_void_p) for n in ("norm1_g", "norm1_b", "qkv_w", "qkv_b", "proj_w", "proj_b", "ls1", "norm2_g", "norm2_b", "fc1_w", "fc1_b",
                                        "fc2_w", "fc2_b", "ls2")]


class VitConfigF32(ctypes.Structure):
    _fields_ = [("H", c_int), ("W", c_int), ("p", c_int), ("D", c_int), ("heads", c_int), ("Dh", c_int), ("depth", c_int), ("eps", c_float),
                ("img", c_void_p), ("patch_w", c_void_p), ("patch_b", c_void_p), ("cls", c_void_p), ("pos", c_void_p),
                ("blocks", ctypes.POINTER(VitBlockF32)), ("norm_g", c_void_p), ("norm_b", c_void_p), ("x_prenorm", c_void_p), ("x_norm", c_void_p),
                ("n_take", c_int), ("norm_take", c_int), ("take", ctypes.POINTER(c_int)), ("take_out", ctypes.POINTER(c_void_p)),
                ("workspace", c_void_p), ("workspace_bytes", c_size_t)]


SIGNATURES.update({
    "dr_gemm_rows_f32": (c_int, [ctypes.POINTER(GemmRowsF32Args), c_void_p]),
    "dr_patch_rows_f32": (c_int, [c_int, c_int, c_int, c_void_p, c_void_p, c_int, c_void_p]),
    "dr_vit_workspace_bytes_f32": (c_size_t, [c_int] * 5),
    "dr_vit_forward_f32": (c_int, [ctypes.POINTER(VitConfigF32), c_void_p]),
    "dr_debug_gemm_rows_f32_tile": (None, [c_int]),
})


def _bind(table):
    for name, (res, args) in table.items():
        if not hasattr(_lib, name):
            raise ImportError("libdiffreg_hip.so has no %s: it was built from an older tree than this binding; rebuild (make -C diff-reg_amd/csrc)"
                              % name)
        fn = getattr(_lib, name)
        fn.restype = res
        fn.argtypes = args


_bind(SIGNATURES)
_INIT_DONE = False

ABI_VERSION = 700
if _lib.dr_version() // 100 != ABI_VERSION // 100:
    raise ImportError("libdiffreg_hip.so is ABI %d, this binding is written against %d: rebuild (make -C diff-reg_amd/csrc)"
                      % (_lib.dr_version(), ABI_VERSION))


def ensure_init():
    global _INIT_DONE
    if not _INIT_DONE:
        if os.environ.get("DR_DIAGNOSTICS") == "1":
            _lib.dr_debug_enable_env(1)
        check(_lib.dr_init())
        _INIT_DONE = True


SK_OUT_CONF, SK_OUT_LOG, SK_MINSHIFT, SK_APPLY_MASK, SK_OUT_F32, SK_STRICT = 0x0, 0x1, 0x2, 0x4, 0x8, 0x10
SK_RAGGED = 0x20


def raw():
    return _lib


def check(code):
    if code != 0:
        msg = _lib.dr_strerror(code).decode()
        if code == -2:
            msg += ": " + _lib.dr_last_hip_error().decode()
        raise RuntimeError("libdiffreg_hip: %s (%d)" % (msg, code))


def loop_status(workspace, clear=True):
    st = torch.cuda.current_stream(workspace.device).cuda_stream
    check(_lib.dr_denoise_loop_status(ptr(workspace), c_void_p(st), 1 if clear else 0))


def device_status(device=None, clear=True):
    st = torch.cuda.current_stream(device).cuda_stream
    check(_lib.dr_device_status(c_void_p(st), 1 if clear else 0))


def ptr(t):
    if t is None:
        return None
    if not t.is_cuda:
        raise RuntimeError("libdiffreg_hip ops need tensors on a ROCm device (got %s); there is no CPU path" % t.device)
    if not t.is_contiguous():
        raise RuntimeError("libdiffreg_hip ops need contiguous tensors")
    return c_void_p(t.data_ptr())


_RAW_STREAM = getattr(torch._C, "_cuda_getCurrentRawStream", None)


def stream_of(t):
    if _RAW_STREAM is not None:
        dev = t.device
        return c_void_p(_RAW_STREAM(dev.index if dev.index is not None else torch.cuda.current_device()))
    return c_void_p(torch.cuda.current_stream(t.device).cuda_stream)


def mask_u8(m):
    if m is None:
        return None
    if m.dtype == torch.bool:
        return m.contiguous().view(torch.uint8)
    return (m != 0).contiguous().view(torch.uint8)


PL_F32, PL_PLANES, PL_LN = 0, 1, 2


def planes_from_f32(x):
    ensure_init()
    x = x.contiguous()
    rows, K = x.shape
    img = torch.zeros(_lib.dr_plane_image_bytes(rows, K), dtype=torch.uint8, device=x.device)
    bnd = torch.empty(rows, device=x.device)
    check(_lib.dr_planes_from_f32(rows, K, ptr(x), K, ptr(img), ptr(bnd), stream_of(x)))
    return img, bnd


def planes_from_f32_bounded(x, bound_in):
    ensure_init()
    x = x.contiguous()
    rows, K = x.shape
    img = torch.zeros(_lib.dr_plane_image_bytes(rows, K), dtype=torch.uint8, device=x.device)
    bnd = torch.empty(rows, device=x.device)
    check(_lib.dr_planes_from_f32_bounded(rows, K, ptr(x), K, ptr(bound_in.contiguous()), ptr(img), ptr(bnd), stream_of(x)))
    return img, bnd


def attention_planes(q, k, v, H, q_mask=None, k_mask=None, f16=False):
    ensure_init()
    P, Lq, C = q.shape
    Lk = k.shape[1]
    d = C // H
    dp = (d + 15) // 16 * 16

    def pad(x):
        y = torch.zeros(x.shape[0] * x.shape[1], H * dp, device=x.device)
        xr = x.reshape(-1, H, d)
# ... 1376 lines not shown
```

include/diffreg_hip_debug.h:

```cpp
#ifndef DIFFREG_HIP_DEBUG_H
#define DIFFREG_HIP_DEBUG_H
#include "diffreg_hip.h"
#ifdef __cplusplus
extern "C" {
#endif

void dr_debug_enable_env(int on);
void dr_debug_gemm_config(int c);
typedef struct dr_debug_gemm_problem {
    const float* A;
    const float* A2;
    const float* W;
    float* out;
    const float* cos_t;
    const float* sin_t;
    const float* bias;
    const float* addend;
    int rows, ncols, K, K1, lda, lda2, ldo;
    int epilogue;
    int rot_C;
    float scale;
    int nbatch;
    long long stride_a, stride_w, stride_o;
} dr_debug_gemm_problem;
int dr_debug_gemm_f32(const dr_debug_gemm_problem* problems, int n, void* stream);
void dr_debug_attention_config(int flash_min_workgroups);
void dr_debug_attention_split(int on);
#define DR_ATTN_FORM_Q32_W4 1
#define DR_ATTN_FORM_Q32_W8 2
#define DR_ATTN_FORM_FLASH_F32 3
#define DR_ATTN_FORM_FLASH_SPLIT 4
#define DR_ATTN_FORM_PLANES_KG1 5
#define DR_ATTN_FORM_PLANES_KG2 6
#define DR_ATTN_FORM_MASK 0xf
#define DR_ATTN_FORM_F16 0x10
#define DR_ATTN_FORM_XCD 0x20
#define DR_ATTN_FORM_GEOM_SHIFT 8
int dr_debug_attention_last_form(void);
#define DR_PROC_FORM_REG 0
#define DR_PROC_FORM_SLICED 1
#define DR_PROC_FORM_SLICED_REREAD 2
int dr_debug_procrustes_last_form(void);
void dr_debug_sinkhorn_spin_limit(unsigned polls);
void dr_debug_gemm_rows_tile(int c);
void dr_debug_gemm_rows_f32_tile(int c);
int dr_debug_launch_chain(int n, int workgroups, int threads, void* stream);

#ifdef __cplusplus
}
#endif
#endif
```

Baseline: 1200 pairs/s.

## Cache step-invariant mlp0 partial accumulators across denoise evaluations

The first denoise evaluation stores the mlp0 GEMM accumulators after the K-range that depends only on step-invariant inputs (the A0 part). Later evaluations reload those partial sums and run only the remaining K-blocks over A1. This cuts roughly half of that GEMM's K-loop on every step, at the cost of an extra workspace slab plus global store and load traffic. It also skips writing the f32 copy of the final layer output when no trace needs it. The cache is keyed by a shape/form tag and only used on the PLANES, non-ksplit, TNW=7 path.

```diff
diff --git a/diff-reg_amd/csrc/api.hip b/diff-reg_amd/csrc/api.hip
--- a/diff-reg_amd/csrc/api.hip
+++ b/diff-reg_amd/csrc/api.hip
@@ -137,6 +137,7 @@
 void dr_debug_attention_split(int on) { attention_force_split(on); }
 int dr_debug_attention_last_form(void) { return attention_last_form(); }
 int dr_debug_procrustes_last_form(void) { return procrustes_last_form(); }
+int dr_debug_pgemm_acc_forms(int clear) { return pgemm_acc_forms(clear != 0); }
 
 int dr_vol_pe_f32(int rows, int rows_per_pair, int C, const float* xyz, const float* R, const float* t, float origin_x,
                   float origin_y, float origin_z, float voxel, const float* freq, float* cos_out, float* sin_out,
diff --git a/diff-reg_amd/csrc/loop.hip b/diff-reg_amd/csrc/loop.hip
--- a/diff-reg_amd/csrc/loop.hip
+++ b/diff-reg_amd/csrc/loop.hip
@@ -84,6 +84,8 @@
     float* pre0;
     char* v0_img; float *v0_bnd, *grp0;
     char* q1_img; float* q1_bnd;
+    bool hoist_mlp0;
+    float* x0_acc[2]; size_t x0_cap[2]; mutable unsigned long long x0_tag[2];
     float* csT;
     size_t qkv_stride;
     size_t side_C, side_att, side_hid;
@@ -105,7 +107,7 @@
         w.qkv_img = c.take<char>(3 * w.qkv_stride); w.qkv_bnd = c.take<float>(3 * (size_t)T);
         w.kvc_img = c.take<char>(2 * w.qkv_stride); w.kvc_bnd = c.take<float>(2 * (size_t)T);
         w.grp_x = c.take<float>(2 * (size_t)P);
-        w.hoist = false;
+        w.hoist = w.hoist_mlp0 = false;
         w.csT = c.take<float>((size_t)T * C);
         w.own_pack = c.take<char>(Prepack::carve(nullptr, cfg, nullptr));
         const bool xk = (T + 63) / 64 + 2 <= PG_XK_MAX_RB;
@@ -120,6 +122,14 @@
         w.v0_img = c.take<char>(plane_image_bytes(PN, Cq)); w.v0_bnd = c.take<float>(PN); w.grp0 = c.take<float>(P);
         w.q1_img = c.take<char>(plane_image_bytes(PM, Cq)); w.q1_bnd = c.take<float>(T);
         w.hoist = c.off <= bytes && env_knob("DR_LOOP_HOIST", 1) != 0;
+        const int side_rows[2] = {PN, PM};
+        for (int i = 0; i < 2; ++i) {
+            w.x0_cap[i] = pgemm_acc_cache_floats(side_rows[i], cfg.C, 2);
+            w.x0_acc[i] = c.take<float>(w.x0_cap[i]);
+            w.x0_tag[i] = 0;
+        }
+        w.hoist_mlp0 = w.hoist && c.off <= bytes && env_knob("DR_LOOP_HOIST_MLP0", 1) != 0 &&
+                       pgemm_acc_cache_ok(cfg.C, cfg.C / 16, cfg.C / 16, Prepack::wide_layout(cfg) ? 2 : 0);
     }
 };
 
@@ -212,6 +222,10 @@
     bool l0_use = false;
     bool q1_fill = false;
     bool q1_use = false;
+    bool x0_store = false;
+    bool x0_use = false;
+    int x0_slab = 0;
+    bool no_f32_out = false;
 };
 static int layer_call_planes(const PlCtx& X, const dr_layer_weights& W, int l, const Tok& xin, int xs, const Tok& yin, int ys,
                              const Tok& out, const Family& f1, const Family* f2, hipStream_t st, const float* kv_cached = nullptr,
@@ -344,6 +358,11 @@
         p.W = L.mlp0; p.nblk = 2; p.rows = S.rows(side); p.C = C; p.mode = PG_PLANES; p.relu = 1; p.scale = 1.f;
         p.pimg = S.at(pw.hid_img, pw.side_hid, side); p.p_nct = 2 * nC; p.pbnd = pw.hid_bnd + S.r0(side);
         if (p.W.sub == 2) xk(p, xk_wide_units(p));
+        if (hz.x0_store || hz.x0_use) {
+            if (hz.x0_store) p.acc_store = pw.x0_acc[hz.x0_slab];
+            else p.acc_load = pw.x0_acc[hz.x0_slab];
+            p.acc_cap = pw.x0_cap[hz.x0_slab]; p.acc_tag = &pw.x0_tag[hz.x0_slab];
+        }
     });
     ++pw.xk_epoch;
     rc = launch_pgemm(g, st);
@@ -355,7 +374,7 @@
         p.W = L.mlp2; p.nblk = 1; p.rows = S.rows(side); p.C = C; p.mode = PG_LN;
         p.gamma = W.norm2_w; p.beta = W.norm2_b; p.lnB = L.lnB2;
         p.resid = xin.f32 + (size_t)S.r0(side) * C; p.ldr = C; p.bnd_res = xin.bnd + S.r0(side);
-        p.out = out.f32 + (size_t)S.r0(side) * C; p.ldo = C;
+        p.out = hz.no_f32_out ? nullptr : out.f32 + (size_t)S.r0(side) * C; p.ldo = C;
         p.pimg = S.at(out.img, pw.side_C, side); p.p_nct = nC; p.pbnd = out.bnd + S.r0(side);
         xk(p, (size_t)(p.rows + 63) / 64);
     });
@@ -424,7 +443,7 @@
 }
 
 static int denoiser_and_sim(const dr_loop_config& cfg, const dr_loop_weights& w, const float* feat0, const uint8_t* tokmask, DenoiseWs& ws,
-                            const float** final_feats, hipStream_t st, bool use_cache = false) {
+                            const float** final_feats, hipStream_t st, bool use_cache = false, bool first_eval = true, bool final_f32 = true) {
     const Sides& S = ws.S;
     const int C = cfg.C, P = S.P, N = S.La, M = S.Lb, PN = S.rows_a;
     auto head = [&](const float* feats) {
@@ -439,8 +458,13 @@
         const PlCtx X = plane_ctx(cfg, ws, tokmask);
         const Tok* cur = &ws.pl.feat0;
         int rc = DR_OK;
+        const bool x0 = use_cache && ws.pl.hoist_mlp0;
+        const bool head_f32 = env_knob("DR_HEAD_F32", 0) != 0;
+        const bool drop_f32 = !final_f32 && !head_f32;
         if (use_cache) {
             PlHoist hz; hz.l0_use = ws.pl.hoist;
+            hz.x0_store = x0 && first_eval; hz.x0_use = x0 && !first_eval; hz.x0_slab = 0;
+            hz.no_f32_out = drop_f32 && cfg.n_layers == 1;
             rc = layer_call_planes(X, w.layers[0], 0, *cur, SIDE_A, *cur, SIDE_A, ws.pl.tgt_l0, S.self_a(), nullptr, st, nullptr, nullptr, hz);
             cur = &ws.pl.tgt_l0;
         }
@@ -449,11 +473,14 @@
                                 [&](int l, int xs, const Tok* x, int ys, const Tok* y, const Tok* out, const Family& f1, const Family* f2) {
                 const bool l1 = use_cache && l == 1;
                 PlHoist hz; hz.q1_use = l1 && xs == SIDE_B && ws.pl.hoist;
+                const bool x1 = x0 && l1 && xs == SIDE_B;
+                hz.x0_store = x1 && first_eval; hz.x0_use = x1 && !first_eval; hz.x0_slab = 1;
+                hz.no_f32_out = drop_f32 && l == cfg.n_layers - 1;
                 return layer_call_planes(X, w.layers[l], l, *x, xs, *y, ys, *out, f1, f2, st, (l1 && xs == SIDE_A) ? ws.kv_l1 : nullptr, nullptr, hz);
             });
         if (rc) return rc;
-        *final_feats = cur->f32;
-        if (env_knob("DR_HEAD_F32", 0)) {
+        *final_feats = drop_f32 ? nullptr : cur->f32;
+        if (head_f32) {
             rc = head(cur->f32);
             return rc ? rc : sim();
         }
@@ -760,9 +787,11 @@
     sa.noise = v4d ? noise : nullptr; sa.bin_score = w->bin_score; sa.trace = trace;
     sa.x = L.x; sa.x_final = x_final; sa.x0 = L.x0; sa.wconf = L.wconf; sa.R = L.R; sa.t = L.t; sa.Rf = L.Rf; sa.tf = L.tf; sa.cond = L.cond; sa.ok = L.ok;
     sa.skws = L.skws; sa.skws_bytes = L.skws_bytes; sa.pws = L.pws; sa.pws_bytes = L.pws_bytes; sa.status = L.status;
+    const bool final_f32 = trace && (trace->feats_nopos || trace->feats_pos);
+    int evals = 0;
     rc = reverse_sampling(sa, [&](const float* Rf, const float* tf) -> int {
         int r = fill_pe(*cfg, *w, P, N, M, s_pcd, Rf, tf, t_pcd, true, false, L.dw, st);
-        if (r == DR_OK) r = denoiser_and_sim(*cfg, *w, L.feat0, tokmask, L.dw, &fin, st, true);
+        if (r == DR_OK) r = denoiser_and_sim(*cfg, *w, L.feat0, tokmask, L.dw, &fin, st, true, evals++ == 0, final_f32);
         if (r) return r;
         return sinkhorn_f32(P, N, M, L.dw.sim, src_mask, tgt_mask, w->bin_score, cfg->sk_iters, DR_SK_OUT_CONF | mflag, L.x0, L.skws, L.skws_bytes, st,
                             L.status);
diff --git a/diff-reg_amd/csrc/pgemm.h b/diff-reg_amd/csrc/pgemm.h
--- a/diff-reg_amd/csrc/pgemm.h
+++ b/diff-reg_amd/csrc/pgemm.h
@@ -38,6 +38,7 @@
     const float* bias; const float* bias_max;
     float* xk_buf; unsigned* xk_flags; unsigned xk_epoch; unsigned* xk_status; int ksplit;
     int xk_cap;
+    float* acc_store; const float* acc_load; long long acc_stride; size_t acc_cap; unsigned long long* acc_tag;
 };
 constexpr int PG_XK_MAX_RB = 160;
 inline size_t pgemm_xk_buf_bytes(int bn) { return (size_t)PG_XK_MAX_RB * 2 * 4 * (bn / 64) * 2 * 64 * 16; }
@@ -46,6 +47,9 @@
 
 bool pgemm_shape_ok(int C);
 int pgemm_bn(int C);
+bool pgemm_acc_cache_ok(int C, int nc0, int nc1, int sub);
+size_t pgemm_acc_cache_floats(int rows, int C, int nblk);
+int pgemm_acc_forms(bool clear);
 int launch_pgemm(const PgBatch& g, hipStream_t st);
 int pgemm_configure();
 
diff --git a/diff-reg_amd/csrc/pgemm.hip b/diff-reg_amd/csrc/pgemm.hip
--- a/diff-reg_amd/csrc/pgemm.hip
+++ b/diff-reg_amd/csrc/pgemm.hip
@@ -86,6 +86,15 @@
     const int t = threadIdx.x, lane = t & 63, l31 = lane & 31, h = lane >> 5;
     const int w = __builtin_amdgcn_readfirstlane(t >> 6), wm = w % WMN, wn = w / WMN;
     const int rb128 = (rb * BM) >> 7, sub = (rb * BM) & 127;
+    constexpr bool ACC_OK = TNW == 7 && MODE == PG_PLANES;
+    const bool acc_st = ACC_OK && nc1 > 0 && P.acc_store != nullptr, acc_ld = ACC_OK && nc1 > 0 && P.acc_load != nullptr;
+    auto acc_slab = [&]() __attribute__((always_inline)) { return ((size_t)rb * nblk + nb) * (size_t)P.acc_stride + (size_t)threadIdx.x * 4; };
+    auto acc_get = [&](f32x4& x, const float* p) __attribute__((always_inline)) {
+        asm volatile("global_load_dwordx4 %0, %1, off" : "+v"(x) : "v"(p) : "memory");
+    };
+    auto acc_put = [&](float* p, f32x4 x) __attribute__((always_inline)) {
+        asm volatile("global_store_dwordx4 %0, %1, off\n\ts_nop 1" ::"v"(p), "v"(x) : "memory");
+    };
 
     float* const s_fac = reinterpret_cast<float*>(lds + GG::WORK);
     float* const s_rinv = s_fac + 128;
@@ -184,10 +193,29 @@
         const int wl = w % WMN;
         const int st0 = GRP ? wl * (WB_CNT / WMN) + min(wl, WB_CNT % WMN) : WB_CNT + wl * (NW0 / WMN) + min(wl, NW0 % WMN);
         const unsigned voffW = lane * 16 + st0 * 1024, voffA = lane * 16 + 2 * wl * 1024;
-        const char* ga = P.A0 + ((size_t)rb128 * P.nc0 + kbeg) * GG::A_IMG + sub * 64;
-        const char* gb = P.W.img + ((size_t)nb * (P.nc0 + nc1) + kbeg) * GG::B_ST;
         const char* const ga1 = nc1 > 0 ? P.A1 + (size_t)rb128 * nc1 * GG::A_IMG + sub * 64 : nullptr;
-        int ti = 0;
+        const int s0 = acc_ld ? nc0 : 0;
+        const char* ga = acc_ld ? ga1 : P.A0 + ((size_t)rb128 * P.nc0 + kbeg) * GG::A_IMG + sub * 64;
+        const char* gb = P.W.img + ((size_t)nb * (P.nc0 + nc1) + kbeg + s0) * GG::B_ST;
+        int ti = s0;
+        auto acc_fetch = [&]() __attribute__((always_inline)) {
+            if constexpr (ACC_OK) {
+                if (acc_ld) {
+                    const float* const lp = P.acc_load + acc_slab();
+#pragma unroll
+                    for (int j = 0; j < TNW; ++j) {
+                        f32x4 x[4] = {};
+                        __builtin_amdgcn_sched_barrier(0);
+#pragma unroll
+                        for (int r4 = 0; r4 < 4; ++r4) acc_get(x[r4], lp + (size_t)(j * 4 + r4) * (NTHR * 4));
+                        PG_VMCNT(0);
+                        __builtin_amdgcn_sched_barrier(0);
+#pragma unroll
+                        for (int r = 0; r < 16; ++r) acc[j][r] = x[r >> 2][r & 3];
+                    }
+                }
+            }
+        };
 #define PG_DMA(ldsaddr, voff, gbase, imm)                                                                  \
     asm volatile("s_mov_b32 m0, %0\n\ts_nop 0\n\tglobal_load_lds_dwordx4 %1, %2 offset:%3" ::"s"(ldsaddr), "v"(voff), "s"(gbase), "i"(imm) : "memory")
         auto dma_piece = [&](int p, unsigned dstb) __attribute__((always_inline)) {
@@ -212,6 +240,16 @@
             const bool do_issue = STEADY || ti < nst;
             const unsigned dstb = lds_base + (unsigned)(ti % NST) * STAGE;
             if (s == nc0 && nc1 > 0) {
+                if constexpr (ACC_OK) {
+                    if (acc_st) {
+                        float* const sp = P.acc_store + acc_slab();
+#pragma unroll
+                        for (int j = 0; j < TNW; ++j)
+#pragma unroll
+                            for (int r4 = 0; r4 < 4; ++r4)
+                                acc_put(sp + (size_t)(j * 4 + r4) * (NTHR * 4), f32x4{acc[j][4 * r4], acc[j][4 * r4 + 1], acc[j][4 * r4 + 2], acc[j][4 * r4 + 3]});
+                    }
+                }
                 const unsigned fb0 = lds_base + GG::WORK + (wm * 32 + 4 * h) * 4;
                 u32x4 f[4];
                 PG_READ(f[0], fb0, 0); PG_READ(f[1], fb0, 32); PG_READ(f[2], fb0, 64); PG_READ(f[3], fb0, 96);
@@ -280,26 +318,28 @@
 
 #pragma unroll
         for (int q2 = 0; q2 < AHEAD; ++q2) {
-            const unsigned dstb = lds_base + (unsigned)q2 * STAGE;
+            const unsigned dstb = lds_base + (unsigned)((s0 + q2) % NST) * STAGE;
 #pragma unroll
             for (int i = 0; i < NPIECE; ++i) dma_piece(i, dstb);
             dma_advance();
             if (q2 == 0) {
                 __builtin_amdgcn_sched_barrier(0);
                 stage_inputs();
+                acc_fetch();
                 __builtin_amdgcn_sched_barrier(0);
                 PG_VMCNT(0);
             }
         }
         __builtin_amdgcn_s_barrier();
-        PG_READ(fa0[0], lds_base + offAh, 0);
-        PG_READ(fa0[1], lds_base + offAl, 0);
+        const unsigned sb0 = lds_base + (unsigned)(s0 % NST) * STAGE;
+        PG_READ(fa0[0], sb0 + offAh, 0);
+        PG_READ(fa0[1], sb0 + offAl, 0);
 #pragma unroll
         for (int j = 0; j < TNW / 2; ++j) {
-            PG_READ(fx[j][0], lds_base + offBh, j * 2048);
-            PG_READ(fx[j][1], lds_base + offBl, j * 2048);
-        }
-        int s = 0;
+            PG_READ(fx[j][0], sb0 + offBh, j * 2048);
+            PG_READ(fx[j][1], sb0 + offBl, j * 2048);
+        }
+        int s = s0;
         for (; s + 1 < nst - (NST - 1); s += 2) {
             stage(s, std::true_type{}, fa0, fa1);
             stage(s + 1, std::true_type{}, fa1, fa0);
@@ -319,18 +359,31 @@
         for (int i = 0; i < 4; ++i)
 #pragma unroll
             for (int j = 0; j < 7; ++j) c16[i][j] = f32x4{0.f, 0.f, 0.f, 0.f};
+        auto acc_fetch = [&]() __attribute__((always_inline)) {
+            if (acc_ld) {
+                const float* const lp = P.acc_load + acc_slab();
+                __builtin_amdgcn_sched_barrier(0);
+#pragma unroll
+                for (int i = 0; i < 4; ++i)
+#pragma unroll
+                    for (int j = 0; j < 7; ++j) acc_get(c16[i][j], lp + (size_t)(i * 7 + j) * (NTHR * 4));
+                PG_VMCNT(0);
+                __builtin_amdgcn_sched_barrier(0);
+            }
+        };
         u32x4 fb[7][2], fa[2][2];
         const int nv0 = (nc0 + 1) & ~1, nvt = nv0 + ((nc1 + 1) & ~1), npair = nvt >> 1;
         const int z0 = (nc0 & 1) ? nv0 - 1 : -1, z1 = (nc1 & 1) ? nvt - 1 : -1;
         const int wl = w & 3, st0 = wl * 7;
         const unsigned voffW = lane * 16 + st0 * 1024, voffA = lane * 16 + 2 * wl * 1024;
-        const char* ga = P.A0 + (size_t)rb128 * nc0 * GG::A_IMG + sub * 64;
-        const char* gb = P.W.img + (size_t)nb * nst * GG::B_ST;
         const char* const ga1 = nc1 > 0 ? P.A1 + (size_t)rb128 * nc1 * GG::A_IMG + sub * 64 : nullptr;
-        int ti = 0, tr = 0;
+        const int p0 = acc_ld ? nv0 >> 1 : 0;
+        const char* ga = acc_ld ? ga1 : P.A0 + (size_t)rb128 * nc0 * GG::A_IMG + sub * 64;
+        const char* gb = P.W.img + ((size_t)nb * nst + (acc_ld ? nc0 : 0)) * GG::B_ST;
+        int ti = 2 * p0, tr = acc_ld ? nc0 : 0;
         auto piece = [&](int q) __attribute__((always_inline)) {
             if (ti == z0 || ti == z1) return;
-            const unsigned dstb = lds_base + (unsigned)(ti % NST) * STAGE;
+            const unsigned dstb = lds_base + ((unsigned)ti % NST) * STAGE;
             const unsigned m0w = dstb + A_ST + st0 * 1024;
             const int pw = q - 2;
             const unsigned hop = (unsigned)(pw >> 2) * 4096;
@@ -351,6 +404,13 @@
             const unsigned sb = lds_base + (unsigned)(p & 1) * 2 * STAGE, sbn = lds_base + (unsigned)((p + 1) & 1) * 2 * STAGE;
             const bool has_next = STEADY || p + 1 < npair;
             if (2 * p == nv0 && nc1 > 0) {
+                if (acc_st) {
+                    float* const sp = P.acc_store + acc_slab();
+#pragma unroll
+                    for (int i = 0; i < 4; ++i)
+#pragma unroll
+                        for (int j = 0; j < 7; ++j) acc_put(sp + (size_t)(i * 7 + j) * (NTHR * 4), c16[i][j]);
+                }
 #pragma unroll
                 for (int i = 0; i < 4; ++i) {
                     const float f = s_fac[wm2 * 64 + 16 * i + l15];
@@ -426,21 +486,24 @@
             advance();
             __builtin_amdgcn_sched_barrier(0);
             stage_inputs();
+            acc_fetch();
             __builtin_amdgcn_sched_barrier(0);
             PG_VMCNT(0);
 #pragma unroll
             for (int q = 0; q < 7; ++q) piece(q);
         } else {
             stage_inputs();
+            acc_fetch();
         }
         __builtin_amdgcn_s_barrier();
-        PG_READ(fa[0][0], lds_base + oAh, 0);
-        PG_READ(fa[0][1], lds_base + oAl, 0);
-#pragma unroll
-        for (int j = 0; j < 7; ++j) PG_READ(fb[j][1], lds_base + oBl, j * 1024);
-#pragma unroll
-        for (int j = 0; j < 7; ++j) PG_READ(fb[j][0], lds_base + oBh, j * 1024);
-        int p = 0;
+        const unsigned sb0 = lds_base + (unsigned)(p0 & 1) * 2 * STAGE;
+        PG_READ(fa[0][0], sb0 + oAh, 0);
+        PG_READ(fa[0][1], sb0 + oAl, 0);
+#pragma unroll
+        for (int j = 0; j < 7; ++j) PG_READ(fb[j][1], sb0 + oBl, j * 1024);
+#pragma unroll
+        for (int j = 0; j < 7; ++j) PG_READ(fb[j][0], sb0 + oBh, j * 1024);
+        int p = p0;
         for (; p < npair - 2; ++p) stage(p, std::true_type{});
         for (; p < npair; ++p) stage(p, std::false_type{});
     };
@@ -1401,6 +1464,14 @@
 bool pgemm_shape_ok(int C) { return C > 0 && C % 16 == 0 && C <= G9::BN; }
 int pgemm_bn(int C) { return C <= G4::BN ? G4::BN : (C <= G7::BN ? G7::BN : G9::BN); }
 static size_t pg_bst(int C) { return (size_t)pgemm_bn(C) * 64; }
+bool pgemm_acc_cache_ok(int C, int nc0, int nc1, int sub) { return sub == 0 && pgemm_shape_ok(C) && pgemm_bn(C) == G7::BN && nc0 >= 5 && nc1 >= 5; }
+size_t pgemm_acc_cache_floats(int rows, int C, int nblk) { return (size_t)((rows + 127) / 128) * 128 * (size_t)nblk * pgemm_bn(C); }
+static thread_local int g_acc_forms = 0;
+int pgemm_acc_forms(bool clear) {
+    const int f = g_acc_forms;
+    if (clear) g_acc_forms = 0;
+    return f;
+}
 
 template <int TNW, int NST, int MODE>
 static int configure_mode() {
@@ -1442,6 +1513,8 @@
     double flops = 0;
     const int mode = g.p[0].mode;
     if (mode != PG_F32 && mode != PG_PLANES) return DR_ENOSUP;
+    for (int i = 0; i < g.n; ++i)
+        if (g.p[i].acc_store || g.p[i].acc_load) return DR_ENOSUP;
     bool ksplit = env_knob("DR_PG_KSPLIT", 1) != 0 && env_knob("DR_PG_KSPLITW", 1) != 0;
     long tiles = 0;
     for (int i = 0; i < g.n; ++i) {
@@ -1510,11 +1583,25 @@
     PgBatch gd = g;
     gd.dbg = env_knob("DR_PG_NOEPI", 0);
     for (int i = 0; i < g.n; ++i) gd.p[i].ksplit = ksplit ? 1 : 0;
+    bool m16 = env_knob("DR_PG_M16", 1) != 0;
+    for (int i = 0; i < g.n; ++i) m16 = m16 && g.p[i].nc0 >= 5 && (!g.p[i].A1 || g.p[i].nc1 >= 5);
+    for (int i = 0; i < g.n; ++i) {
+        PgProblem& p = gd.p[i];
+        if (!p.acc_store && !p.acc_load) continue;
+        if ((p.acc_store && p.acc_load) || !p.A1 || !p.acc_tag) return DR_EINVAL;
+        if (ksplit || mode != PG_PLANES || !pgemm_acc_cache_ok(p.C, p.nc0, p.nc1, p.W.sub)) return DR_ENOSUP;
+        const int form = half ? 3 : (m16 ? 1 : 2);
+        p.acc_stride = (long long)bm * G7::BN;
+        if ((size_t)((p.rows + bm - 1) / bm) * p.nblk * (size_t)p.acc_stride > p.acc_cap) return DR_EWORKSPACE;
+        const unsigned long long tag = (unsigned long long)form | ((unsigned long long)p.nblk << 4) | ((unsigned long long)p.nc0 << 8) |
+                                       ((unsigned long long)p.nc1 << 20) | ((unsigned long long)p.rows << 32);
+        if (p.acc_store) *p.acc_tag = tag;
+        else if (*p.acc_tag != tag) return DR_EINVAL;
+        g_acc_forms |= 1 << ((p.acc_store ? 0 : 4) + form - 1);
+    }
     if (bn == G9::BN) pg_launch<9, 3, 2>(mode, grid, st, gd);
     else if (bn == G4::BN) { if (half) pg_launch<4, 4, 2>(mode, grid, st, gd); else pg_launch<4, 4, 4>(mode, grid, st, gd); }
     else {
-        bool m16 = env_knob("DR_PG_M16", 1) != 0;
-        for (int i = 0; i < g.n; ++i) m16 = m16 && g.p[i].nc0 >= 5 && (!g.p[i].A1 || g.p[i].nc1 >= 5);
         if (half) pg_launch<7, 4, 2>(mode, grid, st, gd);
         else if (m16) {
             using GG = PgGeom<7, 4, 4>;
diff --git a/diff-reg_amd/diffreg_hip/lib.py b/diff-reg_amd/diffreg_hip/lib.py
--- a/diff-reg_amd/diffreg_hip/lib.py
+++ b/diff-reg_amd/diffreg_hip/lib.py
@@ -169,6 +169,7 @@
     "dr_debug_attention_split": (None, [c_int]),
     "dr_debug_attention_last_form": (c_int, []),
     "dr_debug_procrustes_last_form": (c_int, []),
+    "dr_debug_pgemm_acc_forms": (c_int, [c_int]),
     "dr_pnp_ransac_workspace_bytes": (c_size_t, [c_int, c_int]),
     "dr_pnp_ransac_f64": (c_int, [c_int, c_void_p, c_void_p, c_int, c_void_p, c_int, c_double, ctypes.c_uint64, c_void_p, c_void_p, c_void_p, c_void_p, c_size_t,
                                   c_void_p]),
diff --git a/include/diffreg_hip_debug.h b/include/diffreg_hip_debug.h
--- a/include/diffreg_hip_debug.h
+++ b/include/diffreg_hip_debug.h
@@ -41,6 +41,10 @@
 #define DR_PROC_FORM_SLICED 1
 #define DR_PROC_FORM_SLICED_REREAD 2
 int dr_debug_procrustes_last_form(void);
+#define DR_PGEMM_ACC_FORM_M16 1
+#define DR_PGEMM_ACC_FORM_ROWS128 2
+#define DR_PGEMM_ACC_FORM_ROWS64 3
+int dr_debug_pgemm_acc_forms(int clear);
 void dr_debug_sinkhorn_spin_limit(unsigned polls);
 void dr_debug_gemm_rows_tile(int c);
 void dr_debug_gemm_rows_f32_tile(int c);
```

Result: faster. 1217 pairs/s (median of 6 runs) (+1.4%).
